# zalo/TetSim

Hardware: AMD Instinct MI355X
Metric: tet_solves_per_sec (higher is better)
Workload: dtype f32; 1 GPU; Kuhn-6 cube lattice 55x55x55 cells (998250 tets, 175616 particles), polar-decomposition Jacobi, 20 substeps/frame, dt=1/1200 s; solver=polar_jacobi, arithmetic=fast, formulation=reference (rest shape carried from substep to substep, 148 B/tet), tets=998250, particles=175616, parallelism=single GPU

## Files before the change

### include/tetsim.h

```cpp
#ifndef TETSIM_H
#define TETSIM_H

#include <stdint.h>

#ifdef __cplusplus
extern "C" {
#endif

#define TETSIM_ABI_VERSION 5

typedef struct tetsim_body *tetsim_handle;

enum {
    TETSIM_OK = 0,
    TETSIM_EINVAL = 1,
    TETSIM_ENODEVICE = 2,
    TETSIM_EHIP = 3,
    TETSIM_ENOMEM = 4,
    TETSIM_ECOMM = 5,
    TETSIM_ESTATE = 6
};

enum {
    TETSIM_SOLVER_POLAR_JACOBI = 0,
// ... 215 lines not shown
       TETSIM_POSE_L0 = 16 , TETSIM_POSE_G = 19 , TETSIM_POSE_Q0 = 25,
       TETSIM_POSE_COM = 26 , TETSIM_POSE_VCOM = 29 , TETSIM_POSE_Q = 32 , TETSIM_POSE_OMEGA = 36 ,
       TETSIM_POSE_L = 39 , TETSIM_POSE_RESIDUAL = 42, TETSIM_POSE_GAP = 43, TETSIM_POSE_RESERVED = 44  };
int tetsim_body_poses_device(tetsim_handle h, void *dst, uint64_t row_stride, void *caller_stream);
int tetsim_read_body_poses(tetsim_handle h, double *out);
int tetsim_prep_pose_table(const float *verts, uint32_t nv, const int32_t *tets, uint32_t nt,
                           const uint32_t *body_first_vert, const uint32_t *body_first_tet, uint32_t num_bodies,
                           double density, void *records_out, double *centres_out);


#define TETSIM_RAY_INVALID (-1)
int tetsim_raycast_visual_device(tetsim_handle h,
        const void *rays,     uint64_t ray_stride,
        const void *ray_body,
        uint32_t count,
        void *hits,           uint64_t hit_stride,
        void *caller_stream);
int tetsim_visual_bounding_spheres_device(tetsim_handle h, void *dst, uint64_t row_stride, void *caller_stream);


#define TETSIM_STRAIN_WIDTH 16
#define TETSIM_STRAIN_BODY_WIDTH 8
#define TETSIM_STRAIN_SWEEPS 4
enum { TETSIM_STRAIN_F = 0 , TETSIM_STRAIN_J = 9, TETSIM_STRAIN_DEV = 10,
       TETSIM_STRAIN_STRETCH = 11 , TETSIM_STRAIN_GREEN = 14, TETSIM_STRAIN_RESERVED = 15  };
int tetsim_tet_strain_device(tetsim_handle h, void *dst, uint64_t row_stride, void *caller_stream);
int tetsim_read_tet_strain(tetsim_handle h, float *out);
int tetsim_body_strain_device(tetsim_handle h, void *dst, uint64_t row_stride, void *caller_stream);
int tetsim_visual_strain_device(tetsim_handle h, int32_t channel, void *dst, uint64_t row_stride, void *caller_stream);
int tetsim_prep_strain_table(const float *verts, uint32_t nv, const int32_t *tets, uint32_t nt, double density, void *records_out);


int tetsim_profile(tetsim_handle h, uint32_t n, double dt, const TetSimParams *params, TetSimProfile *out);
int tetsim_time_kernels(tetsim_handle h, uint32_t reps, double dt, const TetSimParams *params, TetSimProfile *out);
int tetsim_time_step_n(tetsim_handle h, uint32_t n, double dt, const TetSimParams *params, double *ms_out);
int tetsim_measure_copy_bandwidth(int32_t device, uint64_t bytes, uint32_t reps, double *gbps_out);
int tetsim_measure_stream_bandwidth(int32_t device, uint64_t bytes, uint32_t reps, int32_t kind, double *gbps_out);


int tetsim_comm_unique_id(void *id128);
int tetsim_comm_init(tetsim_handle h, const void *id128, int32_t rank, int32_t nranks);
typedef struct TetSimCommInfo {
    int32_t rccl_ranks, rccl_rank;
    uint32_t neighbours;
    uint64_t send_bytes_per_substep, recv_bytes_per_substep, max_message_bytes;
    int32_t loopback;
    int32_t p2p;
} TetSimCommInfo;
int tetsim_comm_info(tetsim_handle h, TetSimCommInfo *out);
int tetsim_comm_selftest(tetsim_handle h);
int tetsim_comm_probe(tetsim_handle h, uint64_t bytes, uint32_t reps, int32_t use_graph, uint32_t per_graph,
                      double *host_us, double *total_us);
int tetsim_halo_probe(tetsim_handle h, uint32_t reps, double *min_us, double *median_us, double *max_us);
#define TETSIM_P2P_BLOB_BYTES 512
int tetsim_halo_p2p_export(tetsim_handle h, void *blob);
int tetsim_halo_p2p_connect(tetsim_handle h, const void *blobs, uint32_t count);
int tetsim_halo_p2p_probe(tetsim_handle h, uint32_t reps, double *min_us, double *median_us, double *max_us);
int tetsim_group_step_n(tetsim_handle *handles, uint32_t count, uint32_t n, double dt, const TetSimParams *params);
int tetsim_halo_exchange_local(tetsim_handle *handles, uint32_t count);
int tetsim_get_halo_plan(tetsim_handle h, int32_t *neigh ,
                         int32_t *send_counts, int32_t *recv_counts,
                         int32_t *send_ids, int32_t *recv_ids);
int tetsim_halo_export(tetsim_handle h, uint32_t n, float *out_xyzw);
int tetsim_halo_import(tetsim_handle h, uint32_t n, const float *in_xyzw);


int tetsim_prep_levels(const int32_t *tets, uint32_t nt, uint32_t nv, int32_t *level, uint32_t *num_levels);
int tetsim_prep_colours(const int32_t *tets, uint32_t nt, uint32_t nv, int32_t *colour, uint32_t *num_colours);
int tetsim_prep_clusters(const int32_t *tets, uint32_t nt, uint32_t nv, int32_t *order, int32_t *launch, int32_t *lane,
                         int32_t *step, uint32_t *num_launches, uint32_t *num_clusters);
int tetsim_prep_tiles(const float *verts, uint32_t nv, const int32_t *tets, uint32_t nt, const uint32_t *body_first_tet,
                      const uint32_t *body_first_vert, uint32_t bodies, int32_t *tile_tets, uint32_t *tile_off,
                      uint8_t *corner_slot, uint32_t *num_tiles);
int tetsim_prep_slot_table(const int32_t *tets, uint32_t nt, uint32_t nv, int32_t ref_quirk,
                           int32_t *slots , uint32_t *dropped);
int tetsim_prep_call_tiles(const float *verts, uint32_t nv, const int32_t *tets, uint32_t nt, uint32_t sizes[4],
                           uint32_t *blk_vert_off, int32_t *blk_verts, uint32_t *vp_ell);
int tetsim_prep_call_schedule(const int32_t *blk_verts, const uint32_t *blk_vert_off, uint32_t nb, const uint32_t *vp_ell,
                              uint32_t vp_cols, uint32_t nv_pad, uint32_t nv_owned, uint32_t lag, uint32_t *entry,
                              uint32_t capacity, uint32_t *period, uint32_t *tail, int32_t *fell_back);
int tetsim_prep_check_call_schedule(const int32_t *blk_verts, const uint32_t *blk_vert_off, uint32_t nb, const uint32_t *vp_ell,
                                    uint32_t vp_cols, uint32_t nv_pad, uint32_t nv_owned, const uint32_t *entry, uint32_t period,
                                    uint32_t tail);
int tetsim_prep_ref_grab_texels(int32_t grab_id, uint32_t num_elems, uint32_t num_particles, int32_t out[2]);
int tetsim_prep_boundary_surface(const float *verts ,
                                 const int32_t *tets, uint32_t nt, uint32_t nv,
                                 float *vis_verts , int32_t *tri_ids ,
                                 uint32_t *nrows, uint32_t *ntri);
int tetsim_prep_rest(const float *verts, uint32_t nv, const int32_t *tets, uint32_t nt, double density,
                     float *inv_mass, float *inv_rest_pose, float *inv_rest_volume);

int tetsim_prep_partition(const float *verts , uint32_t nv, const int32_t *tets, uint32_t nt,
                          int32_t part_count, int32_t *vert_owner_out);
typedef struct TetSimPartQuality {
    uint32_t owned_particles;
    uint32_t ghost_particles;
    uint32_t boundary_particles;
    uint32_t local_elems;
    uint32_t owned_elems;
    uint32_t num_neighbours;
} TetSimPartQuality;
int tetsim_prep_partition_quality(const int32_t *tets, uint32_t nt, uint32_t nv, int32_t part_count,
                                  const int32_t *vert_owner, TetSimPartQuality *out);

typedef struct tetsim_plan_s *tetsim_plan;
typedef struct TetSimPlanSizes {
    uint32_t owned_particles, boundary_particles, local_particles, local_elems, owned_elems, num_neighbours;
} TetSimPlanSizes;
int tetsim_plan_create(const int32_t *tets, uint32_t nt, uint32_t nv, int32_t part_count, int32_t part_index,
                       const int32_t *vert_owner, tetsim_plan *out);
int tetsim_plan_create_deep(const int32_t *tets, uint32_t nt, uint32_t nv, int32_t part_count, int32_t part_index,
                            const int32_t *vert_owner, int32_t depth, tetsim_plan *out);
int tetsim_plan_layers(tetsim_plan p, uint32_t *first_layer_ghosts, uint8_t *tet_layer);
int tetsim_plan_neighbour_layer2(tetsim_plan p, uint32_t i, uint32_t *send_count, uint32_t *recv_start, uint32_t *recv_count);
int tetsim_plan_neighbour_layer2_ids(tetsim_plan p, uint32_t i, int32_t *send_local, int32_t *send_global, int32_t *recv_global);
void tetsim_plan_destroy(tetsim_plan p);
int tetsim_plan_sizes(tetsim_plan p, TetSimPlanSizes *out);
int tetsim_plan_arrays(tetsim_plan p, int32_t *local_to_global_vert, int32_t *local_to_global_tet, int32_t *local_tets);
int tetsim_plan_neighbour(tetsim_plan p, uint32_t i, int32_t *rank, uint32_t *send_count, uint32_t *recv_start,
                          uint32_t *recv_count, int32_t *send_is_contiguous);
int tetsim_plan_neighbour_ids(tetsim_plan p, uint32_t i, int32_t *send_local, int32_t *send_global, int32_t *recv_global);

int tetsim_abi_version(void);
typedef struct TetSimLibraryInfo {
    int32_t abi;
    int32_t ablation;
    uint32_t debug_env;
    char source_sha[20];
    char kernel_sha[20];
} TetSimLibraryInfo;
int tetsim_library_info(TetSimLibraryInfo *out);

typedef struct TetSimMeshArrays {
    uint32_t num_particles;
    uint32_t num_elems;
    uint32_t num_edges;
    uint32_t num_vis_verts;
    uint32_t num_vis_tris;
    uint32_t part_count;
    const float *verts;
    const int32_t *tets;
    const int32_t *edge_ids;
    const float *vis_verts;
    const int32_t *vis_tri_ids;
    const int32_t *tet_colour;
    const int32_t *vert_owner;
} TetSimMeshArrays;
typedef struct tetsim_mesh_file *tetsim_mesh;

int tetsim_mesh_write(const char *path, const TetSimMeshArrays *a);
int tetsim_mesh_open(const char *path, tetsim_mesh *out);
int tetsim_mesh_arrays(tetsim_mesh m, TetSimMeshArrays *out);
int tetsim_mesh_close(tetsim_mesh m);
int tetsim_create_from_file(const char *path, const TetSimOptions *opts, tetsim_handle *out);

#ifdef __cplusplus
}
#endif
#endif
```

### tetsim_amd/_capi.py

```python
import ctypes as C
import os

_HERE = os.path.dirname(os.path.abspath(__file__))
LIB_PATH = os.environ.get("TETSIM_HIP_LIB") or os.path.join(_HERE, "libtetsim_hip.so")

OK, EINVAL, ENODEVICE, EHIP, ENOMEM, ECOMM, ESTATE = range(7)
RAY_INVALID = -1
SOLVER_POLAR_JACOBI, SOLVER_NEOHOOKEAN_GS = 0, 1
PRECISE, FAST = 0, 1
ORDER_ORIGINAL, ORDER_COLOURED, ORDER_CLUSTERED = 0, 1, 2
FLAG_REF_SLOT_TABLE, FLAG_REF_FIXED_BOUNDS, FLAG_GATHER_FORMULATION, FLAG_CONSTANT_REST_SHAPE, FLAG_REF_GRAB_TEXEL, FLAG_DEEP_GHOSTS = 1, 2, 4, 8, 16, 32
FLAG_REF_ROTATION_EXIT = 64
FLAG_LEAN_STATE = 128
K_TET, K_VERTEX, K_HALO, K_COUNT = 0, 1, 2, 3
COLLIDER_SPHERE, COLLIDER_CAPSULE, COLLIDER_BOX, COLLIDER_PLANE = 0, 1, 2, 3
MAX_COLLIDERS = 8
BODY_COLLIDER_FLOATS = 24
BODY_PARAMS_WIDTH = 10
BP_GRAVITY, BP_FRICTION, BP_DEV_COMPLIANCE, BP_VOL_COMPLIANCE, BP_BOUNDS_LO, BP_BOUNDS_HI = 0, 1, 2, 3, 4, 7
FIELD_POSITIONS, FIELD_VELOCITIES, FIELD_PREV_POSITIONS, FIELD_QUATS, FIELD_VISUAL_POSITIONS, FIELD_VISUAL_NORMALS, FIELD_VISUAL_VERTEX_NORMALS = range(7)
MAX_EXPORT_FIELDS = 8
OBS_WIDTH = 20
(OBS_MASS, OBS_COM, OBS_VCOM, OBS_VOLUME, OBS_REST_VOLUME, OBS_MIN_VOLUME_RATIO, OBS_INVERTED_TETS, OBS_AABB_MIN, OBS_AABB_MAX, OBS_MAX_SPEED2,
 OBS_NONFINITE, OBS_RESERVED) = 0, 1, 4, 7, 8, 9, 10, 11, 14, 17, 18, 19
# ... 40 lines not shown
                ("substeps", C.c_uint32), ("tets_per_tet_launch", C.c_uint32)]


class TetSimLibraryInfo(C.Structure):
    _fields_ = [("abi", C.c_int32), ("ablation", C.c_int32), ("debug_env", C.c_uint32), ("source_sha", C.c_char * 20),
                ("kernel_sha", C.c_char * 20)]


DEBUG_ENV_NAMES = ["TETSIM_DEBUG_LOOPBACK_HALO", "TETSIM_DEBUG_LOOPBACK_COPY", "TETSIM_DEBUG_ONE_STREAM", "TETSIM_DEBUG_GROUP_SYNC",
                   "TETSIM_DEBUG_HOSTPROF", "TETSIM_DEBUG_TRACE", "TETSIM_HALO_SYNC", "TETSIM_HALO_GRAPH", "TETSIM_DEBUG_LOOPBACK_DELAY_US", "TETSIM_NH_QUADS", "TETSIM_FUSED_PARTICLE_PASS",
                   "TETSIM_FRAME_KERNEL", "TETSIM_FRAME_LOCAL", "TETSIM_NH_FOLD", "TETSIM_HALO_ALIGNED_TILES", "TETSIM_HALO_FOLD_WAIT", "TETSIM_QUAD", "TETSIM_QUAD_POLL_DELAY", "TETSIM_NH_FRAME",
                   "TETSIM_NH_ONE_LAUNCH", "TETSIM_PJ_ONE_LAUNCH", "TETSIM_PJ_CALL_LAG"]


LAB_ENV_NAMES = ["TETSIM_DEBUG_TRACE", "TETSIM_NH_QUADS", "TETSIM_FRAME_LOCAL", "TETSIM_NH_FOLD", "TETSIM_HALO_ALIGNED_TILES", "TETSIM_QUAD_POLL_DELAY", "TETSIM_NH_FRAME"]


class TetSimCommInfo(C.Structure):
    _fields_ = [("rccl_ranks", C.c_int32), ("rccl_rank", C.c_int32), ("neighbours", C.c_uint32), ("send_bytes_per_substep", C.c_uint64),
                ("recv_bytes_per_substep", C.c_uint64), ("max_message_bytes", C.c_uint64), ("loopback", C.c_int32), ("p2p", C.c_int32)]


class TetSimPlanSizes(C.Structure):
    _fields_ = [("owned_particles", C.c_uint32), ("boundary_particles", C.c_uint32), ("local_particles", C.c_uint32),
                ("local_elems", C.c_uint32), ("owned_elems", C.c_uint32), ("num_neighbours", C.c_uint32)]


class TetSimPartQuality(C.Structure):
    _fields_ = [("owned_particles", C.c_uint32), ("ghost_particles", C.c_uint32), ("boundary_particles", C.c_uint32),
                ("local_elems", C.c_uint32), ("owned_elems", C.c_uint32), ("num_neighbours", C.c_uint32)]


class TetSimError(RuntimeError):
    def __init__(self, code, msg):
        super().__init__("tetsim error %d: %s" % (code, msg))
        self.code = code


class TetSimCollider(C.Structure):
    _fields_ = [("kind", C.c_int32), ("reserved", C.c_int32), ("a", C.c_double * 3), ("b", C.c_double * 3), ("axes", C.c_double * 9),
                ("radius", C.c_double), ("friction", C.c_double), ("velocity", C.c_double * 3)]


class TetSimRay(C.Structure):
    _fields_ = [("origin", C.c_double * 3), ("direction", C.c_double * 3), ("near", C.c_double), ("far", C.c_double)]


class TetSimRayHit(C.Structure):
    _fields_ = [("hit", C.c_int32), ("body", C.c_int32), ("triangle", C.c_int32), ("reserved", C.c_int32), ("distance", C.c_double),
                ("point", C.c_double * 3)]


class TetSimDeviceField(C.Structure):
    _fields_ = [("field", C.c_int32), ("reserved", C.c_int32), ("dst", C.c_void_p), ("row_stride", C.c_uint64)]


SYMBOLS = [
    "tetsim_abi_version", "tetsim_default_options", "tetsim_default_params", "tetsim_create", "tetsim_create_batch", "tetsim_get_batch_layout", "tetsim_destroy",
    "tetsim_last_error", "tetsim_get_info", "tetsim_step", "tetsim_step_n", "tetsim_sync",
    "tetsim_library_info", "tetsim_read_quats_pinned", "tetsim_state_size", "tetsim_save_state", "tetsim_load_state",
    "tetsim_read_positions", "tetsim_read_positions_pinned", "tetsim_read_prev_positions", "tetsim_read_velocities", "tetsim_read_quats",
    "tetsim_read_vol_error", "tetsim_write_state", "tetsim_get_owned_ids", "tetsim_get_local_tets",
    "tetsim_get_tet_order", "tetsim_get_level_offsets", "tetsim_read_inv_mass", "tetsim_set_visual_mesh", "tetsim_get_visual_ids", "tetsim_halo_refresh_final", "tetsim_group_refresh_final", "tetsim_halo_probe", "tetsim_halo_p2p_probe",
    "tetsim_read_visual_mesh", "tetsim_set_visual_triangles", "tetsim_read_visual_vertex_normals", "tetsim_visual_vertex_normals_from", "tetsim_group_read_visual_vertex_normals", "tetsim_set_grab", "tetsim_set_colliders",
    "tetsim_start_grab", "tetsim_nearest_particle", "tetsim_profile", "tetsim_time_kernels", "tetsim_time_step_n", "tetsim_measure_copy_bandwidth", "tetsim_measure_stream_bandwidth",
    "tetsim_comm_unique_id", "tetsim_comm_init", "tetsim_comm_info", "tetsim_comm_selftest", "tetsim_comm_probe", "tetsim_group_step_n", "tetsim_halo_exchange_local", "tetsim_get_halo_plan",
    "tetsim_halo_p2p_export", "tetsim_halo_p2p_connect",
    "tetsim_halo_export", "tetsim_halo_import", "tetsim_prep_levels", "tetsim_prep_colours", "tetsim_prep_clusters",
    "tetsim_prep_tiles", "tetsim_prep_slot_table", "tetsim_prep_call_tiles", "tetsim_prep_call_schedule", "tetsim_prep_check_call_schedule", "tetsim_prep_ref_grab_texels", "tetsim_prep_rest", "tetsim_prep_partition", "tetsim_prep_partition_quality", "tetsim_plan_create", "tetsim_plan_destroy", "tetsim_plan_sizes",
    "tetsim_plan_arrays", "tetsim_plan_neighbour", "tetsim_plan_neighbour_ids",
    "tetsim_plan_create_deep", "tetsim_plan_layers", "tetsim_plan_neighbour_layer2", "tetsim_plan_neighbour_layer2_ids",
    "tetsim_raycast_visual", "tetsim_start_grab_ray", "tetsim_read_visual_bounding_sphere", "tetsim_prep_boundary_surface",
    "tetsim_export_device", "tetsim_import_device",
    "tetsim_snapshot_create", "tetsim_snapshot_capture", "tetsim_snapshot_restore", "tetsim_snapshot_destroy",
    "tetsim_observe_bodies_device", "tetsim_read_body_observations",
    "tetsim_body_poses_device", "tetsim_read_body_poses", "tetsim_prep_pose_table",
    "tetsim_raycast_visual_device", "tetsim_visual_bounding_spheres_device",
    "tetsim_tet_strain_device", "tetsim_read_tet_strain", "tetsim_body_strain_device", "tetsim_visual_strain_device", "tetsim_prep_strain_table",
    "tetsim_set_body_grabs", "tetsim_set_body_grabs_device", "tetsim_nearest_particles_device",
    "tetsim_set_body_colliders", "tetsim_set_body_colliders_device",
    "tetsim_set_body_params", "tetsim_set_body_params_device",
    "tetsim_place_bodies_device", "tetsim_place_bodies",
    "tetsim_mesh_write", "tetsim_mesh_open", "tetsim_mesh_arrays", "tetsim_mesh_close", "tetsim_create_from_file",
]

OPTIONAL_SYMBOLS = ("tetsim_set_colliders", "tetsim_raycast_visual", "tetsim_start_grab_ray", "tetsim_read_visual_bounding_sphere", "tetsim_prep_boundary_surface",
                    "tetsim_export_device", "tetsim_import_device",
                    "tetsim_snapshot_create", "tetsim_snapshot_capture", "tetsim_snapshot_restore", "tetsim_snapshot_destroy",
                    "tetsim_observe_bodies_device", "tetsim_read_body_observations",
                    "tetsim_raycast_visual_device", "tetsim_visual_bounding_spheres_device",
                    "tetsim_tet_strain_device", "tetsim_read_tet_strain", "tetsim_body_strain_device", "tetsim_visual_strain_device", "tetsim_prep_strain_table",
                    "tetsim_set_body_grabs", "tetsim_set_body_grabs_device", "tetsim_nearest_particles_device",
                    "tetsim_set_body_colliders", "tetsim_set_body_colliders_device",
                    "tetsim_set_body_params", "tetsim_set_body_params_device",
                    "tetsim_place_bodies_device", "tetsim_place_bodies",
                    "tetsim_body_poses_device", "tetsim_read_body_poses", "tetsim_prep_pose_table")

_lib = None


def lib():
    global _lib
    if _lib is not None:
        return _lib
    if not os.path.exists(LIB_PATH):
        raise ImportError("libtetsim_hip.so is not built: run `python -m tetsim_amd.build` "
                          "(the HIP extension is mandatory; there is no CPU fallback)")
    L = C.CDLL(LIB_PATH)
    H, fp, ip, dp = C.c_void_p, C.POINTER(C.c_float), C.POINTER(C.c_int32), C.POINTER(C.c_double)
    u32, i32, dbl = C.c_uint32, C.c_int32, C.c_double
    PP = C.POINTER(TetSimParams)
    L.tetsim_abi_version.restype = C.c_int
    L.tetsim_default_options.argtypes = [C.POINTER(TetSimOptions)]
    L.tetsim_default_options.restype = None
    L.tetsim_default_params.argtypes = [PP]
    L.tetsim_default_params.restype = None
    L.tetsim_create.argtypes = [fp, u32, ip, u32, C.POINTER(TetSimOptions), C.POINTER(H)]
    L.tetsim_create_batch.argtypes = [C.POINTER(fp), C.POINTER(u32), C.POINTER(ip), C.POINTER(u32), u32, C.POINTER(TetSimOptions), C.POINTER(H)]
    L.tetsim_get_batch_layout.argtypes = [H, C.POINTER(u32), C.POINTER(u32)]
    L.tetsim_destroy.argtypes = [H]
    L.tetsim_destroy.restype = None
    L.tetsim_comm_probe.argtypes = [H, C.c_uint64, u32, i32, u32, dp, dp]
    L.tetsim_nearest_particle.argtypes = [H, fp, ip, dp]
    L.tetsim_mesh_write.argtypes = [C.c_char_p, C.POINTER(TetSimMeshArrays)]
    L.tetsim_mesh_open.argtypes = [C.c_char_p, C.POINTER(H)]
    L.tetsim_mesh_arrays.argtypes = [H, C.POINTER(TetSimMeshArrays)]
    L.tetsim_mesh_close.argtypes = [H]
    L.tetsim_create_from_file.argtypes = [C.c_char_p, C.POINTER(TetSimOptions), C.POINTER(H)]
    L.tetsim_last_error.argtypes = [H]
    L.tetsim_last_error.restype = C.c_char_p
    L.tetsim_get_info.argtypes = [H, C.POINTER(TetSimInfo)]
    L.tetsim_step.argtypes = [H, dbl, PP]
    L.tetsim_step_n.argtypes = [H, u32, dbl, PP]
    L.tetsim_sync.argtypes = [H]
    for n in ("positions", "prev_positions", "velocities", "quats", "inv_mass"):
        getattr(L, "tetsim_read_" + n).argtypes = [H, fp]
    L.tetsim_read_positions_pinned.argtypes = [H, C.POINTER(fp)]
    L.tetsim_read_quats_pinned.argtypes = [H, C.POINTER(fp)]
    L.tetsim_library_info.argtypes = [C.POINTER(TetSimLibraryInfo)]
    L.tetsim_state_size.argtypes = [H, C.POINTER(C.c_uint64)]
    L.tetsim_save_state.argtypes = [H, C.c_void_p, C.c_uint64]
    L.tetsim_load_state.argtypes = [H, C.c_void_p, C.c_uint64]
    L.tetsim_read_vol_error.argtypes = [H, dp]
    L.tetsim_write_state.argtypes = [H, fp, fp]
    for n in ("owned_ids", "local_tets", "tet_order", "level_offsets"):
        getattr(L, "tetsim_get_" + n).argtypes = [H, ip]
    L.tetsim_set_visual_mesh.argtypes = [H, fp, u32, fp]
    L.tetsim_read_visual_mesh.argtypes = [H, fp, fp]
    L.tetsim_get_visual_ids.argtypes = [H, C.POINTER(C.c_int32)]
    L.tetsim_halo_refresh_final.argtypes = [H]
    L.tetsim_halo_probe.argtypes = [H, u32, C.POINTER(C.c_double), C.POINTER(C.c_double), C.POINTER(C.c_double)]
    L.tetsim_halo_p2p_probe.argtypes = [H, u32, C.POINTER(C.c_double), C.POINTER(C.c_double), C.POINTER(C.c_double)]
    L.tetsim_group_refresh_final.argtypes = [C.POINTER(H), u32]
    L.tetsim_set_visual_triangles.argtypes = [H, ip, u32]
    L.tetsim_read_visual_vertex_normals.argtypes = [H, fp]
    L.tetsim_visual_vertex_normals_from.argtypes = [H, fp, fp]
    L.tetsim_group_read_visual_vertex_normals.argtypes = [C.POINTER(H), u32, fp, fp]
    L.tetsim_set_grab.argtypes = [H, i32, fp]
    if hasattr(L, "tetsim_set_colliders"):
        L.tetsim_set_colliders.argtypes = [H, C.POINTER(TetSimCollider), u32]
    L.tetsim_start_grab.argtypes = [H, fp, ip]
    if hasattr(L, "tetsim_raycast_visual"):
        L.tetsim_raycast_visual.argtypes = [H, C.c_void_p, u32, C.c_void_p]
        L.tetsim_start_grab_ray.argtypes = [H, C.POINTER(TetSimRay), C.POINTER(TetSimRayHit), ip]
        L.tetsim_read_visual_bounding_sphere.argtypes = [H, dp, dp]
        L.tetsim_prep_boundary_surface.argtypes = [fp, ip, u32, u32, fp, ip, C.POINTER(u32), C.POINTER(u32)]
    if hasattr(L, "tetsim_export_device"):
        L.tetsim_export_device.argtypes = [H, C.POINTER(TetSimDeviceField), u32, C.c_void_p]
        L.tetsim_import_device.argtypes = [H, C.c_void_p, C.c_uint64, C.c_void_p, C.c_uint64, C.c_void_p]
    if hasattr(L, "tetsim_snapshot_create"):
        L.tetsim_snapshot_create.argtypes = [H, C.POINTER(H)]
        L.tetsim_snapshot_capture.argtypes = [H, H, C.c_void_p, C.c_void_p]
        L.tetsim_snapshot_restore.argtypes = [H, H, C.c_void_p, C.c_void_p]
        L.tetsim_snapshot_destroy.argtypes = [H]
        L.tetsim_snapshot_destroy.restype = None
    if hasattr(L, "tetsim_observe_bodies_device"):
        L.tetsim_observe_bodies_device.argtypes = [H, C.c_void_p, C.c_uint64, C.c_void_p]
        L.tetsim_read_body_observations.argtypes = [H, dp]
    if hasattr(L, "tetsim_raycast_visual_device"):
        L.tetsim_raycast_visual_device.argtypes = [H, C.c_void_p, C.c_uint64, C.c_void_p, u32, C.c_void_p, C.c_uint64, C.c_void_p]
        L.tetsim_visual_bounding_spheres_device.argtypes = [H, C.c_void_p, C.c_uint64, C.c_void_p]
    if hasattr(L, "tetsim_tet_strain_device"):
        L.tetsim_tet_strain_device.argtypes = [H, C.c_void_p, C.c_uint64, C.c_void_p]
        L.tetsim_read_tet_strain.argtypes = [H, fp]
        L.tetsim_body_strain_device.argtypes = [H, C.c_void_p, C.c_uint64, C.c_void_p]
        L.tetsim_visual_strain_device.argtypes = [H, i32, C.c_void_p, C.c_uint64, C.c_void_p]
        L.tetsim_prep_strain_table.argtypes = [fp, u32, ip, u32, dbl, C.c_void_p]
    if hasattr(L, "tetsim_set_body_grabs"):
        L.tetsim_set_body_grabs.argtypes = [H, ip, fp]
        L.tetsim_set_body_grabs_device.argtypes = [H, C.c_void_p, C.c_void_p, C.c_uint64, C.c_void_p, C.c_void_p]
        L.tetsim_nearest_particles_device.argtypes = [H, C.c_void_p, C.c_uint64, C.c_void_p, C.c_void_p, C.c_void_p]
    if hasattr(L, "tetsim_set_body_colliders"):
        L.tetsim_set_body_colliders.argtypes = [H, fp, u32]
        L.tetsim_set_body_colliders_device.argtypes = [H, C.c_void_p, C.c_uint64, u32, C.c_void_p, C.c_void_p]
    if hasattr(L, "tetsim_set_body_params"):
        L.tetsim_set_body_params.argtypes = [H, C.POINTER(C.c_double)]
        L.tetsim_set_body_params_device.argtypes = [H, C.c_void_p, C.c_uint64, C.c_void_p, C.c_void_p]
    if hasattr(L, "tetsim_place_bodies_device"):
        L.tetsim_place_bodies_device.argtypes = [H, C.c_void_p, C.c_uint64, C.c_void_p, u32, C.c_void_p]
        L.tetsim_place_bodies.argtypes = [H, fp, C.POINTER(C.c_uint8), u32]
    if hasattr(L, "tetsim_body_poses_device"):
        L.tetsim_body_poses_device.argtypes = [H, C.c_void_p, C.c_uint64, C.c_void_p]
        L.tetsim_read_body_poses.argtypes = [H, dp]
        L.tetsim_prep_pose_table.argtypes = [fp, u32, ip, u32, C.POINTER(u32), C.POINTER(u32), u32, dbl, C.c_void_p, dp]
    L.tetsim_profile.argtypes = [H, u32, dbl, PP, C.POINTER(TetSimProfile)]
    L.tetsim_time_kernels.argtypes = [H, u32, dbl, PP, C.POINTER(TetSimProfile)]
    L.tetsim_time_step_n.argtypes = [H, u32, dbl, PP, dp]
    L.tetsim_measure_copy_bandwidth.argtypes = [i32, C.c_uint64, u32, dp]
    L.tetsim_measure_stream_bandwidth.argtypes = [i32, C.c_uint64, u32, i32, dp]
    L.tetsim_comm_unique_id.argtypes = [C.c_void_p]
    L.tetsim_comm_init.argtypes = [H, C.c_void_p, i32, i32]
    L.tetsim_comm_selftest.argtypes = [H]
    L.tetsim_comm_info.argtypes = [H, C.POINTER(TetSimCommInfo)]
    L.tetsim_group_step_n.argtypes = [C.POINTER(H), u32, u32, dbl, PP]
    L.tetsim_halo_exchange_local.argtypes = [C.POINTER(H), u32]
    L.tetsim_halo_p2p_export.argtypes = [H, C.c_void_p]
    L.tetsim_halo_p2p_connect.argtypes = [H, C.c_void_p, u32]
    L.tetsim_get_halo_plan.argtypes = [H, ip, ip, ip, ip, ip]
    L.tetsim_halo_export.argtypes = [H, u32, fp]
    L.tetsim_halo_import.argtypes = [H, u32, fp]
    L.tetsim_prep_levels.argtypes = [ip, u32, u32, ip, C.POINTER(u32)]
    L.tetsim_prep_colours.argtypes = [ip, u32, u32, ip, C.POINTER(u32)]
    L.tetsim_prep_clusters.argtypes = [ip, u32, u32, ip, ip, ip, ip, C.POINTER(u32), C.POINTER(u32)]
    L.tetsim_prep_tiles.argtypes = [fp, u32, ip, u32, C.POINTER(u32), C.POINTER(u32), u32, ip, C.POINTER(u32), C.POINTER(C.c_uint8), C.POINTER(u32)]
    L.tetsim_prep_slot_table.argtypes = [ip, u32, u32, i32, ip, C.POINTER(u32)]
    up = C.POINTER(u32)
    L.tetsim_prep_call_tiles.argtypes = [fp, u32, ip, u32, up, up, ip, up]
    L.tetsim_prep_call_schedule.argtypes = [ip, up, u32, up, u32, u32, u32, u32, up, u32, up, up, ip]
    L.tetsim_prep_check_call_schedule.argtypes = [ip, up, u32, up, u32, u32, u32, up, u32, u32]
    L.tetsim_prep_ref_grab_texels.argtypes = [i32, u32, u32, ip]
    L.tetsim_prep_rest.argtypes = [fp, u32, ip, u32, dbl, fp, fp, fp]
    L.tetsim_prep_partition.argtypes = [fp, u32, ip, u32, i32, ip]
    L.tetsim_prep_partition_quality.argtypes = [ip, u32, u32, i32, ip, C.POINTER(TetSimPartQuality)]
    L.tetsim_plan_create.argtypes = [ip, u32, u32, i32, i32, ip, C.POINTER(H)]
    L.tetsim_plan_destroy.argtypes = [H]
    L.tetsim_plan_destroy.restype = None
    L.tetsim_plan_sizes.argtypes = [H, C.POINTER(TetSimPlanSizes)]
    L.tetsim_plan_arrays.argtypes = [H, ip, ip, ip]
    L.tetsim_plan_neighbour.argtypes = [H, u32, ip, C.POINTER(u32), C.POINTER(u32), C.POINTER(u32), ip]
    L.tetsim_plan_neighbour_ids.argtypes = [H, u32, ip, ip, ip]
    L.tetsim_plan_create_deep.argtypes = [ip, u32, u32, i32, i32, ip, i32, C.POINTER(H)]
    L.tetsim_plan_layers.argtypes = [H, C.POINTER(u32), C.POINTER(C.c_uint8)]
    L.tetsim_plan_neighbour_layer2.argtypes = [H, u32, C.POINTER(u32), C.POINTER(u32), C.POINTER(u32)]
    L.tetsim_plan_neighbour_layer2_ids.argtypes = [H, u32, ip, ip, ip]
    for s in SYMBOLS:
        if s in OPTIONAL_SYMBOLS and not hasattr(L, s):
            continue
        f = getattr(L, s)
        if s not in ("tetsim_default_options", "tetsim_default_params", "tetsim_destroy", "tetsim_last_error",
                     "tetsim_plan_destroy", "tetsim_snapshot_destroy"):
            f.restype = C.c_int
    _lib = L
    return L


def library_info():
    li = TetSimLibraryInfo()
    check(lib().tetsim_library_info(C.byref(li)))
    return {"abi": li.abi, "ablation": bool(li.ablation), "source_sha": li.source_sha.decode(), "kernel_sha": li.kernel_sha.decode(),
            "debug_env": [n for i, n in enumerate(DEBUG_ENV_NAMES) if li.debug_env >> i & 1], "path": LIB_PATH}


def check(rc, handle=None):
    if rc != OK:
        msg = lib().tetsim_last_error(handle)
        raise TetSimError(rc, msg.decode("utf-8", "replace") if msg else "")
```

### tetsim_amd/csrc/body.h

```cpp
#pragma once
#include <dlfcn.h>
#include <hip/hip_runtime.h>
#include <rccl/rccl.h>

#include <algorithm>
#include <atomic>
#include <chrono>
#include <cmath>
#include <cstdio>
#include <cstdlib>
#include <cstring>
#include <map>
#include <string>
#include <vector>

#include "../../include/tetsim.h"
#include "dev_common.h"
#include "dev_store.h"
#include "query_device.h"
#include "host_prep.h"
#include "mesh_file.h"

namespace tetsim {

// ... 105 lines not shown
    double* partial = nullptr;
    float* rows = nullptr;
    bool ready = false;
};

struct PoseRec {
    double m;
    double q[3];
};
static_assert(sizeof(PoseRec) == 32 && alignof(PoseRec) == 8, "two dwordx4 loads per record");
struct PoseDev {
    const void* table = nullptr;
    double* partial = nullptr;
    double* rows = nullptr;
    bool ready = false;
};

}

using namespace tetsim;

struct tetsim_snapshot_s;

struct tetsim_body {
    std::string err;
    TetSimOptions opt{};
    TetSimInfo info{};
    hipStream_t stream = nullptr, comm_stream = nullptr;
    hipEvent_t ev_fork = nullptr, ev_bnd_tet = nullptr;
    uint32_t interior_tets = 0;
    bool queues_probed = false, queues_independent = false;
    uint64_t probe_generation = 0;
    std::map<uint32_t, std::pair<hipGraphExec_t, hipGraphExec_t>> flag_graphs;
    uint32_t* d_sync = nullptr;
    bool flag_sync = false;
    bool halo_graph_broken = false;
    bool halo_warm = false;
    bool loopback = false;
    bool vel_dead = false;
    bool needs_halo_refresh = false;
    bool fork_needed = true;
    hipEvent_t ev_a = nullptr, ev_b = nullptr, ev_halo = nullptr;
    hipEvent_t ev_boundary2[2] = {nullptr, nullptr}, ev_packed2[2] = {nullptr, nullptr}, ev_sent2[2] = {nullptr, nullptr};
    uint32_t halo_parity = 0;
    DevParams* d_params = nullptr;
    DevParams* d_params_halo = nullptr;
    std::vector<int32_t> tet_colour;
    int32_t grab_global = -1;
    int32_t grab_ref[2] = {-1, -1};
    float grab_pos[3] = {0, 0, 0};
    uint32_t n_colliders = 0;
    DevColliderF col[kMaxColliders] = {};
    DevColliderD d_col[kMaxColliders] = {};
    bool body_grabs_on = false;
    uint32_t* d_grab_body = nullptr;
    int4* d_grab_rows = nullptr;
    bool body_colliders_on = false;
    uint32_t* d_bcol_count = nullptr;
    DevColliderF* d_bcol_f = nullptr;
    DevColliderD* d_bcol_d = nullptr;
    bool body_params_on = false;
    BodyParamsF* d_bp_f = nullptr;
    BodyParamsD* d_bp_d = nullptr;
    uint32_t* d_tet_body = nullptr;
    uint32_t* d_body_first = nullptr;
    double* d_near_d2 = nullptr;
    uint32_t* d_near_id = nullptr;
    std::map<uint32_t, hipGraphExec_t> graphs;
    std::vector<void*> allocs;
    std::vector<float> h_verts;
    std::vector<int32_t> h_tets;
    std::vector<uint32_t> batch_first_vert, batch_first_tet;
    bool fast = false;

    PJDev pj;
    PJBlk blk;
    bool blocked = false;
    bool halo_use_flags = true;
    bool halo_use_graph = true;
    bool fused = false;
    bool pj_one_launch = false;
    uint32_t* d_substep_err = nullptr;
    PJCallSched call_sched;
    float4 *rest0_a = nullptr, *rest0_b = nullptr, *rest0_c = nullptr;
    bool quat_stale = false;
    bool frame = false;
    uint32_t frame_epoch = 1;
    uint32_t fold_wave_limit = 0, fold_tile_limit = 0;
    bool quad = false;
    uint32_t* d_frame_err = nullptr;
    int32_t* d_block_tile = nullptr;
    uint32_t frame_blocks = 0;
    DevParams params_on_device;
    bool params_known = false;
    bool frame_local = false;
    bool frame_turn_counted = false;
    bool epoch_block_fresh = false;
    bool frame_exclusive = false;
    float4* partial_b = nullptr;
    size_t partial_slots = 0;
    float4* pos_final_b = nullptr;
    bool fold_halo = false;
    bool fold_possible = false;
    bool fold_wait = false;
    bool v_pending = false;
    uint32_t fuse_step = 0;
    bool fin_in_b = false;
    std::vector<int32_t> tet_perm;
    std::vector<uint32_t> api2dev, dev2api;
    Partition part;
    bool partitioned = false;
    std::vector<int32_t> g2l_owned;
    std::vector<NeighDev> neigh;
    bool pred_any_dt = true;
    float dt_pred = 0.0f;
    ncclComm_t comm = nullptr;
    int comm_rank = -1, comm_size = 0;
    bool deep = false;
    uint32_t n_ghost1 = 0, nb_first = 0;
    std::vector<int32_t> g2l_ghost1;
    bool p2p = false;
    uint32_t timeout_ms = 0;
    float4* ghost_alt = nullptr;
    uint32_t* d_arrived = nullptr;
    uint32_t* d_peer_slots = nullptr;
    uint32_t p2p_cols = 0, p2p_stride = 0;
    uint32_t* d_peer_slots2 = nullptr;
    uint32_t p2p_cols2 = 0;
    float4* own_g1_even[2] = {nullptr, nullptr};
    float4* own_g1_final[2] = {nullptr, nullptr};
    float4* own_g2_even[2] = {nullptr, nullptr};
    float4* own_g2_odd[2] = {nullptr, nullptr};
    std::vector<PeerLink> links;
    uint32_t p2p_probe_base = 0;
    uint64_t p2p_round = 0;
    bool p2p_raise_pending = false;
    bool halo_pending = false;
    bool final_ghosts_fresh = false;
    std::vector<tetsim_body*> group;

    SkinDev skin;
    std::vector<uint32_t> vis_tet;
    std::vector<int32_t> vis_global;
    bool vis_attached = false;
    uint32_t vis_total = 0;
    float4* d_vis_full = nullptr;
    float* pinned_pos = nullptr;
    float* d_packed = nullptr;
    size_t packed_cap = 0;
    float* pinned_quat = nullptr;
    uint32_t* d_api2dev = nullptr;
    hipEvent_t ev_io[2][2] = {{nullptr, nullptr}, {nullptr, nullptr}};
    uint32_t io_parity = 0;
    std::vector<tetsim_snapshot_s*> snapshots;
    uint32_t *d_snap_first_vert = nullptr, *d_snap_first_elem = nullptr, *d_snap_tet_body = nullptr;
    float* d_place_rows = nullptr;
    uint8_t* d_place_mask = nullptr;
    ChunkTable chunk_table[2];
    ObsDev obs;
    StrainDev strain;
    PoseDev pose;
    double* d_best = nullptr; uint32_t* d_best_id = nullptr;
    uint32_t* d_sphere = nullptr;
    RayIn* d_rays = nullptr; RayPrep* d_ray_prep = nullptr; RayOut* d_ray_hits = nullptr; RayCand* d_ray_cand = nullptr;
    size_t ray_cap = 0, ray_prep_cap = 0, ray_hits_cap = 0, ray_cand_cap = 0;
    std::vector<int32_t> vis_row_body, tri_body;
// ... 196 lines not shown
```

### tetsim_amd/csrc/dev_common.h

```cpp
#pragma once
#include <hip/hip_ext.h>
#include <hip/hip_runtime.h>

#include "host_prep.h"

#include <cstddef>
#include <cstdint>

namespace tetsim {

constexpr uint32_t kMaxColliders = 8;
struct DevColliderF {
    float a[3], b[3], u[9], radius, friction, v[3];
    int32_t kind, pad;
};
struct DevColliderD {
    double a[3], b[3], u[9], radius, friction, v[3];
    int32_t kind, pad;
};

__host__ __device__ inline float ref_fixed_lo(int c) { return c == 1 ? -1.0f : -2.5f; }
__host__ __device__ inline float ref_fixed_hi(int c) { return c == 1 ? 10.0f : 2.5f; }
struct BodyParamsF { float gravity, friction, dev_compliance, vol_compliance, lo[3], hi[3], pad[2]; };
struct BodyParamsD { double gravity, friction, dev_compliance, vol_compliance, lo[3], hi[3]; };
// ... 23 lines not shown
    const BodyParamsD* bp_d;
    const uint32_t* tet_body;
    DevColliderF col[kMaxColliders];
    DevColliderD d_col[kMaxColliders];
};
constexpr size_t kDevParamsHead = offsetof(DevParams, col);
static_assert(kDevParamsHead % 8 == 0 && offsetof(DevParams, d_col) % 8 == 0, "DevParams layout");
constexpr size_t kKernelArgLimit = 4096;
static_assert(sizeof(DevParams) <= 2560, "DevParams must leave room for the other by-value arguments of a launch");
__device__ __forceinline__ void store_params(DevParams* dst, const DevParams& v) {
    const uint2* s = reinterpret_cast<const uint2*>(&v);
    uint2* d = reinterpret_cast<uint2*>(dst);
#pragma unroll
    for (size_t i = 0; i < kDevParamsHead / 8; i++) d[i] = s[i];
    for (uint32_t k = 0; k < v.n_colliders && k < kMaxColliders; k++) { dst->col[k] = v.col[k]; dst->d_col[k] = v.d_col[k]; }
}

__device__ __forceinline__ void body_grab_pick(const DevParams& P, uint32_t v, bool& held, float& x, float& y, float& z) {
    if (P.body_grabs) {
        const int4 row = P.grab_rows[P.grab_body[v]];
        held = row.x == static_cast<int32_t>(v);
        if (held) { x = __int_as_float(row.y); y = __int_as_float(row.z); z = __int_as_float(row.w); }
    }
}
__device__ __forceinline__ uint32_t body_colliders_body(const DevParams& P, uint32_t v) { return P.body_colliders ? P.grab_body[v] : 0u; }
__device__ __forceinline__ void body_colliders_pick(const DevParams& P, uint32_t body, const DevColliderF** list, uint32_t* count) {
    *list = P.col; *count = P.n_colliders;
    if (P.body_colliders) { *list = P.bcol_f + static_cast<size_t>(body) * kMaxColliders; *count = P.bcol_count[body]; }
}
__device__ __forceinline__ void body_colliders_pick(const DevParams& P, uint32_t body, const DevColliderD** list, uint32_t* count) {
    *list = P.d_col; *count = P.n_colliders;
    if (P.body_colliders) { *list = P.bcol_d + static_cast<size_t>(body) * kMaxColliders; *count = P.bcol_count[body]; }
}

__device__ __forceinline__ const BodyParamsF* body_params_row(const DevParams& P, uint32_t body, float) { return P.bp_f + body; }
__device__ __forceinline__ const BodyParamsD* body_params_row(const DevParams& P, uint32_t body, double) { return P.bp_d + body; }
__device__ __forceinline__ uint32_t body_params_uniform(uint32_t body) { return static_cast<uint32_t>(__builtin_amdgcn_readfirstlane(static_cast<int32_t>(body))); }
struct PolarBodyParams { float gravity, friction, lo[3], hi[3]; };
template <bool kUniform>
__device__ __forceinline__ PolarBodyParams body_params_polar(const DevParams& P, uint32_t v) {
    PolarBodyParams o = {P.gravity, P.friction, {P.lo[0], P.lo[1], P.lo[2]}, {P.hi[0], P.hi[1], P.hi[2]}};
    if (P.body_params) {
        uint32_t body = P.grab_body[v];
        if constexpr (kUniform) body = body_params_uniform(body);
        const BodyParamsF* const r = body_params_row(P, body, 0.0f);
        o.gravity = r->gravity; o.friction = r->friction;
        for (int k = 0; k < 3; k++) { o.lo[k] = r->lo[k]; o.hi[k] = r->hi[k]; }
    }
    return o;
}

struct PJDev {
    uint32_t nv_local = 0, nv_owned = 0, nv_boundary = 0, nt = 0;
    uint32_t nt_pad = 0;
    uint32_t nv_pad = 0;
    uint32_t max_valence = 0;
    float4* pos_pred = nullptr;
    float4* pos_final = nullptr;
    float4* vel = nullptr;
    int4* tet_idx = nullptr;
    float4* elem = nullptr;
    float4* quat = nullptr;
    int32_t* slot_tab = nullptr;
    uint32_t* slot_cnt = nullptr;
    const DevParams* params = nullptr;
    float rot_exit_w2 = 1.0e-18f;
};

struct PJBlk {
    uint32_t nb = 0, nb_interior = 0, nt = 0, nv_local = 0, nv_owned = 0, nv_boundary = 0;
    const uint32_t* blk_tet_off = nullptr;
    const uint32_t* blk_vert_off = nullptr;
    const int32_t* blk_verts = nullptr;
    const uchar4* tet_lidx = nullptr;
    float4* rest_a = nullptr;
    float4* rest_b = nullptr;
    float4* rest_c = nullptr;
    float* rest_c1 = nullptr;
    const float* vol = nullptr;
    float4* quat = nullptr;
    const uint32_t* lc_range = nullptr;
    const uint2* lc_ent = nullptr;
    float4* partial = nullptr;
    const float* wsum = nullptr;
    const uint32_t* vp_ell = nullptr;
    uint32_t vp_cols = 0, nv_pad = 0;
    float4* pos_pred = nullptr;
    float4* pos_final = nullptr;
    float4* vel = nullptr;
    const float4* partial_prev = nullptr;
    const float4* fin_in = nullptr;
    float4* fin_out = nullptr;
    const uint32_t* slot_src = nullptr;
    const uint32_t* blk_maxsrc = nullptr;
    uint32_t ns_pad = 0;
    const DevParams* params = nullptr;
    const float4* ghost_alt = nullptr;
    const float4* ghost2 = nullptr;
    uint32_t n_ghost1 = 0xffffffffu;
    bool lean = false;
    bool lean_state = false;
    float rot_exit_w2 = 1.0e-18f;
    uint32_t epoch = 0;
    unsigned long long* trace = nullptr;
    unsigned long long* iter_hist = nullptr;
};

struct NHDev {
    uint32_t nv = 0, nt = 0;
    float4* pos = nullptr;
    float4* prev = nullptr;
    float4* vel = nullptr;
    int4* tet_idx = nullptr;
    float4* irp_a = nullptr;
    float4* irp_b = nullptr;
    float4* irp_c = nullptr;
    double* vol_err = nullptr;
    int32_t* order = nullptr;
    uint32_t* corner_slots = nullptr;
    const DevParams* params = nullptr;
};
constexpr uint32_t max_grid_blocks(uint32_t threads) { return 0xffffffffu / threads; }
struct PJCallSched { const uint32_t* entry = nullptr; uint32_t period = 0, tail = 0; };
constexpr uint32_t pjb_call_chunk(uint32_t period, uint32_t tail, uint32_t threads, uint32_t cap) {
    const uint32_t room = max_grid_blocks(threads) > tail ? max_grid_blocks(threads) - tail : 0u;
    const uint32_t fit = period ? room / period : cap;
    return fit < 1u ? 1u : fit < cap ? fit : cap;
}
constexpr uint32_t nh_call_blocks_per_sub(uint32_t blocks) { return (blocks + 7u) & ~7u; }
constexpr uint32_t call_chunk(uint32_t per_sub, uint32_t threads, uint32_t cap) {
    const uint32_t fit = per_sub ? max_grid_blocks(threads) / per_sub : cap;
    return fit < 1u ? 1u : fit < cap ? fit : cap;
}
static_assert(pjb_call_chunk(pjb_call_blocks_per_sub(2282u, 103823u, 256u), 0u, 256u, 8192u) == 6223u, "46-cell lattice: 2,696 blocks per substep");
static_assert(pjb_call_chunk(pjb_call_blocks_per_sub(2282u, 103823u, 256u), 2696u, 256u, 8192u) == 6222u, "... and a tail of a whole period takes one substep's room");
static_assert(call_chunk(nh_call_blocks_per_sub(2601u), 256u, 65000u / 8u) == 6432u, "55-cell lattice, clustered: 2,608 blocks per substep");

constexpr uint32_t kNHClusterVerts = 8, kNHClusterTets = 8;
struct NHClusterLaunch {
    uint32_t nsteps = 0, clusters = 0;
    uint32_t first[kNHClusterTets] = {}, count[kNHClusterTets] = {};
    const int32_t* slot_vid = nullptr;
    const uint8_t* first_mask = nullptr;
};

struct NHSweepColour {
    NHClusterLaunch L;
    const float* slot_im = nullptr;
    const uint2* delta = nullptr;
    const uint8_t* last_mask = nullptr;
    const uint2* delta_first = nullptr;
    uint32_t first_block = 0;
    uint32_t pad = 0;
};
struct NHSweep {
    const NHSweepColour* colours = nullptr;
    uint32_t ncolours = 0, blocks = 0;
    float4* exchange = nullptr;
    uint32_t* error = nullptr;
    uint32_t timeout_ms = 0;
};
void nh_launch_sweep1_fast(hipStream_t s, const NHDev& d, const NHSweep& w, bool fold, uint32_t sub_index, uint32_t epoch);
void nh_launch_call_fast(hipStream_t s, const NHDev& d, const NHSweep& w, uint32_t n);

void pj_launch_tet_precise(hipStream_t s, const PJDev& d, hipEvent_t e0 = nullptr, hipEvent_t e1 = nullptr);
void pj_launch_tet_fast(hipStream_t s, const PJDev& d, hipEvent_t e0 = nullptr, hipEvent_t e1 = nullptr);
void pj_launch_vertex_precise(hipStream_t s, const PJDev& d, uint32_t first, uint32_t count, hipEvent_t e0 = nullptr, hipEvent_t e1 = nullptr);
void pj_launch_vertex_fast(hipStream_t s, const PJDev& d, uint32_t first, uint32_t count, hipEvent_t e0 = nullptr, hipEvent_t e1 = nullptr);
void pj_launch_repredict_precise(hipStream_t s, const PJDev& d);
void pj_launch_repredict_fast(hipStream_t s, const PJDev& d);

void nh_launch_post_predict_precise(hipStream_t s, const NHDev& d);
void nh_launch_post_predict_fast(hipStream_t s, const NHDev& d);
void nh_launch_cluster_precise(hipStream_t s, const NHDev& d, const NHClusterLaunch& L, bool fold = false);
void nh_launch_cluster_fast(hipStream_t s, const NHDev& d, const NHClusterLaunch& L, bool fold = false);
struct NHFrameLaunch {
    const uint32_t* seg = nullptr;
    const uint32_t* first_vert = nullptr;
    uint32_t levels = 0, bodies = 0, block = 512;
    uint32_t max_body_particles = 0;
};
void nh_launch_frame_precise(hipStream_t s, const NHDev& d, const NHFrameLaunch& f, uint32_t n, const DevParams& params, DevParams* params_dev);
void nh_launch_frame_fast(hipStream_t s, const NHDev& d, const NHFrameLaunch& f, uint32_t n, const DevParams& params, DevParams* params_dev);
constexpr uint32_t kNHQuadLevelFast = 128, kNHQuadLevelPrecise = 64;
void nh_launch_level4_fast(hipStream_t s, const NHDev& d, uint32_t first, uint32_t count);
void nh_launch_level4_precise(hipStream_t s, const NHDev& d, uint32_t first, uint32_t count);
uint32_t nh_frame_lds_limit_precise();
uint32_t nh_frame_lds_limit_fast();
void nh_launch_post_predict_list_precise(hipStream_t s, const NHDev& d, const uint32_t* list, uint32_t n);
void nh_launch_post_predict_list_fast(hipStream_t s, const NHDev& d, const uint32_t* list, uint32_t n);
void pjb_launch_tet(hipStream_t s, const PJBlk& d, uint32_t tile_first, uint32_t tile_count, hipEvent_t e0 = nullptr,
                    hipEvent_t e1 = nullptr, uint32_t* raise_word = nullptr, uint32_t* clear_word = nullptr);
void pjb_launch_call(hipStream_t s, const PJBlk& d, const PJCallSched& sched, uint32_t n, uint32_t* err, uint32_t timeout_ms, const DevParams& params, DevParams* params_dev);
void pjb_launch_tet_fused(hipStream_t s, const PJBlk& d, hipEvent_t e0 = nullptr, hipEvent_t e1 = nullptr);
void pjb_launch_vertex(hipStream_t s, const PJBlk& d, uint32_t first, uint32_t count, hipEvent_t e0 = nullptr, hipEvent_t e1 = nullptr,
                       uint32_t* raise_word = nullptr, uint32_t* clear_word = nullptr);
void pjb_launch_repredict(hipStream_t s, const PJBlk& d);
void pjb_launch_recover_quats(hipStream_t s, const PJBlk& d, const float4* rest0_a, const float4* rest0_b, const float4* rest0_c);
void pjb_launch_frame(hipStream_t s, const PJBlk& d, uint32_t n, const int32_t* block_tile, uint32_t blocks, bool local, float4* pbuf0, float4* pbuf1,
                      uint32_t* err, uint32_t timeout_ms, const DevParams& params, DevParams* params_dev, hipEvent_t e0 = nullptr, hipEvent_t e1 = nullptr);
void pjq_launch_frame(hipStream_t s, const PJBlk& d, uint32_t n, const int32_t* block_tile, uint32_t blocks, bool local, float4* pbuf0, float4* pbuf1,
                      uint32_t* err, uint32_t timeout_ms, const DevParams& params, DevParams* params_dev, hipEvent_t e0 = nullptr, hipEvent_t e1 = nullptr);
void pjq_launch_tet(hipStream_t s, const PJBlk& d, hipEvent_t e0 = nullptr, hipEvent_t e1 = nullptr);
void pjq_launch_vertex(hipStream_t s, const PJBlk& d, hipEvent_t e0 = nullptr, hipEvent_t e1 = nullptr);
uint32_t pjq_frame_capacity(uint32_t* compute_units);
uint32_t pjb_frame_capacity(int mode, uint32_t* compute_units);
void pjb_wait_capacity(int mode, uint32_t* vertex_waves, uint32_t* hwait_blocks);
inline int pjb_mode(const PJBlk& d) { return d.lean ? 1 : d.lean_state ? 2 : 0; }
uint32_t pjb_probe_xcd(hipStream_t s, uint32_t blocks);
struct PJSync {
    uint32_t* flag = nullptr;
    uint32_t* error = nullptr;
    uint32_t timeout_ms = 0;
};
constexpr uint32_t kMaxPeers = 8;
struct PJPeer {
    float4* ghost[kMaxPeers] = {};
    const uint32_t* slots = nullptr;
    uint32_t cols = 0, stride = 0, n = 0;
    float4* fin[kMaxPeers] = {};
    float4* ghost2[kMaxPeers] = {};
    const uint32_t* slots2 = nullptr;
    uint32_t cols2 = 0;
};
struct PJPeerSync {
    uint32_t* raise[kMaxPeers] = {};
    uint32_t* wait[kMaxPeers] = {};
    uint32_t n_raise = 0, n_wait = 0;
    uint32_t delay_us = 0;
};
void pjb_launch_wait(hipStream_t s, const PJSync& y);
void pjb_launch_wait_peers(hipStream_t s, const PJSync& y, const PJPeerSync& w);
struct PJClear { uint32_t* word[kMaxPeers + 1] = {}; uint32_t n = 0; };
void pjb_launch_vertex_peer(hipStream_t s, const PJBlk& d, uint32_t first, uint32_t count, const PJPeer& peer, uint32_t* raise_word, const PJClear& clr = PJClear());
void pjb_launch_tet_hwait(hipStream_t s, const PJBlk& d, uint32_t tile_first, uint32_t tile_count, const PJSync& yv, const PJPeerSync& w, const float4* ghosts);
void pjb_launch_tet_alt(hipStream_t s, const PJBlk& d, uint32_t tile_first, uint32_t tile_count);
void pjb_launch_signal(hipStream_t s, const PJSync& y, uint32_t* clear_word = nullptr);
void pjb_launch_vertex_await(hipStream_t s, const PJBlk& d, uint32_t first, uint32_t count, const PJSync& y, hipEvent_t e0 = nullptr, hipEvent_t e1 = nullptr);

void nh_launch_predict_precise(hipStream_t s, const NHDev& d);
void nh_launch_predict_fast(hipStream_t s, const NHDev& d);
void nh_launch_predict_value_precise(hipStream_t s, const NHDev& d, const DevParams& params, DevParams* params_dev);
void nh_launch_predict_value_fast(hipStream_t s, const NHDev& d, const DevParams& params, DevParams* params_dev);
void nh_launch_level_precise(hipStream_t s, const NHDev& d, uint32_t first, uint32_t count);
void nh_launch_level_fast(hipStream_t s, const NHDev& d, uint32_t first, uint32_t count);
void nh_launch_post_precise(hipStream_t s, const NHDev& d);
void nh_launch_post_fast(hipStream_t s, const NHDev& d);

struct SkinDev {
    uint32_t nvis = 0;
    const int4* corner = nullptr;
    const float4* weight = nullptr;
    const int32_t* qidx = nullptr;
    const float4* normal0 = nullptr;
    float4* out_pos = nullptr;
    float4* out_nrm = nullptr;
    uint32_t ntri = 0;
    const int4* tri = nullptr;
    const uint32_t* vt_off = nullptr;
    const uint32_t* vt_tri = nullptr;
    float4* out_vnrm = nullptr;
    const float4* tri_pos = nullptr;
};
void skin_launch(hipStream_t s, const SkinDev& d, const float4* pos, const float4* quat, bool js_order);
void skin_launch_vertex_normals(hipStream_t s, const SkinDev& d);

void util_launch_nearest(hipStream_t s, const float4* pos, const uint32_t* map, uint32_t n, double px, double py, double pz,
                         double* best_d2, uint32_t* best_id);
void util_launch_copy(hipStream_t s, const float4* src, float4* dst, uint64_t n);
void util_launch_stream(hipStream_t s, int kind, bool nt, uint32_t unroll, uint32_t grid, const float4* src, float4* dst, uint64_t n);
void util_launch_delay(hipStream_t s, uint32_t us);
struct P2PProbe { uint32_t* raise[kMaxPeers] = {}; uint32_t* wait[kMaxPeers] = {}; uint32_t n = 0; };
void util_launch_set_params(hipStream_t s, DevParams* dst, const DevParams& v);
void util_launch_p2p_probe(hipStream_t s, const P2PProbe& p, uint32_t base, uint32_t reps, unsigned long long* ticks, uint32_t* error, uint32_t timeout_ms);
void util_launch_gather4(hipStream_t s, const float4* src, const int32_t* idx, float4* dst, uint32_t n);

// ... 25 lines not shown
```

### tetsim_amd/csrc/dev_store.h

```cpp
#pragma once
#include <hip/hip_runtime.h>

#ifndef TETSIM_POLL_SLEEP
#define TETSIM_POLL_SLEEP 8
#endif
#ifndef TETSIM_NH_POLL_SLEEP
#define TETSIM_NH_POLL_SLEEP 2
#endif

namespace tetsim {

constexpr uint32_t kStoreWtMaxIndex = 1u << 27;

typedef unsigned int v4u_t __attribute__((ext_vector_type(4)));

__device__ __forceinline__ void store_wt(float4* base, uint32_t index, const float4& v) {
    const __amdgpu_buffer_rsrc_t rsrc = __builtin_amdgcn_make_buffer_rsrc(base, 0, 0x7fffffff, 0x00020000);
    const v4u_t x = {__float_as_uint(v.x), __float_as_uint(v.y), __float_as_uint(v.z), __float_as_uint(v.w)};
    __builtin_amdgcn_raw_buffer_store_b128(x, rsrc, static_cast<int>(index * 16u), 0, 0x11);
}

__device__ __forceinline__ void store_wt1(float* base, uint32_t index, float v) {
    const __amdgpu_buffer_rsrc_t rsrc = __builtin_amdgcn_make_buffer_rsrc(base, 0, 0x7fffffff, 0x00020000);
    __builtin_amdgcn_raw_buffer_store_b32(__float_as_uint(v), rsrc, static_cast<int>(index * 4u), 0, 0x11);
}

__device__ __forceinline__ void store_plain(float4* base, uint32_t index, const float4& v) {
    const __amdgpu_buffer_rsrc_t rsrc = __builtin_amdgcn_make_buffer_rsrc(base, 0, 0x7fffffff, 0x00020000);
    const v4u_t x = {__float_as_uint(v.x), __float_as_uint(v.y), __float_as_uint(v.z), __float_as_uint(v.w)};
    __builtin_amdgcn_raw_buffer_store_b128(x, rsrc, static_cast<int>(index * 16u), 0, 0);
}
__device__ __forceinline__ float4 load_l2(const float4* base, uint32_t index) {
    const __amdgpu_buffer_rsrc_t rsrc = __builtin_amdgcn_make_buffer_rsrc(const_cast<float4*>(base), 0, 0x7fffffff, 0x00020000);
    const v4u_t x = __builtin_amdgcn_raw_buffer_load_b128(rsrc, static_cast<int>(index * 16u), 0, 0x10);
    return make_float4(__uint_as_float(x.x), __uint_as_float(x.y), __uint_as_float(x.z), __uint_as_float(x.w));
}

__device__ __forceinline__ float4 load_coherent(const float4* base, uint32_t index) {
    const __amdgpu_buffer_rsrc_t rsrc = __builtin_amdgcn_make_buffer_rsrc(const_cast<float4*>(base), 0, 0x7fffffff, 0x00020000);
    const v4u_t x = __builtin_amdgcn_raw_buffer_load_b128(rsrc, static_cast<int>(index * 16u), 0, 0x11);
    return make_float4(__uint_as_float(x.x), __uint_as_float(x.y), __uint_as_float(x.z), __uint_as_float(x.w));
}

__device__ __forceinline__ float load_coherent1(const float* base, uint32_t index) {
    const __amdgpu_buffer_rsrc_t rsrc = __builtin_amdgcn_make_buffer_rsrc(const_cast<float*>(base), 0, 0x7fffffff, 0x00020000);
    return __uint_as_float(__builtin_amdgcn_raw_buffer_load_b32(rsrc, static_cast<int>(index * 4u), 0, 0x11));
}

}
```

### tetsim_amd/csrc/host_prep.cpp

```cpp
#include "host_prep.h"

#include <algorithm>
#include <cmath>
#include <numeric>

namespace tetsim {

namespace {
inline float fround(double x) { return static_cast<float>(x); }

inline void edge_matrix(const float* verts, const int32_t* t, float m[9]) {
    for (int k = 0; k < 3; k++)
        for (int c = 0; c < 3; c++)
            m[3 * k + c] = fround(static_cast<double>(verts[3 * t[k + 1] + c]) - static_cast<double>(verts[3 * t[0] + c]));
}
inline double det3(const float* A) {
    double a11 = A[0], a12 = A[3], a13 = A[6];
    double a21 = A[1], a22 = A[4], a23 = A[7];
    double a31 = A[2], a32 = A[5], a33 = A[8];
    return a11 * a22 * a33 + a12 * a23 * a31 + a13 * a21 * a32 - a13 * a22 * a31 - a12 * a21 * a33 - a11 * a23 * a32;
}
}

void prep_rest(const float* verts, uint32_t nv, const int32_t* tets, uint32_t nt, double density,
// ... 468 lines not shown
namespace {
struct SchedDeps {
    uint32_t per_xcd = 0, tet_blocks = 0, npb = 0, plain_period = 0;
    std::vector<std::vector<uint32_t>> tiles_of_pb, pbs_of_tile;
};
SchedDeps sched_deps(const int32_t* blk_verts, const uint32_t* blk_vert_off, uint32_t nb, const uint32_t* vp_ell, uint32_t vp_cols, uint32_t nv_pad,
                     uint32_t nv_owned, uint32_t tile) {
    SchedDeps D;
    D.per_xcd = (nb + 7u) / 8u; D.tet_blocks = D.per_xcd * 8u; D.npb = (nv_owned + tile - 1u) / tile;
    D.plain_period = pjb_call_blocks_per_sub(nb, nv_owned, tile);
    D.tiles_of_pb.resize(D.npb); D.pbs_of_tile.resize(nb);
    for (uint32_t v = 0; v < nv_owned; v++)
        for (uint32_t j = 0; j < vp_cols; j++) {
            const uint32_t idx = vp_ell[static_cast<size_t>(j) * nv_pad + v];
            if (idx == 0xffffffffu) continue;
            const uint32_t b = static_cast<uint32_t>(std::upper_bound(blk_vert_off, blk_vert_off + nb + 1, idx) - blk_vert_off) - 1u;
            if (b < nb) D.tiles_of_pb[v / tile].push_back(b);
        }
    for (uint32_t b = 0; b < nb; b++)
        for (uint32_t g = blk_vert_off[b]; g < blk_vert_off[b + 1]; g++)
            if (static_cast<uint32_t>(blk_verts[g]) < nv_owned) D.pbs_of_tile[b].push_back(static_cast<uint32_t>(blk_verts[g]) / tile);
    auto uniq = [](std::vector<uint32_t>& v) { std::sort(v.begin(), v.end()); v.erase(std::unique(v.begin(), v.end()), v.end()); };
    for (auto& v : D.tiles_of_pb) uniq(v);
    for (auto& v : D.pbs_of_tile) uniq(v);
    return D;
}
inline uint32_t sched_tile_of(uint32_t r, uint32_t per_xcd) { return (r & 7u) * per_xcd + (r >> 3); }
void sched_plain(const SchedDeps& D, uint32_t nb, CallSchedule* out) {
    out->period = D.plain_period;
    out->tail = 0; out->lag = 0;
    out->entry.assign(out->period, sched_entry(kSchedEmpty, 0));
    for (uint32_t r = 0; r < D.tet_blocks; r++)
        if (sched_tile_of(r, D.per_xcd) < nb) out->entry[r] = sched_entry(kSchedTile, r);
    for (uint32_t k = 0; k < D.npb; k++) out->entry[D.tet_blocks + k] = sched_entry(kSchedParticles, k);
}
struct SchedPass { std::vector<uint32_t> entry, ready, left; uint32_t head_end = 0; bool stuck = false; };
SchedPass sched_pass(const SchedDeps& D, uint32_t nb, uint32_t lag, const std::vector<uint32_t>& head_at) {
    constexpr uint32_t none = 0xffffffffu;
    SchedPass R;
    R.ready.assign(D.npb, none);
    std::vector<uint32_t> need(D.npb), head, queue;
    std::vector<uint8_t> head_placed(D.npb, 0);
    for (uint32_t k = 0; k < D.npb; k++) {
        need[k] = static_cast<uint32_t>(D.tiles_of_pb[k].size());
        if (head_at[k] != none) head.push_back(k);
        if (need[k] == 0) { R.ready[k] = 0; if (head_at[k] == none) queue.push_back(k); }
    }
    std::stable_sort(head.begin(), head.end(), [&](uint32_t a, uint32_t b) { return head_at[a] < head_at[b]; });
    std::vector<std::vector<uint32_t>> pbs_by_tile(nb);
    for (uint32_t k = 0; k < D.npb; k++) for (uint32_t b : D.tiles_of_pb[k]) pbs_by_tile[b].push_back(k);
    size_t hi = 0, qi = 0;
    uint32_t col_next[8] = {}, tiles_left = D.tet_blocks;
    const uint64_t limit = 4ull * (D.tet_blocks + D.npb) + 64ull * (static_cast<uint64_t>(lag) + 1ull) + 64ull;
    for (uint32_t p = 0;; p++) {
        if (tiles_left == 0 && hi == head.size() && (p & 7u) == 0u) break;
        if (p >= limit) { R.stuck = true; break; }
        const uint32_t x = p & 7u;
        if (hi < head.size() && head_at[head[hi]] <= p) {
            const uint32_t k = head[hi++];
            R.entry.push_back(sched_entry(kSchedParticles, k, true));
            head_placed[k] = 1; R.head_end = p + 1u;
            continue;
        }
        if (qi < queue.size() && R.ready[queue[qi]] <= p) { R.entry.push_back(sched_entry(kSchedParticles, queue[qi++])); continue; }
        if (col_next[x] < D.per_xcd) {
            const uint32_t r = 8u * col_next[x] + x, b = sched_tile_of(r, D.per_xcd);
            bool held = false;
            if (b < nb) for (uint32_t k : D.pbs_of_tile[b]) held = held || (head_at[k] != none && !head_placed[k]);
            if (!held) {
                col_next[x]++; tiles_left--;
                R.entry.push_back(b < nb ? sched_entry(kSchedTile, r) : sched_entry(kSchedEmpty, 0));
                if (b < nb) for (uint32_t k : pbs_by_tile[b])
                    if (--need[k] == 0) { R.ready[k] = p + 8u * lag; if (head_at[k] == none) queue.push_back(k); }
                continue;
            }
        }
        R.entry.push_back(sched_entry(kSchedEmpty, 0));
    }
    R.left.assign(queue.begin() + static_cast<std::ptrdiff_t>(qi), queue.end());
    return R;
}
}

std::string check_call_schedule(const int32_t* blk_verts, const uint32_t* blk_vert_off, uint32_t nb, const uint32_t* vp_ell, uint32_t vp_cols,
                                uint32_t nv_pad, uint32_t nv_owned, const uint32_t* entry, uint32_t period, uint32_t tail, uint32_t tile) {
    constexpr uint32_t none = 0xffffffffu;
    const SchedDeps D = sched_deps(blk_verts, blk_vert_off, nb, vp_ell, vp_cols, nv_pad, nv_owned, tile);
    if (period == 0 || period % 8u != 0u) return "the period is not a positive multiple of 8";
    if (period < D.plain_period) return "the period is shorter than a substep's blocks";
    std::vector<uint64_t> at_tile(nb, none), at_pb(D.npb, none);
    uint32_t col_seen[8] = {}, wrapped_end = 0;
    for (uint32_t p = 0; p < period; p++) {
        const uint32_t kind = entry[p] >> 30, index = entry[p] & kSchedIndexMask;
        const bool wrapped = (entry[p] & kSchedWrapped) != 0u;
        if (kind == kSchedEmpty) continue;
        if (kind == kSchedTile) {
            const uint32_t b = sched_tile_of(index, D.per_xcd);
            if (index >= D.tet_blocks || b >= nb) return "entry " + std::to_string(p) + " names a tile that does not exist";
            if ((index & 7u) != (p & 7u)) return "tile block " + std::to_string(index) + " is not on its XCD";
            if (wrapped) return "tile block " + std::to_string(index) + " is wrapped";
            if ((index >> 3) < col_seen[p & 7u]) return "tile block " + std::to_string(index) + " is out of its XCD's order";
            col_seen[p & 7u] = (index >> 3) + 1u;
            if (at_tile[b] != none) return "tile " + std::to_string(b) + " appears twice";
            at_tile[b] = p;
        } else if (kind == kSchedParticles) {
            if (index >= D.npb) return "entry " + std::to_string(p) + " names a particle block that does not exist";
            if (at_pb[index] != none) return "particle block " + std::to_string(index) + " appears twice";
            at_pb[index] = static_cast<uint64_t>(p) + (wrapped ? period : 0u);
            if (wrapped) wrapped_end = p + 1u;
        } else return "entry " + std::to_string(p) + " has no kind";
    }
    for (uint32_t b = 0; b < nb; b++) if (at_tile[b] == none) return "tile " + std::to_string(b) + " is missing";
    for (uint32_t k = 0; k < D.npb; k++) if (at_pb[k] == none) return "particle block " + std::to_string(k) + " is missing";
    if (tail < wrapped_end || tail > period) return "the tail does not cover the wrapped entries";
    for (uint32_t k = 0; k < D.npb; k++)
        for (uint32_t b : D.tiles_of_pb[k])
            if (!(at_tile[b] < at_pb[k])) return "particle block " + std::to_string(k) + " does not follow tile " + std::to_string(b) + " of its lists";
    for (uint32_t b = 0; b < nb; b++)
        for (uint32_t k : D.pbs_of_tile[b])
            if (!(at_pb[k] < at_tile[b] + period)) return "tile " + std::to_string(b) + " of the next substep does not follow particle block " + std::to_string(k);
    return "";
}

void build_call_schedule(const int32_t* blk_verts, const uint32_t* blk_vert_off, uint32_t nb, const uint32_t* vp_ell, uint32_t vp_cols,
                         uint32_t nv_pad, uint32_t nv_owned, uint32_t lag, CallSchedule* out, uint32_t tile) {
    constexpr uint32_t none = 0xffffffffu;
    const SchedDeps D = sched_deps(blk_verts, blk_vert_off, nb, vp_ell, vp_cols, nv_pad, nv_owned, tile);
    *out = CallSchedule();
    auto plain = [&](const std::string& why) {
        sched_plain(D, nb, out);
        out->fell_back = !why.empty(); out->why = why;
    };
    if (lag == 0 || nb == 0) return plain("");
    if (static_cast<uint64_t>(lag) * 8u >= D.plain_period) return plain("lag " + std::to_string(lag) + ": a whole substep or more");
    std::vector<uint32_t> head_at(D.npb, none);
    SchedPass R;
    bool settled = false;
    for (int pass = 0; pass < 64 && !settled; pass++) {
        R = sched_pass(D, nb, lag, head_at);
        if (R.stuck) return plain("lag " + std::to_string(lag) + ": the layout does not close");
        const uint32_t period = static_cast<uint32_t>(R.entry.size());
        settled = R.left.empty();
        for (uint32_t k : R.left) head_at[k] = 0;
        for (uint32_t k = 0; k < D.npb; k++)
            if (head_at[k] != none && !settled) head_at[k] = R.ready[k] != none && R.ready[k] > period ? R.ready[k] - period : 0u;
    }
    if (!settled) return plain("lag " + std::to_string(lag) + ": the wrapped blocks do not settle");
    out->entry = R.entry;
    out->period = static_cast<uint32_t>(R.entry.size());
    out->tail = R.head_end;
    out->lag = lag;
    const std::string bad = check_call_schedule(blk_verts, blk_vert_off, nb, vp_ell, vp_cols, nv_pad, nv_owned, out->entry.data(), out->period, out->tail, tile);
    if (!bad.empty()) return plain("lag " + std::to_string(lag) + ": " + bad);
}

std::string validate_mesh(const float* verts, uint32_t nv, const int32_t* tets, uint32_t nt, bool forbid_repeats) {
    if ((nv && !verts) || (nt && !tets)) return "null mesh pointer";
    if (nv == 0) return "mesh has no vertices";
    if (nv > 0x3fffffffu || nt > 0x1fffffffu) return "mesh too large for 32-bit slot encoding";
    for (uint32_t e = 0; e < nt; e++) {
        const int32_t* t = &tets[4 * e];
        for (int k = 0; k < 4; k++)
            if (t[k] < 0 || static_cast<uint32_t>(t[k]) >= nv)
                return "tet " + std::to_string(e) + " references vertex " + std::to_string(t[k]) + " outside [0," + std::to_string(nv) + ")";
        if (forbid_repeats && (t[0] == t[1] || t[0] == t[2] || t[0] == t[3] || t[1] == t[2] || t[1] == t[3] || t[2] == t[3]))
            return "tet " + std::to_string(e) + " repeats a vertex (unsupported by the parallel Gauss-Seidel schedule)";
    }
    return "";
}

std::string build_partition(const int32_t* tets, uint32_t nt, uint32_t nv, int part_count, int part_index,
                            const int32_t* vert_owner, Partition* out, int depth) {
    Partition& P = *out;
    P = Partition();
    P.nv_global = nv;
    P.nt_global = nt;
    P.part_count = part_count;
    P.part_index = part_index;
    P.depth = depth;
    if (part_count < 1 || part_index < 0 || part_index >= part_count) return "bad part_index/part_count";
    if (depth != 1 && depth != 2) return "ghost depth must be 1 or 2";

    std::vector<int32_t> owner(nv);
    if (vert_owner) {
        for (uint32_t v = 0; v < nv; v++) {
            if (vert_owner[v] < 0 || vert_owner[v] >= part_count) return "vert_owner out of range";
            owner[v] = vert_owner[v];
        }
    } else {
        const std::string perr = prep_partition(nullptr, nv, tets, nt, part_count, owner.data());
        if (!perr.empty()) return perr;
    }
    const int me = part_index;

    std::vector<std::vector<int32_t>> near1(nv), near2(depth == 2 ? nv : 0);
    auto add = [](std::vector<int32_t>& s, int32_t r) { if (std::find(s.begin(), s.end(), r) == s.end()) s.push_back(r); };
    for (uint32_t e = 0; e < nt; e++) {
        const int32_t* t = &tets[4 * e];
        const int32_t o[4] = {owner[t[0]], owner[t[1]], owner[t[2]], owner[t[3]]};
        if (o[0] == o[1] && o[1] == o[2] && o[2] == o[3]) continue;
        for (int a = 0; a < 4; a++)
            for (int b = 0; b < 4; b++)
                if (o[b] != o[a]) add(near1[t[a]], o[b]);
    }
    if (depth == 2)
        for (uint32_t e = 0; e < nt; e++) {
            const int32_t* t = &tets[4 * e];
            for (int a = 0; a < 4; a++)
                for (int32_t r : near1[t[a]])
                    for (int b = 0; b < 4; b++) {
                        const int32_t v = t[b];
                        if (owner[v] != r && std::find(near1[v].begin(), near1[v].end(), r) == near1[v].end()) add(near2[v], r);
                    }
        }
    auto reads = [&](const std::vector<std::vector<int32_t>>& near, uint32_t v, int32_t r) {
        return !near.empty() && std::find(near[v].begin(), near[v].end(), r) != near[v].end();
    };

    for (uint32_t e = 0; e < nt; e++) {
        const int32_t* t = &tets[4 * e];
        bool mine = false, first_layer = false;
        int lowest = part_count;
        for (int k = 0; k < 4; k++) {
            if (owner[t[k]] == me) mine = true;
            else if (reads(near1, static_cast<uint32_t>(t[k]), me)) first_layer = true;
            lowest = std::min(lowest, owner[t[k]]);
        }
        if (!mine && !(depth == 2 && first_layer)) continue;
        P.local_to_global_tet.push_back(static_cast<int32_t>(e));
        P.tet_layer.push_back(mine ? 0 : 1);
        if (mine && lowest == me) P.owned_tets++;
    }

    std::vector<int32_t> g2l(nv, -1);
    auto is_boundary = [&](uint32_t v) { return !near1[v].empty() || (depth == 2 && !near2[v].empty()); };
    for (uint32_t v = 0; v < nv; v++)
// ... 52 lines not shown
```

### tetsim_amd/csrc/host_prep.h

```cpp
#pragma once
#include <cstdint>
#include <string>
#include <vector>

namespace tetsim {

constexpr int kRefSlots = 36;

void prep_rest(const float* verts, uint32_t nv, const int32_t* tets, uint32_t nt, double density,
               float* inv_mass, float* inv_rest_pose, float* inv_rest_volume);

float pj_inv_rest_volume(const float* verts, const int32_t* tet);

uint32_t prep_levels(const int32_t* tets, uint32_t nt, uint32_t nv, int32_t* level);
uint32_t prep_colours(const int32_t* tets, uint32_t nt, uint32_t nv, int32_t* colour);
constexpr uint32_t kClusterTets = 8, kClusterVerts = 8;
struct ClusterPlan {
    std::vector<int32_t> pre;
    std::vector<uint32_t> exec_pos;
    std::vector<uint32_t> corner_slots;
    std::vector<uint32_t> launch_off;
    std::vector<uint32_t> step_off;
    std::vector<uint32_t> step_first, step_count;
    std::vector<uint32_t> vid_off;
// ... 8 lines not shown
    std::vector<int32_t> slot;
    uint32_t max_valence = 0;
    uint32_t dropped = 0;
};
Incidence build_incidence(const int32_t* tets, uint32_t nt, uint32_t nv, bool ref_quirk, bool ref_cap);

struct Partition {
    uint32_t nv_global = 0, nt_global = 0;
    int part_count = 1, part_index = 0;
    std::vector<int32_t> local_to_global_vert;
    uint32_t n_owned = 0, n_boundary = 0;
    std::vector<int32_t> local_to_global_tet;
    std::vector<int32_t> local_tets;
    uint32_t owned_tets = 0;
    struct Neighbour {
        int rank;
        std::vector<int32_t> send_local;
        std::vector<int32_t> send_global;
        uint32_t recv_start = 0, recv_count = 0;
        std::vector<int32_t> recv_global;
        bool send_contiguous = false;
        std::vector<int32_t> send2_local, send2_global;
        uint32_t recv2_start = 0, recv2_count = 0;
        std::vector<int32_t> recv2_global;
    };
    std::vector<Neighbour> neigh;
    int depth = 1;
    uint32_t n_ghost1 = 0;
    std::vector<uint8_t> tet_layer;
};
std::string prep_partition(const float* verts, uint32_t nv, const int32_t* tets, uint32_t nt, int parts, int32_t* out_owner);
struct PartQuality {
    uint32_t owned_particles = 0, ghost_particles = 0, boundary_particles = 0;
    uint32_t local_elems = 0, owned_elems = 0;
    uint32_t num_neighbours = 0;
};
std::string partition_quality(const int32_t* tets, uint32_t nt, uint32_t nv, int parts, const int32_t* owner, PartQuality* out);
std::string build_partition(const int32_t* tets, uint32_t nt, uint32_t nv, int part_count, int part_index,
                            const int32_t* vert_owner, Partition* out, int depth = 1);

std::vector<uint32_t> morton_vertex_order(const float* xyz, uint32_t n, uint32_t first, uint32_t count);

#ifndef TETSIM_TILE
#define TETSIM_TILE 256
#endif
constexpr uint32_t kBlockTile = TETSIM_TILE;
constexpr uint32_t kQuadTile = 64;
constexpr int32_t kQuadPollDelay = 0;
constexpr uint32_t kQuadMaxPartials = 12;
struct BlockPlan {
    uint32_t num_blocks = 0;
    uint32_t tile = kBlockTile;
    std::vector<int32_t> tet_perm;
    std::vector<uint32_t> blk_tet_off;
    std::vector<uint32_t> blk_vert_off;
    std::vector<int32_t> blk_verts;
    std::vector<uint8_t> tet_lidx;
    std::vector<uint32_t> lc_range;
    std::vector<uint16_t> lc_ent;
    std::vector<uint32_t> vp_off;
    std::vector<uint32_t> vp_idx;
    std::vector<uint32_t> vp_ell;
    uint32_t vp_cols = 0;
    std::vector<uint32_t> slot_src;
    std::vector<uint32_t> blk_maxsrc;
    uint32_t ns_pad = 0;
    bool every_owned_particle_has_a_partial = true;
    uint32_t nv_pad = 0;
    uint32_t max_tile_verts = 0, max_partials = 0;
    uint32_t num_interior_blocks = 0;
    uint32_t num_first_blocks = 0;
};
void build_blocks(const float* verts, const int32_t* tets, uint32_t nt, uint32_t nv, uint32_t nv_sum,
                  const Incidence& inc, BlockPlan* out, const uint32_t* body_first_tet = nullptr,
                  const uint32_t* body_first_vert = nullptr, uint32_t bodies = 1, uint32_t nv_boundary = 0,
                  const uint8_t* tet_class = nullptr, uint32_t nv_owned = 0xffffffffu, uint32_t tile = kBlockTile);

constexpr uint32_t kSchedTile = 0u, kSchedParticles = 1u, kSchedEmpty = 2u, kSchedWrapped = 1u << 29, kSchedIndexMask = (1u << 29) - 1u;
constexpr uint32_t sched_entry(uint32_t kind, uint32_t index, bool wrapped = false) { return kind << 30 | (wrapped ? kSchedWrapped : 0u) | index; }
constexpr uint32_t pjb_call_blocks_per_sub(uint32_t nb, uint32_t nv_owned, uint32_t threads) {
    return (((nb + 7u) & ~7u) + (nv_owned + threads - 1u) / threads + 7u) & ~7u;
}
constexpr uint32_t kPJCallLagDefault = 0;
struct CallSchedule {
    std::vector<uint32_t> entry;
    uint32_t period = 0, tail = 0;
    uint32_t lag = 0;
    bool fell_back = false;
    std::string why;
};
void build_call_schedule(const int32_t* blk_verts, const uint32_t* blk_vert_off, uint32_t nb, const uint32_t* vp_ell, uint32_t vp_cols,
                         uint32_t nv_pad, uint32_t nv_owned, uint32_t lag, CallSchedule* out, uint32_t tile = kBlockTile);
std::string check_call_schedule(const int32_t* blk_verts, const uint32_t* blk_vert_off, uint32_t nb, const uint32_t* vp_ell, uint32_t vp_cols,
                                uint32_t nv_pad, uint32_t nv_owned, const uint32_t* entry, uint32_t period, uint32_t tail, uint32_t tile = kBlockTile);

std::string validate_mesh(const float* verts, uint32_t nv, const int32_t* tets, uint32_t nt, bool forbid_repeats);

}
```

### tetsim_amd/csrc/pj_blocked.hip

```cpp
#define TETSIM_FAST 1
#include <cstdio>
#include <algorithm>
#include <cstdlib>
#include <type_traits>
#include <vector>

#include "collide.h"
#include "dev_common.h"
#include "dev_store.h"
#include "host_prep.h"
#include "pj_lab.h"

namespace tetsim {
namespace {

#include "pj_math.inc"
#include "pj_blocked_lab.inc"


__device__ __forceinline__ uint32_t xcd_tile(uint32_t b, uint32_t tiles_per_xcd) { return (b & 7u) * tiles_per_xcd + (b >> 3); }

struct VertexOut { f3 p, vel, pred; };
template <bool kUniformBody, bool kTable = true>
__device__ __forceinline__ VertexOut pjb_vertex_update(f3 acc, float wsum, f3 prev, const DevParams& P, uint32_t v) {
    const float rw = __builtin_amdgcn_rcpf(wsum);
    f3 p = F3(acc.x * rw, acc.y * rw, acc.z * rw);
    bool grabbed = static_cast<int32_t>(v) == P.grab_local || static_cast<int32_t>(v) == P.grab_local2;
    if (grabbed) p = F3(P.grab[0], P.grab[1], P.grab[2]);
    body_grab_pick(P, v, grabbed, p.x, p.y, p.z);
    PolarBodyParams B = {P.gravity, P.friction, {P.lo[0], P.lo[1], P.lo[2]}, {P.hi[0], P.hi[1], P.hi[2]}};
    if constexpr (kTable) B = body_params_polar<kUniformBody>(P, v);
    p.x = fminf(fmaxf(p.x, B.lo[0]), B.hi[0]);
    p.y = fminf(fmaxf(p.y, B.lo[1]), B.hi[1]);
    p.z = fminf(fmaxf(p.z, B.lo[2]), B.hi[2]);
    if (p.y < 0.0f) {
        p.y = 0.0f;
        const float Fx = prev.x - p.x, Fz = prev.z - p.z;
        const float fr = fminf(1.0f, P.dt * B.friction);
        p.x = fmaf(Fx, fr, p.x);
        p.z = fmaf(Fz, fr, p.z);
    }
    if (any_colliders(P)) collide_particle_f32<true>(p.x, p.y, p.z, prev.x, prev.y, prev.z, P, v, !grabbed);
    const float dt = P.dt;
    const float rdt = __builtin_amdgcn_rcpf(dt);
    VertexOut o;
    o.p = p;
    const float gx = dt * 0.0f, gy = dt * B.gravity, gz = dt * 0.0f;
    o.vel = F3(fmaf(rdt, p.x - prev.x, gx), fmaf(rdt, p.y - prev.y, gy), fmaf(rdt, p.z - prev.z, gz));
    o.pred = F3(fmaf(dt, o.vel.x, p.x), fmaf(dt, o.vel.y, p.y), fmaf(dt, o.vel.z, p.z));
    return o;
}

constexpr uint32_t kTile = kBlockTile;

__device__ __forceinline__ f3 lean_fourth_corner(const f3 r[4]) {
    return F3(-((r[0].x + r[1].x) + r[2].x), -((r[0].y + r[1].y) + r[2].y), -((r[0].z + r[1].z) + r[2].z));
}
struct PJHaloWait { const PJPeerSync* w; const uint32_t* vflag; uint32_t* error; uint32_t timeout_ms; const float4* ghosts; };
constexpr int kModeCarried = 0, kModeConstantRest = 1, kModeLeanState = 2;
inline int blk_mode(const PJBlk& d) { return pjb_mode(d); }
struct PJPoll { uint32_t block, want; uint32_t* error; uint32_t timeout_ms; };
template <int kMode, bool kFused, bool kAlt = false, bool kHaloWait = false, bool kPoll = false>
__device__ __forceinline__ void pjb_tet_body(const PJBlk& d, uint32_t tile_first, uint32_t tile_count, uint32_t tiles_per_xcd TETSIM_DBG_PARAM,
                                             [[maybe_unused]] const PJHaloWait* hw = nullptr, const uint32_t stamp = 0u, [[maybe_unused]] const PJPoll* poll = nullptr) {
    __shared__ float4 s_pos[kTile];
    __shared__ float s_gx[4 * kTile];
    __shared__ float s_gy[4 * kTile];
    __shared__ float s_gz[4 * kTile];
    __shared__ uint2 s_ent[kTile];

    constexpr bool kLean = kMode == kModeConstantRest;
    uint32_t block_index = blockIdx.x;
    if constexpr (kPoll) block_index = poll->block;
    const uint32_t rel = xcd_tile(block_index, tiles_per_xcd);
    if (rel >= tile_count) return;
    const uint32_t b = tile_first + rel;
    const uint32_t tid = threadIdx.x;
    TETSIM_LAB_TILE_BEGIN();
    TETSIM_POLL_TILE(0);
    const uint32_t t0 = d.blk_tet_off[b], ntb = d.blk_tet_off[b + 1] - t0;
    const uint32_t v0 = d.blk_vert_off[b], nu = d.blk_vert_off[b + 1] - v0;

    const bool has_slot = tid < nu, has_tet = tid < ntb;
    const uint32_t slot = v0 + (has_slot ? tid : 0u), e = t0 + (has_tet ? tid : 0u);
    const uint32_t vid = static_cast<uint32_t>(d.blk_verts[slot]);
    const uint32_t range = has_slot ? d.lc_range[slot] : 0u;
    uint32_t src[8];
    uint32_t src8 = 0xffffffffu;
    [[maybe_unused]] uint32_t maxsrc = 0;
    if constexpr (kFused) {
        maxsrc = d.blk_maxsrc[b];
        const uint32_t* col = d.slot_src + slot;
#pragma unroll
        for (uint32_t j = 0; j < 8u; j++) src[j] = (j < maxsrc) ? col[static_cast<size_t>(j) * d.ns_pad] : 0xffffffffu;
        if (maxsrc > 8u) src8 = col[8ull * d.ns_pad];
    }
    const uchar4 li = d.tet_lidx[e];
    auto rec4 = [](const float4* a, uint32_t i) { if constexpr (kPoll) return load_coherent(a, i); else return a[i]; };
    float4 ra = make_float4(0.0f, 0.0f, 0.0f, 0.0f), rb = ra, rc = ra, q_old = make_float4(0.0f, 0.0f, 0.0f, 1.0f);
    auto load_record = [&]() {
        ra = rec4(d.rest_a, e); rb = rec4(d.rest_b, e);
        if constexpr (kMode == kModeLeanState) { if constexpr (kPoll) rc.x = load_coherent1(d.rest_c1, e); else rc.x = d.rest_c1[e]; }
        else { rc = rec4(d.rest_c, e); q_old = rec4(d.quat, e); }
    };
    bool record_late = false;
    if constexpr (kPoll) record_late = poll->want != 0u;
    if (!record_late) load_record();
    const float V = d.vol[e];
    const uint2 ent_row = d.lc_ent[e];
    float4 pos_stage;
    if constexpr (kFused) {
        f3 g[8];
#pragma unroll
        for (uint32_t j = 0; j < 8u; j++) {
            const float4 t = d.partial_prev[src[j] == 0xffffffffu ? 0u : src[j]];
            g[j] = src[j] == 0xffffffffu ? F3(0.0f, 0.0f, 0.0f) : xyz(t);
        }
        const float4 t8 = d.partial_prev[src8 == 0xffffffffu ? 0u : src8];
        const float4 prev4 = d.fin_in[vid];
        const float wsum = d.wsum[vid];
        f3 acc = F3(0.0f, 0.0f, 0.0f);
#pragma unroll
        for (uint32_t j = 0; j < 8u; j++) { acc.x += g[j].x; acc.y += g[j].y; acc.z += g[j].z; }
        if (src8 != 0xffffffffu) { acc.x += t8.x; acc.y += t8.y; acc.z += t8.z; }
        if (maxsrc > 9u) {
            const uint32_t* col = d.slot_src + slot;
            for (uint32_t j = 9u; j < maxsrc; j++) {
                const uint32_t sj = col[static_cast<size_t>(j) * d.ns_pad];
                const float4 tj = d.partial_prev[sj == 0xffffffffu ? 0u : sj];
                if (sj != 0xffffffffu) { acc.x += tj.x; acc.y += tj.y; acc.z += tj.z; }
            }
        }
        const VertexOut o = pjb_vertex_update<true>(acc, wsum, xyz(prev4), *d.params, vid);
        pos_stage = make_float4(o.pred.x, o.pred.y, o.pred.z, 0.0f);
        if (has_slot && ((range >> 15) & 1u)) {
            store_wt(d.fin_out, vid, make_float4(o.p.x, o.p.y, o.p.z, 0.0f));
            if (d.vel) store_wt(d.vel, vid, make_float4(o.vel.x, o.vel.y, o.vel.z, 0.0f));
        }
    } else if constexpr (kHaloWait) {
        if (tid < 64u) {
            const PJPeerSync& w = *hw->w;
            const uint32_t* word = tid == 0u ? hw->vflag : (tid <= w.n_wait ? w.wait[tid - 1u] : nullptr);
            bool pending = word != nullptr;
            const long long t0 = wall_clock64(), limit = 100000ll * hw->timeout_ms;
            while (true) {
                if (pending) pending = __hip_atomic_load(word, __ATOMIC_RELAXED, __HIP_MEMORY_SCOPE_SYSTEM) == 0u;
                if (__builtin_amdgcn_ballot_w64(pending) == 0ull) break;
                __builtin_amdgcn_s_sleep(16);
                if (limit && wall_clock64() - t0 > limit) { if (tid == 0) __hip_atomic_store(hw->error, 1u, __ATOMIC_RELAXED, __HIP_MEMORY_SCOPE_SYSTEM); break; }
            }
            if (w.delay_us && w.n_wait) { const long long d0 = wall_clock64(); while (wall_clock64() - d0 < 100ll * w.delay_us) __builtin_amdgcn_s_sleep(8); }
        }
        __syncthreads();
        const bool ghost = vid >= d.nv_owned;
        const float4 own = load_coherent(d.pos_pred, ghost ? 0u : vid), gh = load_coherent(hw->ghosts, ghost ? vid - d.nv_owned : 0u);
        pos_stage = ghost ? gh : own;
    } else if constexpr (kAlt) {
        const uint32_t g = vid - d.nv_owned;
        const float4* src = vid >= d.nv_owned ? (g < d.n_ghost1 ? d.ghost_alt + g : d.ghost2 + (g - d.n_ghost1)) : d.pos_pred + vid;
        pos_stage = *src;
    } else if constexpr (kPoll) {
        TETSIM_POLL_BEGIN();
        TETSIM_POLL_TILE(1);
        pos_stage = load_coherent(d.pos_pred, vid);
        if (poll->want != 0u) {
            bool pend = has_slot && __float_as_uint(pos_stage.w) != poll->want;
            if (__builtin_amdgcn_ballot_w64(pend) != 0ull) {
                const long long t0 = wall_clock64(), limit = 100000ll * poll->timeout_ms;
                do {
                    __builtin_amdgcn_s_sleep(TETSIM_POLL_SLEEP);
                    TETSIM_POLL_LOOK();
                    asm volatile("" ::: "memory");
                    if (pend) { pos_stage = load_coherent(d.pos_pred, vid); pend = __float_as_uint(pos_stage.w) != poll->want; }
                    if (limit && pend && wall_clock64() - t0 > limit) { __hip_atomic_store(poll->error, 1u, __ATOMIC_RELAXED, __HIP_MEMORY_SCOPE_SYSTEM); pend = false; }
                } while (__builtin_amdgcn_ballot_w64(pend) != 0ull);
            }
            TETSIM_POLL_TILE(2);
            __syncthreads();
            TETSIM_POLL_TILE(3);
            load_record();
        }
        TETSIM_POLL_TILE_SAVE();
    } else {
        pos_stage = d.pos_pred[vid];
    }
    if (has_slot) s_pos[tid] = pos_stage;
    if (has_tet) s_ent[tid] = ent_row;
    TETSIM_STAMP(1);
    __builtin_amdgcn_s_waitcnt(0x0F70);
    __syncthreads();
    TETSIM_STAMP(2);

    if (has_tet) {
        f3 cur[4], rest[4], goal[4];
        cur[0] = xyz(s_pos[li.x]); cur[1] = xyz(s_pos[li.y]); cur[2] = xyz(s_pos[li.z]); cur[3] = xyz(s_pos[li.w]);
        rest[0] = F3(ra.x, ra.y, ra.z); rest[1] = F3(ra.w, rb.x, rb.y);
        rest[2] = F3(rb.z, rb.w, rc.x); rest[3] = F3(rc.y, rc.z, rc.w);
        if constexpr (kMode == kModeLeanState) rest[3] = lean_fourth_corner(rest);
        float4 q_new;
        f3 cc;
        TETSIM_LAB_SOLVE_TET(cur, rest, q_old, q_new, goal, cc);
        TETSIM_STAMP(3);
        const f3 vcc = cc * V;
#pragma unroll
        for (int k = 0; k < 4; k++) {
            s_gx[k * kTile + tid] = fmaf(goal[k].x, V, vcc.x);
            s_gy[k * kTile + tid] = fmaf(goal[k].y, V, vcc.y);
            s_gz[k * kTile + tid] = fmaf(goal[k].z, V, vcc.z);
        }
        if constexpr (kMode != kModeLeanState) store_wt(d.quat, e, q_new);
        if (!kLean && TETSIM_DBG_STORE_REST) {
            store_wt(d.rest_a, e, make_float4(goal[0].x, goal[0].y, goal[0].z, goal[1].x));
            store_wt(d.rest_b, e, make_float4(goal[1].y, goal[1].z, goal[2].x, goal[2].y));
            if constexpr (kMode == kModeLeanState) store_wt1(d.rest_c1, e, goal[2].z);
            else store_wt(d.rest_c, e, make_float4(goal[2].z, goal[3].x, goal[3].y, goal[3].z));
        }
    }
    TETSIM_STAMP(4);
    if constexpr (kPoll) __builtin_amdgcn_s_waitcnt(0x0F70);
    __syncthreads();
    TETSIM_STAMP(5);

    if (tid < nu) {
        const uint32_t first = range & 0x7ffu, last = range >> 16;
        const uint16_t* ent = reinterpret_cast<const uint16_t*>(s_ent);
        auto plane = [](const float* base, uint32_t byte_off) { return *reinterpret_cast<const float*>(reinterpret_cast<const char*>(base) + byte_off); };
        float4 acc = make_float4(0.0f, 0.0f, 0.0f, 0.0f);
        uint32_t i = first;
        for (; i + 4u <= last; i += 4u) {
            uint32_t o[4];
            float gx[4], gy[4], gz[4];
#pragma unroll
            for (uint32_t j = 0; j < 4u; j++) o[j] = static_cast<uint32_t>(ent[i + j]) << 2;
#pragma unroll
            for (uint32_t j = 0; j < 4u; j++) { gx[j] = plane(s_gx, o[j]); gy[j] = plane(s_gy, o[j]); gz[j] = plane(s_gz, o[j]); }
#pragma unroll
            for (uint32_t j = 0; j < 4u; j++) { acc.x += gx[j]; acc.y += gy[j]; acc.z += gz[j]; }
        }
        for (; i < last; i++) {
            const uint32_t o = static_cast<uint32_t>(ent[i]) << 2;
            acc.x += plane(s_gx, o); acc.y += plane(s_gy, o); acc.z += plane(s_gz, o);
        }
        acc.w = __uint_as_float(stamp);
        store_wt(d.partial, v0 + tid, acc);
    }
    TETSIM_STAMP(6);
    TETSIM_POLL_TILE(4);
}

__global__ __launch_bounds__(kTile, 2) void pjb_tet_kernel(PJBlk d, uint32_t tile_first, uint32_t tile_count,
                                                        uint32_t tiles_per_xcd TETSIM_DBG_PARAM) {
    pjb_tet_body<kModeCarried, false>(d, tile_first, tile_count, tiles_per_xcd TETSIM_DBG_ARG);
}
__global__ __launch_bounds__(kTile, 2) void pjb_tet_kernel_constant_rest(PJBlk d, uint32_t tile_first, uint32_t tile_count,
                                                                      uint32_t tiles_per_xcd TETSIM_DBG_PARAM) {
    pjb_tet_body<kModeConstantRest, false>(d, tile_first, tile_count, tiles_per_xcd TETSIM_DBG_ARG);
// ... 212 lines not shown
    }
}
#define TETSIM_FRAME_KERNEL(name, mode, local)                                                                                         \
    __global__ __launch_bounds__(kTile, 2) void name(PJBlk d, uint32_t n, const int32_t* block_tile, float4* pbuf0, float4* pbuf1, uint32_t* err, \
                                                     uint32_t timeout_ms, DevParams pv, DevParams* pdev) {                             \
        if (blockIdx.x == 0u && threadIdx.x == 0u) store_params(pdev, pv);              \
        pjb_frame_body<mode, local>(d, pv, n, block_tile, pbuf0, pbuf1, err, timeout_ms);                                              \
    }
TETSIM_FRAME_KERNEL(pjb_frame_kernel, kModeCarried, false)
TETSIM_FRAME_KERNEL(pjb_frame_kernel_constant_rest, kModeConstantRest, false)
TETSIM_FRAME_KERNEL(pjb_frame_kernel_lean, kModeLeanState, false)
TETSIM_FRAME_KERNEL(pjb_frame_kernel_local, kModeCarried, true)
TETSIM_FRAME_KERNEL(pjb_frame_kernel_constant_rest_local, kModeConstantRest, true)
TETSIM_FRAME_KERNEL(pjb_frame_kernel_lean_local, kModeLeanState, true)
#undef TETSIM_FRAME_KERNEL
__global__ void pjb_probe_xcd_kernel(uint32_t* out) {
    if (threadIdx.x == 0) out[blockIdx.x] = __builtin_amdgcn_s_getreg(20 | (0 << 6) | (3 << 11));
}

__device__ __forceinline__ void await_done(const PJSync& y) {
    if (threadIdx.x == 0) {
        const long long t0 = wall_clock64(), limit = 100000ll * y.timeout_ms;
        while (__hip_atomic_load(y.flag, __ATOMIC_ACQUIRE, __HIP_MEMORY_SCOPE_AGENT) == 0u) {
            __builtin_amdgcn_s_sleep(4);
            if (limit && wall_clock64() - t0 > limit) {
                __hip_atomic_store(y.error, 1u, __ATOMIC_RELAXED, __HIP_MEMORY_SCOPE_SYSTEM);
                return;
            }
        }
        __hip_atomic_store(y.flag, 0u, __ATOMIC_RELAXED, __HIP_MEMORY_SCOPE_AGENT);
    }
}

template <bool kPeer = false, bool kCoherent = false>
__device__ __forceinline__ void pjb_vertex_body(const PJBlk& d, uint32_t first, uint32_t count, const PJPeer* peer = nullptr) {
    const uint32_t i = blockIdx.x * 64u + threadIdx.x;
    if (i >= count) return;
    const uint32_t v = first + i;

    float4 acc = make_float4(0.0f, 0.0f, 0.0f, 0.0f);
    const uint32_t* col = d.vp_ell + v;
    for (uint32_t j0 = 0; j0 < d.vp_cols; j0 += 8u) {
        uint32_t idx[8];
        float4 g[8];
#pragma unroll
        for (uint32_t j = 0; j < 8u; j++) idx[j] = (j0 + j < d.vp_cols) ? col[static_cast<size_t>(j0 + j) * d.nv_pad] : 0xffffffffu;
#pragma unroll
        for (uint32_t j = 0; j < 8u; j++) {
            if constexpr (kCoherent) { const float4 t = load_coherent(d.partial, idx[j] != 0xffffffffu ? idx[j] : 0u); g[j] = idx[j] != 0xffffffffu ? t : make_float4(0.0f, 0.0f, 0.0f, 0.0f); }
            else g[j] = idx[j] != 0xffffffffu ? d.partial[idx[j]] : make_float4(0.0f, 0.0f, 0.0f, 0.0f);
        }
#pragma unroll
        for (uint32_t j = 0; j < 8u; j++) { acc.x += g[j].x; acc.y += g[j].y; acc.z += g[j].z; }
        if (__all(idx[7] == 0xffffffffu)) break;
    }
    const VertexOut o = pjb_vertex_update<false>(xyz(acc), d.wsum[v], xyz(d.fin_in[v]), *d.params, v);
    store_wt(d.fin_out, v, make_float4(o.p.x, o.p.y, o.p.z, 0.0f));
    if (d.vel) store_wt(d.vel, v, make_float4(o.vel.x, o.vel.y, o.vel.z, 0.0f));
    store_wt(d.pos_pred, v, make_float4(o.pred.x, o.pred.y, o.pred.z, 0.0f));
    if constexpr (kPeer) {
        const float4 pred4 = make_float4(o.pred.x, o.pred.y, o.pred.z, 0.0f), fin4 = make_float4(o.p.x, o.p.y, o.p.z, 0.0f);
        const uint32_t* col = peer->slots + v;
        for (uint32_t c = 0; c < peer->cols; c++) {
            const uint32_t e = col[static_cast<size_t>(c) * peer->stride];
            for (uint32_t k = 0; k < peer->n; k++) {
                if (peer->ghost[k] && e != 0xffffffffu && (e >> 24) == k) store_wt(peer->ghost[k], e & 0xffffffu, pred4);
                if (peer->fin[k] && e != 0xffffffffu && (e >> 24) == k) store_wt(peer->fin[k], e & 0xffffffu, fin4);
            }
        }
        if (peer->slots2) {
            const uint32_t* col2 = peer->slots2 + v;
            for (uint32_t c = 0; c < peer->cols2; c++) {
                const uint32_t e = col2[static_cast<size_t>(c) * peer->stride];
                for (uint32_t k = 0; k < peer->n; k++)
                    if (peer->ghost2[k] && e != 0xffffffffu && (e >> 24) == k) store_wt(peer->ghost2[k], e & 0xffffffu, pred4);
            }
        }
    }
}

__global__ __launch_bounds__(64) void pjb_vertex_kernel(PJBlk d, uint32_t first, uint32_t count) { pjb_vertex_body(d, first, count); }

template <int kMode>
__global__ __launch_bounds__(kTile, 2) void pjb_call_kernel(PJBlk d, uint32_t n_sub, uint32_t tile_count, uint32_t tiles_per_xcd, const uint32_t* __restrict__ sched, uint32_t period,
                                                           uint32_t* err, uint32_t timeout_ms, DevParams pv, DevParams* pdev TETSIM_DBG_PARAM) {
    const uint32_t turn = blockIdx.x / period, entry = sched[blockIdx.x - turn * period];
    if (blockIdx.x == 0u && threadIdx.x == 0u) store_params(pdev, pv);
    const uint32_t back = (entry & kSchedWrapped) ? 1u : 0u, kind = entry >> 30, r = entry & kSchedIndexMask;
    if (kind == kSchedEmpty || turn < back || turn - back >= n_sub) return;
    const uint32_t sub = turn - back;
    const uint32_t stamp = (d.epoch ? d.epoch : pv.epoch) + sub + 1u;
    TETSIM_LAB_CALL_MARK(sub, n_sub);
    if (kind == kSchedTile) {
        const PJPoll poll = {r, sub ? stamp - 1u : 0u, err, timeout_ms};
        pjb_tet_body<kMode, false, false, false, true>(d, 0u, tile_count, tiles_per_xcd TETSIM_DBG_ARG, nullptr, stamp, &poll);
        return;
    }
    const uint32_t v = r * kTile + threadIdx.x;
    if (v >= d.nv_owned) return;
    TETSIM_POLL_BEGIN();
    TETSIM_POLL_PB(0);
    float4 acc = make_float4(0.0f, 0.0f, 0.0f, 0.0f);
    const uint32_t* col = d.vp_ell + v;
    const long long limit = 100000ll * timeout_ms;
    const float wsum = d.wsum[v];
    float4 prev = load_coherent(d.fin_in, v);
    for (uint32_t j0 = 0; j0 < d.vp_cols; j0 += 8u) {
        uint32_t idx[8];
        float4 g[8];
#pragma unroll
        for (uint32_t j = 0; j < 8u; j++) idx[j] = (j0 + j < d.vp_cols) ? col[static_cast<size_t>(j0 + j) * d.nv_pad] : 0xffffffffu;
        uint32_t pend = 0;
        TETSIM_POLL_PB_FIRST(j0);
#pragma unroll
        for (uint32_t j = 0; j < 8u; j++) {
            const float4 t = load_coherent(d.partial, idx[j] != 0xffffffffu ? idx[j] : 0u);
            g[j] = idx[j] != 0xffffffffu ? t : make_float4(0.0f, 0.0f, 0.0f, 0.0f);
            pend |= (idx[j] != 0xffffffffu && __float_as_uint(t.w) != stamp ? 1u : 0u) << j;
        }
        if (__builtin_amdgcn_ballot_w64(pend != 0u) != 0ull) {
            const long long t0 = wall_clock64();
            do {
                __builtin_amdgcn_s_sleep(TETSIM_POLL_SLEEP);
                TETSIM_POLL_LOOK();
                asm volatile("" ::: "memory");
#pragma unroll
                for (uint32_t j = 0; j < 8u; j++)
                    if ((pend >> j) & 1u) {
                        const float4 t = load_coherent(d.partial, idx[j]);
                        if (__float_as_uint(t.w) == stamp) { g[j] = t; pend &= ~(1u << j); }
                    }
                if (limit && pend != 0u && wall_clock64() - t0 > limit) {
                    __hip_atomic_store(err, 1u, __ATOMIC_RELAXED, __HIP_MEMORY_SCOPE_SYSTEM);
                    pend = 0u;
                }
            } while (__builtin_amdgcn_ballot_w64(pend != 0u) != 0ull);
        }
#pragma unroll
        for (uint32_t j = 0; j < 8u; j++) { acc.x += g[j].x; acc.y += g[j].y; acc.z += g[j].z; }
        if (__all(idx[7] == 0xffffffffu)) break;
    }
    TETSIM_POLL_PB(2);
    if (sub) {
        const long long t0 = wall_clock64();
        while (__float_as_uint(prev.w) != stamp - 1u) {
            __builtin_amdgcn_s_sleep(4);
            TETSIM_POLL_LOOK();
            asm volatile("" ::: "memory");
            prev = load_coherent(d.fin_in, v);
            if (limit && wall_clock64() - t0 > limit) { __hip_atomic_store(err, 1u, __ATOMIC_RELAXED, __HIP_MEMORY_SCOPE_SYSTEM); break; }
        }
    }
    TETSIM_POLL_PB(3);
    const VertexOut o = pv.body_params ? pjb_vertex_update<false, true>(xyz(acc), wsum, xyz(prev), pv, v) : pjb_vertex_update<false, false>(xyz(acc), wsum, xyz(prev), pv, v);
    store_wt(d.fin_out, v, make_float4(o.p.x, o.p.y, o.p.z, __uint_as_float(stamp)));
    if (d.vel && sub + 1u == n_sub) store_wt(d.vel, v, make_float4(o.vel.x, o.vel.y, o.vel.z, 0.0f));
    store_wt(d.pos_pred, v, make_float4(o.pred.x, o.pred.y, o.pred.z, __uint_as_float(stamp)));
    TETSIM_POLL_PB(4);
    TETSIM_POLL_PB_SAVE();
}
__global__ __launch_bounds__(64) void pjb_vertex_kernel_raise(PJBlk d, uint32_t first, uint32_t count, uint32_t* sig, uint32_t* clear) {
    clear_then_raise(clear, sig);
    pjb_vertex_body(d, first, count);
}
__global__ __launch_bounds__(64) void pjb_vertex_kernel_await(PJBlk d, uint32_t first, uint32_t count, uint32_t* flag, uint32_t* error, uint32_t timeout_ms) {
    if (threadIdx.x == 0) {
        const long long t0 = wall_clock64(), limit = 100000ll * timeout_ms;
        while (__hip_atomic_load(flag, __ATOMIC_RELAXED, __HIP_MEMORY_SCOPE_AGENT) == 0u) {
            __builtin_amdgcn_s_sleep(16);
            if (limit && wall_clock64() - t0 > limit) { __hip_atomic_store(error, 1u, __ATOMIC_RELAXED, __HIP_MEMORY_SCOPE_SYSTEM); break; }
        }
    }
    __builtin_amdgcn_wave_barrier();
    pjb_vertex_body<false, true>(d, first, count);
}
__global__ __launch_bounds__(64) void pjb_vertex_kernel_peer(PJBlk d, uint32_t first, uint32_t count, PJPeer peer, uint32_t* sig, PJClear clr) {
    if (blockIdx.x == 0 && threadIdx.x == 0) {
        for (uint32_t i = 0; i < clr.n; i++) __hip_atomic_store(clr.word[i], 0u, __ATOMIC_RELAXED, __HIP_MEMORY_SCOPE_SYSTEM);
        if (sig) __hip_atomic_store(sig, 1u, __ATOMIC_RELEASE, __HIP_MEMORY_SCOPE_AGENT);
    }
    pjb_vertex_body<true>(d, first, count, &peer);
}
__global__ void pjb_wait_peers_kernel(uint32_t* flag, uint32_t* error, uint32_t timeout_ms, PJPeerSync w) {
    PJSync y;
    y.flag = flag; y.error = error; y.timeout_ms = timeout_ms;
    const uint32_t t = threadIdx.x;
    if (t < w.n_raise) __hip_atomic_store(w.raise[t], 1u, __ATOMIC_RELEASE, __HIP_MEMORY_SCOPE_SYSTEM);
    if (y.flag) await_done(y);
    if (t < w.n_wait) {
        const long long t0 = wall_clock64(), limit = 100000ll * y.timeout_ms;
        while (__hip_atomic_load(w.wait[t], __ATOMIC_ACQUIRE, __HIP_MEMORY_SCOPE_SYSTEM) == 0u) {
            __builtin_amdgcn_s_sleep(4);
            if (limit && wall_clock64() - t0 > limit) { __hip_atomic_store(y.error, 1u, __ATOMIC_RELAXED, __HIP_MEMORY_SCOPE_SYSTEM); break; }
        }
        __hip_atomic_store(w.wait[t], 0u, __ATOMIC_RELAXED, __HIP_MEMORY_SCOPE_SYSTEM);
        if (w.delay_us) { const long long d0 = wall_clock64(); while (wall_clock64() - d0 < 100ll * w.delay_us) __builtin_amdgcn_s_sleep(8); }
    }
}
__global__ void pjb_wait_kernel(uint32_t* flag, uint32_t* error, uint32_t timeout_ms) {
    PJSync y;
    y.flag = flag; y.error = error; y.timeout_ms = timeout_ms;
    await_done(y);
}
__global__ void pjb_signal_kernel(uint32_t* flag, uint32_t* clear) {
    if (threadIdx.x == 0) {
        if (clear) __hip_atomic_store(clear, 0u, __ATOMIC_RELAXED, __HIP_MEMORY_SCOPE_AGENT);
        __hip_atomic_store(flag, 1u, __ATOMIC_RELEASE, __HIP_MEMORY_SCOPE_AGENT);
    }
}

__global__ __launch_bounds__(256) void pjb_recover_quat_kernel(const float4* __restrict__ r0a, const float4* __restrict__ r0b, const float4* __restrict__ r0c,
                                                              const float4* __restrict__ ca, const float4* __restrict__ cb, const float* __restrict__ cc1,
                                                              float4* __restrict__ quat, uint32_t nt) {
    const uint32_t e = blockIdx.x * 256u + threadIdx.x;
    if (e >= nt) return;
    const float4 a0 = r0a[e], b0 = r0b[e], c0 = r0c[e], a = ca[e], b = cb[e];
    const float c1 = cc1[e];
    const float4 qp = quat[e];
    const double s[3][3] = {{a0.x, a0.y, a0.z}, {a0.w, b0.x, b0.y}, {b0.z, b0.w, c0.x}};
    const double c[3][3] = {{a.x, a.y, a.z}, {a.w, b.x, b.y}, {b.z, b.w, c1}};
    auto cr = [](const double* u, const double* v, double* o) { o[0] = u[1] * v[2] - u[2] * v[1]; o[1] = u[2] * v[0] - u[0] * v[2]; o[2] = u[0] * v[1] - u[1] * v[0]; };
    double inv[3][3];
    cr(s[1], s[2], inv[0]); cr(s[2], s[0], inv[1]); cr(s[0], s[1], inv[2]);
    const double det = s[0][0] * inv[0][0] + s[0][1] * inv[0][1] + s[0][2] * inv[0][2];
    if (!(fabs(det) > 1.0e-300)) return;
    const double rd = 1.0 / det;
    double R[3][3];
    for (int i = 0; i < 3; i++)
        for (int j = 0; j < 3; j++) R[i][j] = (c[0][i] * inv[0][j] + c[1][i] * inv[1][j] + c[2][i] * inv[2][j]) * rd;
    const double tr = R[0][0] + R[1][1] + R[2][2];
    double x, y, z, w;
    if (tr > 0.0) { w = tr + 1.0; x = R[2][1] - R[1][2]; y = R[0][2] - R[2][0]; z = R[1][0] - R[0][1]; }
    else if (R[0][0] >= R[1][1] && R[0][0] >= R[2][2]) { x = 1.0 + R[0][0] - R[1][1] - R[2][2]; y = R[0][1] + R[1][0]; z = R[0][2] + R[2][0]; w = R[2][1] - R[1][2]; }
    else if (R[1][1] >= R[2][2]) { y = 1.0 + R[1][1] - R[0][0] - R[2][2]; x = R[0][1] + R[1][0]; z = R[1][2] + R[2][1]; w = R[0][2] - R[2][0]; }
    else { z = 1.0 + R[2][2] - R[0][0] - R[1][1]; x = R[0][2] + R[2][0]; y = R[1][2] + R[2][1]; w = R[1][0] - R[0][1]; }
    const double n2 = x * x + y * y + z * z + w * w;
    if (!(n2 > 0.0) || !(n2 < 1.0e300)) return;
    double k = 1.0 / sqrt(n2);
    if (x * qp.x + y * qp.y + z * qp.z + w * qp.w < 0.0) k = -k;
    quat[e] = make_float4(static_cast<float>(x * k), static_cast<float>(y * k), static_cast<float>(z * k), static_cast<float>(w * k));
}

__global__ __launch_bounds__(256) void pjb_repredict_kernel(PJBlk d) {
    const uint32_t v = blockIdx.x * 256u + threadIdx.x;
    if (v >= d.nv_owned) return;
    const f3 pred = xyz(d.pos_final[v]) + xyz(d.vel[v]) * d.params->dt;
    d.pos_pred[v] = make_float4(pred.x, pred.y, pred.z, 0.0f);
}

}

void pjb_launch_tet(hipStream_t s, const PJBlk& d, uint32_t tile_first, uint32_t tile_count, hipEvent_t e0, hipEvent_t e1, uint32_t* raise_word,
                    uint32_t* clear_word) {
    if (tile_count == 0) return;
    if (raise_word || clear_word) return launch_tet_x(s, d, tile_first, tile_count, TetRaise{raise_word, clear_word}, e0, e1);
    const uint32_t per_xcd = (tile_count + 7u) / 8u;
    const int mode = blk_mode(d);
    auto* kernel = mode == kModeConstantRest ? pjb_tet_kernel_constant_rest : mode == kModeLeanState ? pjb_tet_kernel_lean : pjb_tet_kernel;
    if (e0) hipExtLaunchKernelGGL(kernel, dim3(per_xcd * 8u), dim3(kTile), 0, s, e0, e1, 0, d, tile_first, tile_count, per_xcd TETSIM_DBG_LAUNCH);
    else hipLaunchKernelGGL(kernel, dim3(per_xcd * 8u), dim3(kTile), 0, s, d, tile_first, tile_count, per_xcd TETSIM_DBG_LAUNCH);
}
void pjb_launch_call(hipStream_t s, const PJBlk& d, const PJCallSched& sched, uint32_t n, uint32_t* err, uint32_t timeout_ms, const DevParams& params, DevParams* params_dev) {
    if (d.nb == 0 || n == 0 || sched.period == 0) return;
    const uint32_t per_xcd = (d.nb + 7u) / 8u;
    const int mode = blk_mode(d);
    auto* kernel = mode == kModeConstantRest ? pjb_call_kernel<kModeConstantRest> : mode == kModeLeanState ? pjb_call_kernel<kModeLeanState> : pjb_call_kernel<kModeCarried>;
    hipLaunchKernelGGL(kernel, dim3(sched.period * n + sched.tail), dim3(kTile), 0, s, d, n, d.nb, per_xcd, sched.entry, sched.period, err, timeout_ms, params, params_dev TETSIM_DBG_LAUNCH);
}
void pjb_launch_tet_fused(hipStream_t s, const PJBlk& d, hipEvent_t e0, hipEvent_t e1) { launch_tet_x(s, d, 0u, d.nb, TetFused{0u}, e0, e1); }
void pjb_launch_frame(hipStream_t s, const PJBlk& d, uint32_t n, const int32_t* block_tile, uint32_t blocks, bool local, float4* pbuf0, float4* pbuf1,
                      uint32_t* err, uint32_t timeout_ms, const DevParams& params, DevParams* params_dev, hipEvent_t e0, hipEvent_t e1) {
    if (d.nb == 0 || n == 0 || blocks == 0) return;
    const int mode = blk_mode(d);
    auto* kernel = local ? (mode == kModeConstantRest ? pjb_frame_kernel_constant_rest_local : mode == kModeLeanState ? pjb_frame_kernel_lean_local : pjb_frame_kernel_local)
                         : (mode == kModeConstantRest ? pjb_frame_kernel_constant_rest : mode == kModeLeanState ? pjb_frame_kernel_lean : pjb_frame_kernel);
    if (e0) hipExtLaunchKernelGGL(kernel, dim3(blocks), dim3(kTile), 0, s, e0, e1, 0, d, n, block_tile, pbuf0, pbuf1, err, timeout_ms, params, params_dev);
    else hipLaunchKernelGGL(kernel, dim3(blocks), dim3(kTile), 0, s, d, n, block_tile, pbuf0, pbuf1, err, timeout_ms, params, params_dev);
}
uint32_t pjb_frame_capacity(int mode, uint32_t* compute_units) {
    int per_cu = 0, dev = 0;
    hipDeviceProp_t prop;
    if (hipGetDevice(&dev) != hipSuccess || hipGetDeviceProperties(&prop, dev) != hipSuccess) return 0;
    int per_cu_any = 0;
    auto* k_local = mode == kModeConstantRest ? pjb_frame_kernel_constant_rest_local : mode == kModeLeanState ? pjb_frame_kernel_lean_local : pjb_frame_kernel_local;
    auto* k_any = mode == kModeConstantRest ? pjb_frame_kernel_constant_rest : mode == kModeLeanState ? pjb_frame_kernel_lean : pjb_frame_kernel;
    const hipError_t e = hipOccupancyMaxActiveBlocksPerMultiprocessor(&per_cu, k_local, static_cast<int>(kTile), 0);
    const hipError_t e2 = hipOccupancyMaxActiveBlocksPerMultiprocessor(&per_cu_any, k_any, static_cast<int>(kTile), 0);
    if (e != hipSuccess || e2 != hipSuccess || per_cu <= 0 || per_cu_any <= 0) return 0;
    per_cu = std::min(per_cu, per_cu_any);
    if (compute_units) *compute_units = static_cast<uint32_t>(prop.multiProcessorCount);
    return static_cast<uint32_t>(per_cu);
}
void pjb_wait_capacity(int mode, uint32_t* vertex_waves, uint32_t* hwait_blocks) {
    *vertex_waves = 0; *hwait_blocks = 0;
    int per_cu_v = 0, per_cu_t = 0, dev = 0;
    hipDeviceProp_t prop;
    if (hipGetDevice(&dev) != hipSuccess || hipGetDeviceProperties(&prop, dev) != hipSuccess) return;
    if (hipOccupancyMaxActiveBlocksPerMultiprocessor(&per_cu_v, pjb_vertex_kernel_await, 64, 0) != hipSuccess) per_cu_v = 0;
    auto* k_hwait = mode == kModeConstantRest ? pjb_tet_kernel_x<kModeConstantRest, TetHwait> : mode == kModeLeanState ? pjb_tet_kernel_x<kModeLeanState, TetHwait> : pjb_tet_kernel_x<kModeCarried, TetHwait>;
    const hipError_t e = hipOccupancyMaxActiveBlocksPerMultiprocessor(&per_cu_t, k_hwait, static_cast<int>(kTile), 0);
    if (e != hipSuccess) per_cu_t = 0;
    const uint32_t cus = static_cast<uint32_t>(std::max(prop.multiProcessorCount, 0));
    *vertex_waves = static_cast<uint32_t>(std::max(per_cu_v, 0)) * cus / 2u;
    *hwait_blocks = static_cast<uint32_t>(std::max(per_cu_t, 0)) * cus / 4u;
}
uint32_t pjb_probe_xcd(hipStream_t s, uint32_t blocks) {
    uint32_t* d_out = nullptr;
    if (blocks < 16u || hipMalloc(reinterpret_cast<void**>(&d_out), blocks * sizeof(uint32_t)) != hipSuccess) return 0;
    std::vector<uint32_t> out(blocks, 0xffffffffu);
    hipLaunchKernelGGL(pjb_probe_xcd_kernel, dim3(blocks), dim3(64), 0, s, d_out);
    const bool ok = hipStreamSynchronize(s) == hipSuccess && hipMemcpy(out.data(), d_out, blocks * sizeof(uint32_t), hipMemcpyDeviceToHost) == hipSuccess;
    (void)hipFree(d_out);
    if (!ok) return 0;
    for (uint32_t i = 0; i < 8u; i++)
        for (uint32_t j = 0; j < i; j++) if (out[i] == out[j]) return 0;
    for (uint32_t i = 8u; i < blocks; i++) if (out[i] != out[i & 7u]) return 0;
    return 8;
}
void pjb_launch_wait_peers(hipStream_t s, const PJSync& y, const PJPeerSync& w) { hipLaunchKernelGGL(pjb_wait_peers_kernel, dim3(1), dim3(64), 0, s, y.flag, y.error, y.timeout_ms, w); }
void pjb_launch_vertex_peer(hipStream_t s, const PJBlk& d, uint32_t first, uint32_t count, const PJPeer& peer, uint32_t* raise_word, const PJClear& clr) {
    if (count == 0) return;
    hipLaunchKernelGGL(pjb_vertex_kernel_peer, dim3((count + 63u) / 64u), dim3(64), 0, s, d, first, count, peer, raise_word, clr);
}
void pjb_launch_tet_hwait(hipStream_t s, const PJBlk& d, uint32_t tile_first, uint32_t tile_count, const PJSync& yv, const PJPeerSync& w, const float4* ghosts) {
    launch_tet_x(s, d, tile_first, tile_count, TetHwait{w, yv.flag, yv.error, yv.timeout_ms, ghosts});
}
void pjb_launch_tet_alt(hipStream_t s, const PJBlk& d, uint32_t tile_first, uint32_t tile_count) { launch_tet_x(s, d, tile_first, tile_count, TetAlt{0u}); }
void pjb_launch_wait(hipStream_t s, const PJSync& y) { hipLaunchKernelGGL(pjb_wait_kernel, dim3(1), dim3(64), 0, s, y.flag, y.error, y.timeout_ms); }
void pjb_launch_signal(hipStream_t s, const PJSync& y, uint32_t* clear_word) { hipLaunchKernelGGL(pjb_signal_kernel, dim3(1), dim3(64), 0, s, y.flag, clear_word); }
void pjb_launch_vertex_await(hipStream_t s, const PJBlk& d, uint32_t first, uint32_t count, const PJSync& y, hipEvent_t e0, hipEvent_t e1) {
    if (count == 0) return;
    if (e0) hipExtLaunchKernelGGL(pjb_vertex_kernel_await, dim3((count + 63u) / 64u), dim3(64), 0, s, e0, e1, 0, d, first, count, y.flag, y.error, y.timeout_ms);
    else hipLaunchKernelGGL(pjb_vertex_kernel_await, dim3((count + 63u) / 64u), dim3(64), 0, s, d, first, count, y.flag, y.error, y.timeout_ms);
}
void pjb_launch_vertex(hipStream_t s, const PJBlk& d, uint32_t first, uint32_t count, hipEvent_t e0, hipEvent_t e1, uint32_t* raise_word, uint32_t* clear_word) {
    if (count == 0) return;
    if (raise_word || clear_word) {
        if (e0) hipExtLaunchKernelGGL(pjb_vertex_kernel_raise, dim3((count + 63u) / 64u), dim3(64), 0, s, e0, e1, 0, d, first, count, raise_word, clear_word);
        else hipLaunchKernelGGL(pjb_vertex_kernel_raise, dim3((count + 63u) / 64u), dim3(64), 0, s, d, first, count, raise_word, clear_word);
        return;
    }
    if (e0) hipExtLaunchKernelGGL(pjb_vertex_kernel, dim3((count + 63u) / 64u), dim3(64), 0, s, e0, e1, 0, d, first, count);
    else hipLaunchKernelGGL(pjb_vertex_kernel, dim3((count + 63u) / 64u), dim3(64), 0, s, d, first, count);
}
void pjb_launch_recover_quats(hipStream_t s, const PJBlk& d, const float4* rest0_a, const float4* rest0_b, const float4* rest0_c) {
    if (d.nt == 0 || !d.lean_state) return;
    hipLaunchKernelGGL(pjb_recover_quat_kernel, dim3((d.nt + 255u) / 256u), dim3(256), 0, s, rest0_a, rest0_b, rest0_c, d.rest_a, d.rest_b, d.rest_c1, d.quat, d.nt);
}
void pjb_launch_repredict(hipStream_t s, const PJBlk& d) {
    if (d.nv_owned == 0) return;
    hipLaunchKernelGGL(pjb_repredict_kernel, dim3((d.nv_owned + 255u) / 256u), dim3(256), 0, s, d);
// ... 4 lines not shown
```

### tetsim_amd/csrc/tetsim_api.hip

```cpp
#include <mutex>

#include "body.h"

using namespace tetsim;

namespace tetsim {

namespace {
thread_local std::string g_create_error;
}
HostProf g_hostprof;

int fail(tetsim_body* h, int code, const std::string& msg) {
    if (h) h->err = msg; else g_create_error = msg;
    return code;
}
const char* create_error() { return g_create_error.c_str(); }
int group_result(tetsim_body* const* hs, uint32_t count, int rc) {
    if (rc == TETSIM_OK || !hs) return rc;
    for (uint32_t i = 0; i < count; i++)
        if (hs[i] && !hs[i]->err.empty()) { g_create_error = "partition " + std::to_string(i) + ": " + hs[i]->err; return rc; }
    if (g_create_error.empty()) g_create_error = "bad argument";
    return rc;
}
void group_begin(tetsim_body* const* hs, uint32_t count) {
    g_create_error.clear();
    if (hs) for (uint32_t i = 0; i < count; i++) if (hs[i]) hs[i]->err.clear();
}

void ref_grab_texels(int32_t grab_id, uint32_t num_elems, uint32_t num_particles, int32_t out[2]) {
    out[0] = out[1] = -1;
    if (grab_id < 0) return;
    const int R = static_cast<int>(std::ceil(std::sqrt(static_cast<double>(num_elems))));
    const float Rf = static_cast<float>(R), Rm1 = Rf - 1.0f;
    int n = 0;
    for (int py = 0; py < R && n < 2; py++) {
        const float uy = (static_cast<float>(py) + 0.5f) / Rf;
        const int row = static_cast<int>((uy * Rm1) * Rf);
        const int a = grab_id - row;
        if (a < 0 || a >= R) continue;
        for (int px = std::max(0, a - 1); px <= std::min(R - 1, a + 1) && n < 2; px++) {
            const float ux = (static_cast<float>(px) + 0.5f) / Rf;
            const int idx = static_cast<int>(ux * Rm1) + row;
            const int64_t particle = static_cast<int64_t>(py) * R + px;
            if (static_cast<float>(idx) == static_cast<float>(grab_id) && particle < static_cast<int64_t>(num_particles)) out[n++] = static_cast<int32_t>(particle);
        }
    }
}

void fill_params(const tetsim_body* h, double dt, const TetSimParams& p, DevParams* o) {
    std::memset(o, 0, sizeof(*o));
    o->dt = static_cast<float>(dt);
    o->gravity = static_cast<float>(p.gravity);
    o->friction = static_cast<float>(p.friction);
    const bool fixed = h->opt.solver == TETSIM_SOLVER_POLAR_JACOBI && (h->opt.flags & TETSIM_FLAG_REF_FIXED_BOUNDS);
    for (int c = 0; c < 3; c++) {
        o->lo[c] = fixed ? ref_fixed_lo(c) : static_cast<float>(p.worldBounds[c]);
        o->hi[c] = fixed ? ref_fixed_hi(c) : static_cast<float>(p.worldBounds[3 + c]);
        o->d_lo[c] = p.worldBounds[c];
        o->d_hi[c] = p.worldBounds[3 + c];
        o->grab[c] = h->grab_pos[c];
    }
    auto to_device = [&](int32_t global) -> int32_t {
        if (global < 0) return -1;
        int32_t a = -1;
        if (!h->partitioned) a = global;
        else if (static_cast<size_t>(global) < h->g2l_owned.size()) a = h->g2l_owned[global];
        if (a < 0 && static_cast<size_t>(global) < h->g2l_ghost1.size()) a = h->g2l_ghost1[global];
        if (a < 0) return -1;
        return h->api2dev.empty() ? a : static_cast<int32_t>(h->api2dev[a]);
    };
    o->grab_local = o->grab_local2 = -1;
    if (h->grab_global >= 0) {
        if (h->opt.solver == TETSIM_SOLVER_POLAR_JACOBI && (h->opt.flags & TETSIM_FLAG_REF_GRAB_TEXEL)) {
            o->grab_local = to_device(h->grab_ref[0]);
            o->grab_local2 = to_device(h->grab_ref[1]);
        } else o->grab_local = to_device(h->grab_global);
    }
    o->body_grabs = h->body_grabs_on ? 1u : 0u;
    o->grab_body = h->d_grab_body;
    o->grab_rows = h->d_grab_rows;
    o->body_colliders = h->body_colliders_on ? 1u : 0u;
    o->bcol_count = h->d_bcol_count;
    o->bcol_f = h->d_bcol_f;
    o->bcol_d = h->d_bcol_d;
    o->body_params = h->body_params_on ? 1u : 0u;
    o->bp_f = h->d_bp_f;
    o->bp_d = h->d_bp_d;
    o->tet_body = h->d_tet_body;
    o->epoch = h->frame_epoch;
    static const int32_t poll_delay = [] { const char* e = lab_env("TETSIM_QUAD_POLL_DELAY"); return e ? atoi(e) : kQuadPollDelay; }();
    o->poll_delay = poll_delay;
    o->d_dt = dt;
    o->d_gravity = p.gravity;
    o->d_friction = p.friction;
    o->d_dev_compliance = p.devCompliance;
    o->d_vol_compliance = p.volCompliance;
    o->n_colliders = h->n_colliders;
    for (uint32_t k = 0; k < h->n_colliders; k++) { o->col[k] = h->col[k]; o->d_col[k] = h->d_col[k]; }
}

int next_epoch_block(tetsim_body* h) {
    if (h->frame_epoch >= 0xfffe0000u) {
        if (h->partial_b && h->partial_slots) {
            HIPCHK(h, hipMemsetAsync(h->blk.partial, 0, h->partial_slots * sizeof(float4), h->stream));
            HIPCHK(h, hipMemsetAsync(h->partial_b, 0, h->partial_slots * sizeof(float4), h->stream));
        }
        if (h->nh_one_launch) HIPCHK(h, hipMemsetAsync(h->nh_sweep1.exchange, 0, static_cast<size_t>(h->nh.nv) * sizeof(float4), h->stream));
        h->frame_epoch = 1u;
    }
    h->frame_epoch += 65536u;
    return 0;
}

constexpr uint32_t kDirectLaunchTets = 150000u;

int push_params(tetsim_body* h, double dt, const TetSimParams* params, bool reuse_ok) {
    if (!params) return fail(h, TETSIM_EINVAL, "params is null");
    if (!(dt > 0.0) || !std::isfinite(dt)) return fail(h, TETSIM_EINVAL, "dt must be a positive finite number");
    HIPCHK(h, hipSetDevice(h->opt.device));
    h->final_ghosts_fresh = false;
    h->quat_stale = true;
    if (reuse_ok && h->params_known && !h->comm_stream && !h->partitioned) {
        DevParams now;
        fill_params(h, dt, *params, &now);
        now.epoch = h->params_on_device.epoch;
        if (std::memcmp(&now, &h->params_on_device, sizeof now) == 0) { h->fork_needed = true; return 0; }
    }
    if (int rc = next_epoch_block(h)) return rc;
    h->epoch_block_fresh = reuse_ok;
    fill_params(h, dt, *params, &h->params_on_device);
    h->params_known = true;
    util_launch_set_params(h->stream, h->d_params, h->params_on_device);
    if (h->comm_stream && h->d_params_halo) util_launch_set_params(h->comm_stream, h->d_params_halo, h->params_on_device);
    const hipError_t le = hipGetLastError();
    if (le != hipSuccess) return fail(h, TETSIM_EHIP, std::string("kernel launch: ") + hipGetErrorString(le));
    h->fork_needed = true;
    return 0;
}

int stage_params(tetsim_body* h, double dt, const TetSimParams* params) {
    if (!params) return fail(h, TETSIM_EINVAL, "params is null");
    if (!(dt > 0.0) || !std::isfinite(dt)) return fail(h, TETSIM_EINVAL, "dt must be a positive finite number");
    HIPCHK(h, hipSetDevice(h->opt.device));
    h->final_ghosts_fresh = false;
    h->quat_stale = true;
    if (int rc = next_epoch_block(h)) return rc;
    h->epoch_block_fresh = false;
    fill_params(h, dt, *params, &h->params_on_device);
    h->params_known = true;
    h->fork_needed = true;
    return 0;
}

int params_for_launch(tetsim_body* h, double dt, const TetSimParams* params) {
    const bool repredict = h->opt.solver == TETSIM_SOLVER_POLAR_JACOBI && !h->pred_any_dt && static_cast<float>(dt) != h->dt_pred;
    if (int rc = repredict ? push_params(h, dt, params) : stage_params(h, dt, params)) return rc;
    return ensure_prediction(h, dt);
}

void pj_tet(tetsim_body* h, hipEvent_t e0, hipEvent_t e1) {
    if (h->quad) pjq_launch_tet(h->stream, h->blk, e0, e1);
    else if (h->blocked) pjb_launch_tet(h->stream, h->blk, 0, h->blk.nb, e0, e1);
    else h->fast ? pj_launch_tet_fast(h->stream, h->pj, e0, e1) : pj_launch_tet_precise(h->stream, h->pj, e0, e1);
}
void pj_vertex(tetsim_body* h, uint32_t first, uint32_t count, hipEvent_t e0, hipEvent_t e1) {
    if (h->quad) pjq_launch_vertex(h->stream, h->blk, e0, e1);
    else if (h->blocked) pjb_launch_vertex(h->stream, h->blk, first, count, e0, e1);
    else h->fast ? pj_launch_vertex_fast(h->stream, h->pj, first, count, e0, e1) : pj_launch_vertex_precise(h->stream, h->pj, first, count, e0, e1);
}
void pj_fused_substep(tetsim_body* h, bool first, bool last, hipEvent_t* e) {
    PJBlk k = h->blk;
    if (first) { h->fuse_step = 0; h->fin_in_b = false; }
    const uint32_t s = h->fuse_step++;
    float4* const pbuf[2] = {h->blk.partial, h->partial_b};
    float4* const fbuf[2] = {h->pj.pos_final, h->pos_final_b};
    k.partial = pbuf[s & 1u];
    if (s == 0) pjb_launch_tet(h->stream, k, 0, k.nb, e ? e[0] : nullptr, e ? e[1] : nullptr);
    else {
        k.partial_prev = pbuf[(s - 1u) & 1u];
        k.fin_in = fbuf[h->fin_in_b ? 1 : 0];
        k.fin_out = fbuf[h->fin_in_b ? 0 : 1];
        { PJBlk kf = k; kf.vel = nullptr; pjb_launch_tet_fused(h->stream, kf, e ? e[0] : nullptr, e ? e[1] : nullptr); }
        h->fin_in_b = !h->fin_in_b;
    }
    if (last) {
        k.fin_in = fbuf[h->fin_in_b ? 1 : 0];
        k.fin_out = h->pj.pos_final;
        pjb_launch_vertex(h->stream, k, 0, h->pj.nv_owned, e ? e[2] : nullptr, e ? e[3] : nullptr);
        h->fin_in_b = false;
// ... 606 lines not shown
```

### tetsim_amd/csrc/tetsim_create.hip

```cpp
#include "body.h"

namespace tetsim {

int create_polar(tetsim_body* h, const float* verts, uint32_t nv, const int32_t* tets, uint32_t nt) {
    const TetSimOptions& o = h->opt;
    const bool ref_table = (o.flags & TETSIM_FLAG_REF_SLOT_TABLE) != 0;
    std::vector<int32_t> ltets;
    std::vector<int32_t> l2g_v, l2g_t;
    uint32_t nvl = nv, nvo = nv, nvb = 0, ntl = nt;
    h->partitioned = o.part_count > 1;
    h->deep = h->partitioned && (o.flags & TETSIM_FLAG_DEEP_GHOSTS);
    {
        const char* sy = getenv("TETSIM_HALO_SYNC");
        const char* gr = getenv("TETSIM_HALO_GRAPH");
        h->halo_use_flags = !(sy && sy[0] == 'e');
        h->halo_use_graph = !(gr && gr[0] == '0');
    }
    if ((o.flags & TETSIM_FLAG_DEEP_GHOSTS) && !(h->partitioned && h->fast && !(o.flags & TETSIM_FLAG_GATHER_FORMULATION)))
        return fail(h, TETSIM_EINVAL, "TETSIM_FLAG_DEEP_GHOSTS needs a partitioned POLAR_JACOBI body in the blocked FAST formulation");
    uint32_t nvg1 = 0;
    if (h->partitioned) {
        std::string e = build_partition(tets, nt, nv, o.part_count, o.part_index, o.vert_owner, &h->part, h->deep ? 2 : 1);
        if (!e.empty()) return fail(h, TETSIM_EINVAL, e);
        if (h->deep) {
// ... 164 lines not shown
        if ((rc = dev_alloc(h, &bvo, B.blk_vert_off.size()))) return rc;
        if ((rc = dev_alloc(h, &bv, nslots))) return rc;
        if (ntl >= kStoreWtMaxIndex || nslots >= kStoreWtMaxIndex || nvl >= kStoreWtMaxIndex)
            return fail(h, TETSIM_EINVAL, "body too large for one handle (2^27 tets / particles / partial sums: 32-bit store offsets, dev_store.h); partition it");
        if ((rc = dev_alloc(h, &lidx, ntl))) return rc;
        if ((rc = dev_alloc(h, &k.rest_a, ntl))) return rc;
        if ((rc = dev_alloc(h, &k.rest_b, ntl))) return rc;
        if (lean_state) {
            if ((rc = dev_alloc(h, &k.rest_c1, ntl))) return rc;
            if ((rc = dev_alloc(h, &h->rest0_a, ntl))) return rc;
            if ((rc = dev_alloc(h, &h->rest0_b, ntl))) return rc;
            if ((rc = dev_alloc(h, &h->rest0_c, ntl))) return rc;
        } else if ((rc = dev_alloc(h, &k.rest_c, ntl))) return rc;
        if ((rc = dev_alloc(h, &vol, ntl))) return rc;
        if ((rc = dev_alloc(h, &k.quat, ntl))) return rc;
        if ((rc = dev_alloc(h, &lcr, nslots))) return rc;
        if ((rc = dev_alloc(h, &lce, ntl))) return rc;
        if ((rc = dev_alloc(h, &k.partial, nslots))) return rc;
        if ((rc = dev_alloc(h, &vpe, B.vp_ell.size()))) return rc;
        std::vector<float4> ra(ntl), rb(ntl), rcv(ntl), quat(ntl, make_float4(0, 0, 0, 1));
        std::vector<float> volh(ntl);
        std::vector<uchar4> lidxh(ntl);
        std::vector<uint2> lceh(ntl);
        for (uint32_t i = 0; i < ntl; i++) {
            const uint32_t lt = static_cast<uint32_t>(B.tet_perm[i]);
            const int32_t* c = &ltets[4 * lt];
            const float4 p0 = pos[c[0]], p1 = pos[c[1]], p2 = pos[c[2]], p3 = pos[c[3]];
            float4 r0 = p0, r1 = p1, r2 = p2, r3 = p3;
            {
                const float cx = (((p0.x + p1.x) + p2.x) + p3.x) * 0.25f, cy = (((p0.y + p1.y) + p2.y) + p3.y) * 0.25f,
                            cz = (((p0.z + p1.z) + p2.z) + p3.z) * 0.25f;
                r0 = make_float4(p0.x - cx, p0.y - cy, p0.z - cz, 0.0f); r1 = make_float4(p1.x - cx, p1.y - cy, p1.z - cz, 0.0f);
                r2 = make_float4(p2.x - cx, p2.y - cy, p2.z - cz, 0.0f); r3 = make_float4(p3.x - cx, p3.y - cy, p3.z - cz, 0.0f);
            }
            ra[i] = make_float4(r0.x, r0.y, r0.z, r1.x);
            rb[i] = make_float4(r1.y, r1.z, r2.x, r2.y);
            rcv[i] = make_float4(r2.z, r3.x, r3.y, r3.z);
            volh[i] = rest_weight(lt);
            lidxh[i] = make_uchar4(B.tet_lidx[4ull * i], B.tet_lidx[4ull * i + 1], B.tet_lidx[4ull * i + 2], B.tet_lidx[4ull * i + 3]);
            const uint16_t* en = &B.lc_ent[4ull * i];
            lceh[i] = make_uint2(en[0] | (static_cast<uint32_t>(en[1]) << 16), en[2] | (static_cast<uint32_t>(en[3]) << 16));
        }
        std::vector<float> wsum(std::max<size_t>(B.nv_pad, 1), 0.0f);
        {
            std::vector<float> slot_w(nslots, 0.0f);
            for (uint32_t b = 0; b < B.num_blocks; b++) {
                const uint32_t t0 = B.blk_tet_off[b], v0 = B.blk_vert_off[b], nu = B.blk_vert_off[b + 1] - v0;
                for (uint32_t u = 0; u < nu; u++) {
                    const uint32_t first = B.lc_range[v0 + u] & 0x7ffu, last = B.lc_range[v0 + u] >> 16;
                    float w = 0.0f;
                    for (uint32_t i = first; i < last; i++) w += volh[t0 + (B.lc_ent[4ull * t0 + i] % B.tile)];
                    slot_w[v0 + u] = w;
                }
            }
            for (uint32_t v = 0; v < nvo + nvg1; v++) {
                float w = 0.0f;
                for (uint32_t j = 0; j < B.max_partials; j++) {
                    const uint32_t idx = B.vp_ell[static_cast<size_t>(j) * B.nv_pad + v];
                    if (idx != 0xffffffffu) w += slot_w[idx];
                }
                wsum[v] = w;
            }
        }
        float* dws;
        if ((rc = dev_alloc(h, &dws, wsum.size()))) return rc;
        if ((rc = upload(h, dws, wsum))) return rc;
        k.wsum = dws;
        static const bool allow_fused = [] { const char* e = getenv("TETSIM_FUSED_PARTICLE_PASS"); return !(e && e[0] == '0'); }();
        static const bool force_fused = [] { const char* e = getenv("TETSIM_FUSED_PARTICLE_PASS"); return e && e[0] == '1'; }();
        h->fused = allow_fused && !h->quad && !h->partitioned && nvo == nvl && B.every_owned_particle_has_a_partial && ntl > 0 &&
                   (B.num_blocks < 2048u || force_fused);
        k.fin_in = d.pos_final; k.fin_out = d.pos_final;
        h->info.fused_particle_pass = h->fused ? 1u : 0u;
        {
            const char* e = getenv("TETSIM_PJ_ONE_LAUNCH");
            h->pj_one_launch = !(e && e[0] == '0') && !h->fused && !h->quad && !h->partitioned && nvo == nvl && ntl > 0 && B.num_blocks > 0;
            if (h->pj_one_launch) {
                h->info.fused_particle_pass = 5u;
                if ((rc = dev_alloc(h, &h->d_substep_err, 1))) return rc;
                HIPCHK(h, hipMemset(h->d_substep_err, 0, sizeof(uint32_t)));
                const char* lag_env = getenv("TETSIM_PJ_CALL_LAG");
                const uint32_t lag = lag_env ? static_cast<uint32_t>(std::min<unsigned long>(strtoul(lag_env, nullptr, 10), 1ul << 24)) : kPJCallLagDefault;
                CallSchedule S;
                build_call_schedule(B.blk_verts.data(), B.blk_vert_off.data(), B.num_blocks, B.vp_ell.data(), B.vp_cols, B.nv_pad, nvo, lag, &S);
                if (S.fell_back) fprintf(stderr, "[tetsim] TETSIM_PJ_CALL_LAG=%u ignored (%s): the call runs in the plain order\n", lag, S.why.c_str());
                uint32_t* dsched;
                if ((rc = dev_alloc(h, &dsched, S.entry.size()))) return rc;
                if ((rc = upload(h, dsched, S.entry))) return rc;
                h->call_sched.entry = dsched; h->call_sched.period = S.period; h->call_sched.tail = S.tail;
            }
        }
        if (h->fused || h->quad) {
            uint32_t *dsrc, *dmax;
            if ((rc = dev_alloc(h, &dsrc, B.slot_src.size()))) return rc;
            if ((rc = dev_alloc(h, &dmax, B.blk_maxsrc.size()))) return rc;
            if ((rc = dev_alloc(h, &h->partial_b, nslots))) return rc;
            if ((rc = upload(h, dsrc, B.slot_src))) return rc;
            if ((rc = upload(h, dmax, B.blk_maxsrc))) return rc;
            HIPCHK(h, hipMemset(h->partial_b, 0, std::max<size_t>(nslots, 1) * sizeof(float4)));
            h->partial_slots = nslots;
            if (h->fused) {
                if ((rc = dev_alloc(h, &h->pos_final_b, nvl))) return rc;
                if ((rc = upload(h, h->pos_final_b, pos))) return rc;
            }
            k.slot_src = dsrc; k.blk_maxsrc = dmax; k.ns_pad = B.ns_pad;
            static const bool allow_frame = [] { const char* e = getenv("TETSIM_FRAME_KERNEL"); return !(e && e[0] == '0'); }();
            uint32_t cus = 0;
            const uint32_t per_cu = !allow_frame ? 0u : h->quad ? pjq_frame_capacity(&cus) : pjb_frame_capacity(pjb_mode(k), &cus);
            const uint32_t nbk = B.num_blocks;
            std::vector<int32_t> block_tile;
            const uint32_t slots = per_cu * cus, exclusive_max = slots - slots / 10u;
            if (per_cu != 0u && nbk != 0u && nbk <= (h->partitioned ? slots / 2u : exclusive_max)) {
                h->frame_exclusive = nbk > slots / 2u;
                static const bool allow_local = [] { const char* e = lab_env("TETSIM_FRAME_LOCAL"); return !(e && e[0] == '0'); }();
                static int xcd_rule[64] = {};
                int& rule = xcd_rule[o.device & 63];
                if (allow_local && rule == 0) rule = pjb_probe_xcd(h->stream, 256) == 8u ? 1 : 2;
                std::vector<std::vector<uint32_t>> groups(bodies);
                for (uint32_t b = 0; b < nbk; b++) {
                    const uint32_t body = batch ? body_of_tet(h, static_cast<uint32_t>(B.tet_perm[B.blk_tet_off[b]])) : 0u;
                    groups[std::min(body, bodies - 1u)].push_back(b);
                }
                const uint32_t budget = per_cu * (cus / 8u) / 2u;
                std::vector<uint32_t> by_size(bodies);
                for (uint32_t g = 0; g < bodies; g++) by_size[g] = g;
                std::stable_sort(by_size.begin(), by_size.end(), [&](uint32_t a, uint32_t c) { return groups[a].size() > groups[c].size(); });
                std::vector<std::vector<uint32_t>> on_xcd(8);
                bool local = allow_local && rule == 1 && cus % 8u == 0u;
                for (uint32_t g : by_size) {
                    if (!local) break;
                    uint32_t best = 0;
                    for (uint32_t x = 1; x < 8u; x++) if (on_xcd[x].size() < on_xcd[best].size()) best = x;
                    if (on_xcd[best].size() + groups[g].size() > budget) { local = false; break; }
                    on_xcd[best].insert(on_xcd[best].end(), groups[g].begin(), groups[g].end());
                }
                if (!local) {
                    for (auto& v : on_xcd) v.clear();
                    for (uint32_t b = 0; b < nbk; b++) on_xcd[b & 7u].push_back(b);
                }
                uint32_t most = 0;
                for (auto& v : on_xcd) most = std::max<uint32_t>(most, static_cast<uint32_t>(v.size()));
                block_tile.assign(8ull * most, -1);
                for (uint32_t x = 0; x < 8u; x++)
                    for (uint32_t j = 0; j < on_xcd[x].size(); j++) block_tile[8ull * j + x] = static_cast<int32_t>(on_xcd[x][j]);
                h->frame = true;
                frame_turn_enter(h);
                h->frame_local = local;
                h->frame_blocks = static_cast<uint32_t>(block_tile.size());
            }
            if (h->frame) {
                if ((rc = dev_alloc(h, &h->d_block_tile, block_tile.size()))) return rc;
                if ((rc = upload(h, h->d_block_tile, block_tile))) return rc;
                if ((rc = dev_alloc(h, &h->d_frame_err, 1))) return rc;
                HIPCHK(h, hipMemset(h->d_frame_err, 0, sizeof(uint32_t)));
                h->info.fused_particle_pass = h->quad ? 3u : 2u;
            }
        }
        if ((rc = upload(h, bto, B.blk_tet_off))) return rc;
        if ((rc = upload(h, bvo, B.blk_vert_off))) return rc;
        if ((rc = upload(h, bv, B.blk_verts))) return rc;
        if ((rc = upload(h, lidx, lidxh))) return rc;
        if ((rc = upload(h, k.rest_a, ra))) return rc;
        if ((rc = upload(h, k.rest_b, rb))) return rc;
        if (lean_state) {
            std::vector<float> rc1(ntl);
            for (uint32_t i = 0; i < ntl; i++) rc1[i] = rcv[i].x;
            if ((rc = upload(h, k.rest_c1, rc1))) return rc;
            if ((rc = upload(h, h->rest0_a, ra))) return rc;
            if ((rc = upload(h, h->rest0_b, rb))) return rc;
            if ((rc = upload(h, h->rest0_c, rcv))) return rc;
        } else if ((rc = upload(h, k.rest_c, rcv))) return rc;
        if ((rc = upload(h, vol, volh))) return rc;
// ... 326 lines not shown
```

### tetsim_amd/csrc/tetsim_host.cpp

```cpp
#include "body.h"

using namespace tetsim;

namespace tetsim {
void build_strain_table(const float* verts, uint32_t nv, const int32_t* tets, uint32_t nt, double density, StrainRec* out) {
    std::vector<float> inv_mass(nv), irp(9ull * nt), irv(nt);
    prep_rest(verts, nv, tets, nt, density, inv_mass.data(), irp.data(), irv.data());
    for (uint32_t e = 0; e < nt; e++) {
        StrainRec& r = out[e];
        const int32_t* t = &tets[4ull * e];
        const double v0 = rest_volume(verts, t);
        bool finite = true;
        for (uint32_t k = 0; k < 9u; k++) {
            r.b[k] = irp[9ull * e + k];
            finite = finite && std::isfinite(r.b[k]);
        }
        for (uint32_t k = 0; k < 4u; k++) r.id[k] = t[k];
        r.degenerate = (v0 == 0.0 || !finite) ? 1u : 0u;
        r.v0_abs = std::fabs(v0);
    }
}
void build_pose_table(const float* verts, uint32_t nv, const int32_t* tets, uint32_t nt, const uint32_t* first_vert, uint32_t bodies, double density,
                      PoseRec* out, double* centres) {
    for (uint32_t i = 0; i < nv; i++) out[i].m = 0.0;
// ... 35 lines not shown
    if (!e.empty()) return fail(nullptr, TETSIM_EINVAL, e);
    *out = new tetsim_mesh_file{m};
    return TETSIM_OK;
}
int tetsim_mesh_arrays(tetsim_mesh m, TetSimMeshArrays* out) {
    if (!m || !out) return fail(nullptr, TETSIM_EINVAL, "null argument");
    *out = mesh_arrays(m->m);
    return TETSIM_OK;
}
int tetsim_mesh_close(tetsim_mesh m) {
    if (!m) return TETSIM_OK;
    mesh_close(m->m);
    delete m;
    return TETSIM_OK;
}

int tetsim_prep_levels(const int32_t* tets, uint32_t nt, uint32_t nv, int32_t* level, uint32_t* num_levels) {
    if ((nt && (!tets || !level)) || !num_levels) return TETSIM_EINVAL;
    std::string e = validate_mesh(reinterpret_cast<const float*>(tets), nv ? nv : 1, tets, nt, false);
    if (!e.empty()) return fail(nullptr, TETSIM_EINVAL, e);
    *num_levels = prep_levels(tets, nt, nv, level);
    return 0;
}
int tetsim_prep_colours(const int32_t* tets, uint32_t nt, uint32_t nv, int32_t* colour, uint32_t* num_colours) {
    if ((nt && (!tets || !colour)) || !num_colours) return TETSIM_EINVAL;
    std::string e = validate_mesh(reinterpret_cast<const float*>(tets), nv ? nv : 1, tets, nt, false);
    if (!e.empty()) return fail(nullptr, TETSIM_EINVAL, e);
    *num_colours = prep_colours(tets, nt, nv, colour);
    return 0;
}
int tetsim_prep_clusters(const int32_t* tets, uint32_t nt, uint32_t nv, int32_t* order, int32_t* launch, int32_t* lane, int32_t* step,
                         uint32_t* num_launches, uint32_t* num_clusters) {
    if ((nt && (!tets || !order || !launch || !lane || !step)) || !num_launches) return TETSIM_EINVAL;
    std::string e = validate_mesh(reinterpret_cast<const float*>(tets), nv ? nv : 1, tets, nt, false);
    if (!e.empty()) return fail(nullptr, TETSIM_EINVAL, e);
    const ClusterPlan P = prep_clusters(tets, nt, nv);
    for (uint32_t i = 0; i < nt; i++) order[i] = P.pre[i];
    const uint32_t nl = static_cast<uint32_t>(P.launch_off.size() - 1);
    for (uint32_t l = 0; l < nl; l++)
        for (uint32_t j = P.step_off[l]; j < P.step_off[l + 1]; j++)
            for (uint32_t i = 0; i < P.step_count[j]; i++) {
                const uint32_t pos = P.exec_pos[P.step_first[j] + i];
                launch[pos] = static_cast<int32_t>(l);
                lane[pos] = static_cast<int32_t>(i);
                step[pos] = static_cast<int32_t>(j - P.step_off[l]);
            }
    *num_launches = nl;
    if (num_clusters) *num_clusters = P.num_clusters;
    return 0;
}
int tetsim_prep_tiles(const float* verts, uint32_t nv, const int32_t* tets, uint32_t nt, const uint32_t* body_first_tet,
                      const uint32_t* body_first_vert, uint32_t bodies, int32_t* tile_tets, uint32_t* tile_off, uint8_t* corner_slot,
                      uint32_t* num_tiles) {
    if (!num_tiles) return TETSIM_EINVAL;
    std::string e = validate_mesh(verts, nv, tets, nt, false);
    if (!e.empty()) return fail(nullptr, TETSIM_EINVAL, e);
    if (body_first_tet && body_first_vert && bodies) {
        if (body_first_tet[0] != 0 || body_first_vert[0] != 0 || body_first_tet[bodies] != nt || body_first_vert[bodies] != nv)
            return fail(nullptr, TETSIM_EINVAL, "body ranges must cover the whole mesh");
        for (uint32_t b = 0; b < bodies; b++) {
            if (body_first_tet[b] > body_first_tet[b + 1] || body_first_vert[b] >= body_first_vert[b + 1]) return fail(nullptr, TETSIM_EINVAL, "body ranges must ascend");
            for (uint64_t i = 4ull * body_first_tet[b]; i < 4ull * body_first_tet[b + 1]; i++)
                if (static_cast<uint32_t>(tets[i]) < body_first_vert[b] || static_cast<uint32_t>(tets[i]) >= body_first_vert[b + 1])
                    return fail(nullptr, TETSIM_EINVAL, "a tet references a particle of another body");
        }
    }
    const Incidence inc = build_incidence(tets, nt, nv, false, false);
    BlockPlan B;
    build_blocks(verts, tets, nt, nv, nv, inc, &B, body_first_tet, body_first_vert, bodies);
    *num_tiles = B.num_blocks;
    if (tile_tets) std::copy(B.tet_perm.begin(), B.tet_perm.end(), tile_tets);
    if (tile_off) std::copy(B.blk_tet_off.begin(), B.blk_tet_off.end(), tile_off);
    if (corner_slot) std::copy(B.tet_lidx.begin(), B.tet_lidx.end(), corner_slot);
    return 0;
}
int tetsim_prep_slot_table(const int32_t* tets, uint32_t nt, uint32_t nv, int32_t ref_quirk, int32_t* slots, uint32_t* dropped) {
    if ((nt && !tets) || !slots) return TETSIM_EINVAL;
    std::string e = validate_mesh(reinterpret_cast<const float*>(tets), nv ? nv : 1, tets, nt, false);
    if (!e.empty()) return fail(nullptr, TETSIM_EINVAL, e);
    const uint32_t d = prep_slot_table(tets, nt, nv, ref_quirk != 0, slots);
    if (dropped) *dropped = d;
    return 0;
}
int tetsim_prep_call_tiles(const float* verts, uint32_t nv, const int32_t* tets, uint32_t nt, uint32_t sizes[4], uint32_t* blk_vert_off,
                           int32_t* blk_verts, uint32_t* vp_ell) {
    if (!sizes) return TETSIM_EINVAL;
    std::string e = validate_mesh(verts, nv, tets, nt, false);
    if (!e.empty()) return fail(nullptr, TETSIM_EINVAL, e);
    const std::vector<uint32_t> order = morton_vertex_order(verts, nv, 0, nv);
    std::vector<int32_t> to_dev(nv), ltets(4ull * nt);
    std::vector<float> lverts(3ull * nv);
    for (uint32_t i = 0; i < nv; i++) {
        to_dev[order[i]] = static_cast<int32_t>(i);
        for (int c = 0; c < 3; c++) lverts[3ull * i + c] = verts[3ull * order[i] + c];
    }
    for (uint64_t i = 0; i < 4ull * nt; i++) ltets[i] = to_dev[tets[i]];
    const Incidence inc = build_incidence(ltets.data(), nt, nv, false, false);
    BlockPlan B;
    build_blocks(lverts.data(), ltets.data(), nt, nv, nv, inc, &B);
    sizes[0] = B.num_blocks; sizes[1] = static_cast<uint32_t>(B.blk_verts.size()); sizes[2] = B.vp_cols; sizes[3] = B.nv_pad;
    if (blk_vert_off) std::copy(B.blk_vert_off.begin(), B.blk_vert_off.end(), blk_vert_off);
    if (blk_verts) std::copy(B.blk_verts.begin(), B.blk_verts.end(), blk_verts);
    if (vp_ell) std::copy(B.vp_ell.begin(), B.vp_ell.begin() + static_cast<std::ptrdiff_t>(static_cast<size_t>(B.vp_cols) * B.nv_pad), vp_ell);
    return 0;
}
int tetsim_prep_call_schedule(const int32_t* blk_verts, const uint32_t* blk_vert_off, uint32_t nb, const uint32_t* vp_ell, uint32_t vp_cols,
                              uint32_t nv_pad, uint32_t nv_owned, uint32_t lag, uint32_t* entry, uint32_t capacity, uint32_t* period,
                              uint32_t* tail, int32_t* fell_back) {
    if (!blk_vert_off || (nb && !blk_verts) || (vp_cols && !vp_ell) || !period || !tail) return TETSIM_EINVAL;
    if (nv_owned > nv_pad && vp_cols) return fail(nullptr, TETSIM_EINVAL, "tetsim_prep_call_schedule: nv_owned exceeds the column stride of vp_ell");
    CallSchedule S;
    build_call_schedule(blk_verts, blk_vert_off, nb, vp_ell, vp_cols, nv_pad, nv_owned, lag, &S);
    *period = S.period; *tail = S.tail;
    if (fell_back) *fell_back = S.fell_back ? 1 : 0;
    if (S.fell_back) fail(nullptr, TETSIM_OK, "tetsim_prep_call_schedule: " + S.why + " -- the plain order instead");
    if (entry) {
        if (capacity < S.period) return fail(nullptr, TETSIM_EINVAL, "tetsim_prep_call_schedule: the table needs " + std::to_string(S.period) + " entries");
        std::copy(S.entry.begin(), S.entry.end(), entry);
    }
    return 0;
}
int tetsim_prep_check_call_schedule(const int32_t* blk_verts, const uint32_t* blk_vert_off, uint32_t nb, const uint32_t* vp_ell, uint32_t vp_cols,
                                    uint32_t nv_pad, uint32_t nv_owned, const uint32_t* entry, uint32_t period, uint32_t tail) {
    if (!blk_vert_off || (nb && !blk_verts) || (vp_cols && !vp_ell) || !entry) return TETSIM_EINVAL;
    const std::string bad = check_call_schedule(blk_verts, blk_vert_off, nb, vp_ell, vp_cols, nv_pad, nv_owned, entry, period, tail);
    return bad.empty() ? 0 : fail(nullptr, TETSIM_EINVAL, "call schedule: " + bad);
}
int tetsim_prep_ref_grab_texels(int32_t grab_id, uint32_t num_elems, uint32_t num_particles, int32_t out[2]) {
    if (!out) return TETSIM_EINVAL;
    ref_grab_texels(grab_id, num_elems, num_particles, out);
    return 0;
}
int tetsim_prep_boundary_surface(const float* verts, const int32_t* tets, uint32_t nt, uint32_t nv, float* vis_verts, int32_t* tri_ids,
                                 uint32_t* nrows, uint32_t* ntri) {
    if ((nt && !tets) || !nrows || !ntri || (!vis_verts != !tri_ids)) return fail(nullptr, TETSIM_EINVAL, "tetsim_prep_boundary_surface: null argument");
    if (nt && nv == 0) return fail(nullptr, TETSIM_EINVAL, "tetsim_prep_boundary_surface: tets without particles (nv == 0)");
    std::string e = validate_mesh(reinterpret_cast<const float*>(tets), nv ? nv : 1, tets, nt, false);
    if (!e.empty()) return fail(nullptr, TETSIM_EINVAL, e);
    if (nt > (1u << 24)) return fail(nullptr, TETSIM_EINVAL, "tetsim_prep_boundary_surface: a tet id above 2^24 does not fit the f32 row format");
    static const int kFace[4][3] = {{1, 2, 3}, {0, 3, 2}, {0, 1, 3}, {0, 2, 1}};
    struct Face { int32_t key[3]; uint32_t tet, face; };
    std::vector<Face> faces(4ull * nt);
    for (uint32_t t = 0; t < nt; t++)
        for (uint32_t k = 0; k < 4; k++) {
            Face& f = faces[4ull * t + k];
            for (int j = 0; j < 3; j++) f.key[j] = tets[4 * t + kFace[k][j]];
            std::sort(f.key, f.key + 3);
            f.tet = t; f.face = k;
        }
    std::sort(faces.begin(), faces.end(), [](const Face& a, const Face& b) {
        return std::lexicographical_compare(a.key, a.key + 3, b.key, b.key + 3) || (std::equal(a.key, a.key + 3, b.key) && (a.tet < b.tet || (a.tet == b.tet && a.face < b.face)));
    });
    std::vector<uint64_t> boundary;
    for (size_t i = 0; i < faces.size();) {
        size_t j = i + 1;
        while (j < faces.size() && std::equal(faces[i].key, faces[i].key + 3, faces[j].key)) j++;
        if (j - i == 1) boundary.push_back(4ull * faces[i].tet + faces[i].face);
        i = j;
    }
    std::sort(boundary.begin(), boundary.end());
    std::vector<int32_t> row(nv, -1);
    for (uint64_t b : boundary)
        for (int j = 0; j < 3; j++) row[tets[4 * (b >> 2) + kFace[b & 3][j]]] = 0;
    uint32_t rows = 0;
    for (uint32_t v = 0; v < nv; v++)
        if (row[v] == 0) row[v] = static_cast<int32_t>(rows++);
    *nrows = rows;
    *ntri = static_cast<uint32_t>(boundary.size());
    if (!vis_verts) return 0;
    std::vector<uint8_t> done(rows, 0);
    for (uint32_t t = 0; t < nt; t++)
        for (int k = 0; k < 4; k++) {
            const int32_t r = row[tets[4 * t + k]];
            if (r < 0 || done[r]) continue;
            done[r] = 1;
            vis_verts[4 * r] = static_cast<float>(t);
            for (int j = 0; j < 3; j++) vis_verts[4 * r + 1 + j] = j == k ? 1.0f : 0.0f;
        }
    for (size_t i = 0; i < boundary.size(); i++) {
        const uint32_t t = static_cast<uint32_t>(boundary[i] >> 2), k = static_cast<uint32_t>(boundary[i] & 3);
        bool flip = false;
        if (verts) {
            const int32_t* c = tets + 4 * t;
            double m[3][3];
            for (int a = 0; a < 3; a++)
                for (int x = 0; x < 3; x++) m[a][x] = static_cast<double>(verts[3 * c[a + 1] + x]) - static_cast<double>(verts[3 * c[0] + x]);
            const double det = m[0][0] * (m[1][1] * m[2][2] - m[1][2] * m[2][1]) - m[0][1] * (m[1][0] * m[2][2] - m[1][2] * m[2][0]) +
                               m[0][2] * (m[1][0] * m[2][1] - m[1][1] * m[2][0]);
            flip = det < 0.0;
        }
        const int32_t a = row[tets[4 * t + kFace[k][0]]], b = row[tets[4 * t + kFace[k][1]]], c2 = row[tets[4 * t + kFace[k][2]]];
        tri_ids[3 * i] = a;
        tri_ids[3 * i + 1] = flip ? c2 : b;
        tri_ids[3 * i + 2] = flip ? b : c2;
    }
    return 0;
}
int tetsim_prep_rest(const float* verts, uint32_t nv, const int32_t* tets, uint32_t nt, double density, float* inv_mass, float* inv_rest_pose, float* inv_rest_volume) {
    if (!inv_mass || (nt && (!inv_rest_pose || !inv_rest_volume))) return TETSIM_EINVAL;
    std::string e = validate_mesh(verts, nv, tets, nt, false);
    if (!e.empty()) return fail(nullptr, TETSIM_EINVAL, e);
    prep_rest(verts, nv, tets, nt, density, inv_mass, inv_rest_pose, inv_rest_volume);
    return 0;
}

int tetsim_prep_strain_table(const float* verts, uint32_t nv, const int32_t* tets, uint32_t nt, double density, void* records_out) {
    if (nt && !records_out) return TETSIM_EINVAL;
    std::string e = validate_mesh(verts, nv, tets, nt, false);
// ... 147 lines not shown
```

Baseline: 35160 M tet-solves/s.

## Widen one-launch call dispatch entries to carry tile offsets; add optional push staging

Each one-launch schedule entry now becomes a 4-word record that carries the tile's tet offset, vertex offset and packed counts. The persistent kernel can then read its tile bounds from a single 16-byte load instead of separate dependent reads of blk_tet_off and blk_vert_off. An optional compile-time push mode (off by default) polls a per-slot staging buffer rather than gathering positions by vertex id. The schedule table grows fourfold, and a stricter host-side check validates the slot lists and the wide entries.

```diff
diff --git a/include/tetsim.h b/include/tetsim.h
--- a/include/tetsim.h
+++ b/include/tetsim.h
@@ -321,6 +321,15 @@
 int tetsim_prep_check_call_schedule(const int32_t *blk_verts, const uint32_t *blk_vert_off, uint32_t nb, const uint32_t *vp_ell,
                                     uint32_t vp_cols, uint32_t nv_pad, uint32_t nv_owned, const uint32_t *entry, uint32_t period,
                                     uint32_t tail);
+int tetsim_prep_call_tile_tets(const float *verts, uint32_t nv, const int32_t *tets, uint32_t nt, uint32_t *blk_tet_off,
+                               uint32_t capacity);
+int tetsim_prep_call_schedule_wide(const int32_t *blk_verts, const uint32_t *blk_vert_off, const uint32_t *blk_tet_off, uint32_t nb,
+                                   const uint32_t *vp_ell, uint32_t vp_cols, uint32_t nv_pad, uint32_t nv_owned, uint32_t lag,
+                                   uint32_t *wide , uint32_t capacity, uint32_t *period, uint32_t *tail,
+                                   int32_t *fell_back);
+int tetsim_prep_check_call_schedule_wide(const int32_t *blk_verts, const uint32_t *blk_vert_off, const uint32_t *blk_tet_off,
+                                         uint32_t nb, const uint32_t *vp_ell, uint32_t vp_cols, uint32_t nv_pad, uint32_t nv_owned,
+                                         const uint32_t *wide, uint32_t period, uint32_t tail);
 int tetsim_prep_ref_grab_texels(int32_t grab_id, uint32_t num_elems, uint32_t num_particles, int32_t out[2]);
 int tetsim_prep_boundary_surface(const float *verts ,
                                  const int32_t *tets, uint32_t nt, uint32_t nv,
diff --git a/tetsim_amd/_capi.py b/tetsim_amd/_capi.py
--- a/tetsim_amd/_capi.py
+++ b/tetsim_amd/_capi.py
@@ -146,6 +146,7 @@
     "tetsim_set_body_params", "tetsim_set_body_params_device",
     "tetsim_place_bodies_device", "tetsim_place_bodies",
     "tetsim_mesh_write", "tetsim_mesh_open", "tetsim_mesh_arrays", "tetsim_mesh_close", "tetsim_create_from_file",
+    "tetsim_prep_call_tile_tets", "tetsim_prep_call_schedule_wide", "tetsim_prep_check_call_schedule_wide",
 ]
 
 OPTIONAL_SYMBOLS = ("tetsim_set_colliders", "tetsim_raycast_visual", "tetsim_start_grab_ray", "tetsim_read_visual_bounding_sphere", "tetsim_prep_boundary_surface",
@@ -158,7 +159,8 @@
                     "tetsim_set_body_colliders", "tetsim_set_body_colliders_device",
                     "tetsim_set_body_params", "tetsim_set_body_params_device",
                     "tetsim_place_bodies_device", "tetsim_place_bodies",
-                    "tetsim_body_poses_device", "tetsim_read_body_poses", "tetsim_prep_pose_table")
+                    "tetsim_body_poses_device", "tetsim_read_body_poses", "tetsim_prep_pose_table",
+                    "tetsim_prep_call_tile_tets", "tetsim_prep_call_schedule_wide", "tetsim_prep_check_call_schedule_wide")
 
 _lib = None
 
@@ -292,6 +294,10 @@
     L.tetsim_prep_call_tiles.argtypes = [fp, u32, ip, u32, up, up, ip, up]
     L.tetsim_prep_call_schedule.argtypes = [ip, up, u32, up, u32, u32, u32, u32, up, u32, up, up, ip]
     L.tetsim_prep_check_call_schedule.argtypes = [ip, up, u32, up, u32, u32, u32, up, u32, u32]
+    if hasattr(L, "tetsim_prep_call_schedule_wide"):
+        L.tetsim_prep_call_tile_tets.argtypes = [fp, u32, ip, u32, up, u32]
+        L.tetsim_prep_call_schedule_wide.argtypes = [ip, up, up, u32, up, u32, u32, u32, u32, up, u32, up, up, ip]
+        L.tetsim_prep_check_call_schedule_wide.argtypes = [ip, up, up, u32, up, u32, u32, u32, up, u32, u32]
     L.tetsim_prep_ref_grab_texels.argtypes = [i32, u32, u32, ip]
     L.tetsim_prep_rest.argtypes = [fp, u32, ip, u32, dbl, fp, fp, fp]
     L.tetsim_prep_partition.argtypes = [fp, u32, ip, u32, i32, ip]
diff --git a/tetsim_amd/csrc/body.h b/tetsim_amd/csrc/body.h
--- a/tetsim_amd/csrc/body.h
+++ b/tetsim_amd/csrc/body.h
@@ -211,6 +211,7 @@
     bool pj_one_launch = false;
     uint32_t* d_substep_err = nullptr;
     PJCallSched call_sched;
+    size_t stage_slots = 0;
     float4 *rest0_a = nullptr, *rest0_b = nullptr, *rest0_c = nullptr;
     bool quat_stale = false;
     bool frame = false;
diff --git a/tetsim_amd/csrc/dev_common.h b/tetsim_amd/csrc/dev_common.h
--- a/tetsim_amd/csrc/dev_common.h
+++ b/tetsim_amd/csrc/dev_common.h
@@ -129,6 +129,7 @@
     const uint32_t* lc_range = nullptr;
     const uint2* lc_ent = nullptr;
     float4* partial = nullptr;
+    float4* stage = nullptr;
     const float* wsum = nullptr;
     const uint32_t* vp_ell = nullptr;
     uint32_t vp_cols = 0, nv_pad = 0;
@@ -168,7 +169,7 @@
     const DevParams* params = nullptr;
 };
 constexpr uint32_t max_grid_blocks(uint32_t threads) { return 0xffffffffu / threads; }
-struct PJCallSched { const uint32_t* entry = nullptr; uint32_t period = 0, tail = 0; };
+struct PJCallSched { const uint4* entry = nullptr; uint32_t period = 0, tail = 0; };
 constexpr uint32_t pjb_call_chunk(uint32_t period, uint32_t tail, uint32_t threads, uint32_t cap) {
     const uint32_t room = max_grid_blocks(threads) > tail ? max_grid_blocks(threads) - tail : 0u;
     const uint32_t fit = period ? room / period : cap;
@@ -239,6 +240,7 @@
 void pjb_launch_tet(hipStream_t s, const PJBlk& d, uint32_t tile_first, uint32_t tile_count, hipEvent_t e0 = nullptr,
                     hipEvent_t e1 = nullptr, uint32_t* raise_word = nullptr, uint32_t* clear_word = nullptr);
 void pjb_launch_call(hipStream_t s, const PJBlk& d, const PJCallSched& sched, uint32_t n, uint32_t* err, uint32_t timeout_ms, const DevParams& params, DevParams* params_dev);
+bool pjb_call_pushes();
 void pjb_launch_tet_fused(hipStream_t s, const PJBlk& d, hipEvent_t e0 = nullptr, hipEvent_t e1 = nullptr);
 void pjb_launch_vertex(hipStream_t s, const PJBlk& d, uint32_t first, uint32_t count, hipEvent_t e0 = nullptr, hipEvent_t e1 = nullptr,
                        uint32_t* raise_word = nullptr, uint32_t* clear_word = nullptr);
diff --git a/tetsim_amd/csrc/dev_store.h b/tetsim_amd/csrc/dev_store.h
--- a/tetsim_amd/csrc/dev_store.h
+++ b/tetsim_amd/csrc/dev_store.h
@@ -42,6 +42,11 @@
     return make_float4(__uint_as_float(x.x), __uint_as_float(x.y), __uint_as_float(x.z), __uint_as_float(x.w));
 }
 
+__device__ __forceinline__ uint32_t load_word(const uint32_t* base, uint32_t index) {
+    const __amdgpu_buffer_rsrc_t rsrc = __builtin_amdgcn_make_buffer_rsrc(const_cast<uint32_t*>(base), 0, 0x7fffffff, 0x00020000);
+    return __builtin_amdgcn_raw_buffer_load_b32(rsrc, static_cast<int>(index * 4u), 0, 0);
+}
+
 __device__ __forceinline__ float load_coherent1(const float* base, uint32_t index) {
     const __amdgpu_buffer_rsrc_t rsrc = __builtin_amdgcn_make_buffer_rsrc(const_cast<float*>(base), 0, 0x7fffffff, 0x00020000);
     return __uint_as_float(__builtin_amdgcn_raw_buffer_load_b32(rsrc, static_cast<int>(index * 4u), 0, 0x11));
diff --git a/tetsim_amd/csrc/host_prep.cpp b/tetsim_amd/csrc/host_prep.cpp
--- a/tetsim_amd/csrc/host_prep.cpp
+++ b/tetsim_amd/csrc/host_prep.cpp
@@ -574,9 +574,41 @@
 }
 }
 
+void widen_call_schedule(const uint32_t* entry, uint32_t period, const uint32_t* blk_tet_off, const uint32_t* blk_vert_off, uint32_t nb, std::vector<uint32_t>* wide) {
+    const uint32_t per_xcd = (nb + 7u) / 8u;
+    wide->assign(static_cast<size_t>(period) * kSchedWideWords, 0u);
+    for (uint32_t p = 0; p < period; p++) {
+        uint32_t* w = wide->data() + static_cast<size_t>(p) * kSchedWideWords;
+        w[0] = entry[p];
+        if (entry[p] >> 30 != kSchedTile) continue;
+        const uint32_t b = sched_tile_of(entry[p] & kSchedIndexMask, per_xcd);
+        if (b >= nb) continue;
+        w[1] = blk_tet_off[b]; w[2] = blk_vert_off[b];
+        w[3] = (blk_tet_off[b + 1] - blk_tet_off[b]) | (blk_vert_off[b + 1] - blk_vert_off[b]) << 16;
+    }
+}
+
 std::string check_call_schedule(const int32_t* blk_verts, const uint32_t* blk_vert_off, uint32_t nb, const uint32_t* vp_ell, uint32_t vp_cols,
-                                uint32_t nv_pad, uint32_t nv_owned, const uint32_t* entry, uint32_t period, uint32_t tail, uint32_t tile) {
+                                uint32_t nv_pad, uint32_t nv_owned, const uint32_t* entry, uint32_t period, uint32_t tail, uint32_t tile,
+                                const uint32_t* wide, const uint32_t* blk_tet_off) {
     constexpr uint32_t none = 0xffffffffu;
+    if ((wide == nullptr) != (blk_tet_off == nullptr)) return "a wide table needs blk_tet_off, and blk_tet_off a wide table";
+    {
+        const uint32_t nslots = blk_vert_off[nb];
+        std::vector<uint8_t> listed(nslots, 0);
+        for (uint32_t v = 0; v < nv_owned; v++)
+            for (uint32_t j = 0; j < vp_cols; j++) {
+                const uint32_t idx = vp_ell[static_cast<size_t>(j) * nv_pad + v];
+                if (idx == none) continue;
+                if (idx >= nslots) return "particle " + std::to_string(v) + " lists slot " + std::to_string(idx) + ", which no tile has";
+                if (static_cast<uint32_t>(blk_verts[idx]) != v) return "particle " + std::to_string(v) + " lists slot " + std::to_string(idx) + ", which holds another particle";
+                if (listed[idx]) return "slot " + std::to_string(idx) + " is listed twice";
+                listed[idx] = 1;
+            }
+        for (uint32_t g = 0; g < nslots; g++)
+            if (static_cast<uint32_t>(blk_verts[g]) < nv_owned && !listed[g])
+                return "slot " + std::to_string(g) + " stages particle " + std::to_string(blk_verts[g]) + " but is not on its list";
+    }
     const SchedDeps D = sched_deps(blk_verts, blk_vert_off, nb, vp_ell, vp_cols, nv_pad, nv_owned, tile);
     if (period == 0 || period % 8u != 0u) return "the period is not a positive multiple of 8";
     if (period < D.plain_period) return "the period is shorter than a substep's blocks";
@@ -611,17 +643,29 @@
     for (uint32_t b = 0; b < nb; b++)
         for (uint32_t k : D.pbs_of_tile[b])
             if (!(at_pb[k] < at_tile[b] + period)) return "tile " + std::to_string(b) + " of the next substep does not follow particle block " + std::to_string(k);
+    if (wide) {
+        std::vector<uint32_t> want;
+        widen_call_schedule(entry, period, blk_tet_off, blk_vert_off, nb, &want);
+        for (uint32_t p = 0; p < period; p++)
+            for (uint32_t w = 0; w < kSchedWideWords; w++)
+                if (wide[static_cast<size_t>(p) * kSchedWideWords + w] != want[static_cast<size_t>(p) * kSchedWideWords + w])
+                    return "wide entry " + std::to_string(p) + ", word " + std::to_string(w) + " differs from " + (w ? "the offset arrays" : "the entry");
+        for (uint32_t b = 0; b < nb; b++)
+            if (blk_tet_off[b + 1] - blk_tet_off[b] > 0xffffu || blk_vert_off[b + 1] - blk_vert_off[b] > 0xffffu) return "tile " + std::to_string(b) + " does not fit a wide entry's counts";
+    }
     return "";
 }
 
 void build_call_schedule(const int32_t* blk_verts, const uint32_t* blk_vert_off, uint32_t nb, const uint32_t* vp_ell, uint32_t vp_cols,
-                         uint32_t nv_pad, uint32_t nv_owned, uint32_t lag, CallSchedule* out, uint32_t tile) {
+                         uint32_t nv_pad, uint32_t nv_owned, uint32_t lag, CallSchedule* out, uint32_t tile, const uint32_t* blk_tet_off) {
     constexpr uint32_t none = 0xffffffffu;
     const SchedDeps D = sched_deps(blk_verts, blk_vert_off, nb, vp_ell, vp_cols, nv_pad, nv_owned, tile);
     *out = CallSchedule();
+    auto widen = [&]() { if (blk_tet_off) widen_call_schedule(out->entry.data(), out->period, blk_tet_off, blk_vert_off, nb, &out->wide); };
     auto plain = [&](const std::string& why) {
         sched_plain(D, nb, out);
         out->fell_back = !why.empty(); out->why = why;
+        widen();
     };
     if (lag == 0 || nb == 0) return plain("");
     if (static_cast<uint64_t>(lag) * 8u >= D.plain_period) return plain("lag " + std::to_string(lag) + ": a whole substep or more");
@@ -644,6 +688,7 @@
     out->lag = lag;
     const std::string bad = check_call_schedule(blk_verts, blk_vert_off, nb, vp_ell, vp_cols, nv_pad, nv_owned, out->entry.data(), out->period, out->tail, tile);
     if (!bad.empty()) return plain("lag " + std::to_string(lag) + ": " + bad);
+    widen();
 }
 
 std::string validate_mesh(const float* verts, uint32_t nv, const int32_t* tets, uint32_t nt, bool forbid_repeats) {
diff --git a/tetsim_amd/csrc/host_prep.h b/tetsim_amd/csrc/host_prep.h
--- a/tetsim_amd/csrc/host_prep.h
+++ b/tetsim_amd/csrc/host_prep.h
@@ -114,17 +114,21 @@
     return (((nb + 7u) & ~7u) + (nv_owned + threads - 1u) / threads + 7u) & ~7u;
 }
 constexpr uint32_t kPJCallLagDefault = 0;
+constexpr uint32_t kSchedWideWords = 4u;
 struct CallSchedule {
     std::vector<uint32_t> entry;
+    std::vector<uint32_t> wide;
     uint32_t period = 0, tail = 0;
     uint32_t lag = 0;
     bool fell_back = false;
     std::string why;
 };
 void build_call_schedule(const int32_t* blk_verts, const uint32_t* blk_vert_off, uint32_t nb, const uint32_t* vp_ell, uint32_t vp_cols,
-                         uint32_t nv_pad, uint32_t nv_owned, uint32_t lag, CallSchedule* out, uint32_t tile = kBlockTile);
+                         uint32_t nv_pad, uint32_t nv_owned, uint32_t lag, CallSchedule* out, uint32_t tile = kBlockTile, const uint32_t* blk_tet_off = nullptr);
 std::string check_call_schedule(const int32_t* blk_verts, const uint32_t* blk_vert_off, uint32_t nb, const uint32_t* vp_ell, uint32_t vp_cols,
-                                uint32_t nv_pad, uint32_t nv_owned, const uint32_t* entry, uint32_t period, uint32_t tail, uint32_t tile = kBlockTile);
+                                uint32_t nv_pad, uint32_t nv_owned, const uint32_t* entry, uint32_t period, uint32_t tail, uint32_t tile = kBlockTile,
+                                const uint32_t* wide = nullptr, const uint32_t* blk_tet_off = nullptr);
+void widen_call_schedule(const uint32_t* entry, uint32_t period, const uint32_t* blk_tet_off, const uint32_t* blk_vert_off, uint32_t nb, std::vector<uint32_t>* wide);
 
 std::string validate_mesh(const float* verts, uint32_t nv, const int32_t* tets, uint32_t nt, bool forbid_repeats);
 
diff --git a/tetsim_amd/csrc/pj_blocked.hip b/tetsim_amd/csrc/pj_blocked.hip
--- a/tetsim_amd/csrc/pj_blocked.hip
+++ b/tetsim_amd/csrc/pj_blocked.hip
@@ -59,7 +59,14 @@
 struct PJHaloWait { const PJPeerSync* w; const uint32_t* vflag; uint32_t* error; uint32_t timeout_ms; const float4* ghosts; };
 constexpr int kModeCarried = 0, kModeConstantRest = 1, kModeLeanState = 2;
 inline int blk_mode(const PJBlk& d) { return pjb_mode(d); }
-struct PJPoll { uint32_t block, want; uint32_t* error; uint32_t timeout_ms; };
+struct PJPoll { uint32_t block, want; uint32_t* error; uint32_t timeout_ms; uint32_t t0, v0, ntb, nu; };
+#ifndef TETSIM_CALL_PUSH
+#define TETSIM_CALL_PUSH 0
+#endif
+#ifndef TETSIM_CALL_WIDE
+#define TETSIM_CALL_WIDE 1
+#endif
+constexpr bool kCallPush = TETSIM_CALL_PUSH != 0, kCallWide = TETSIM_CALL_WIDE != 0;
 template <int kMode, bool kFused, bool kAlt = false, bool kHaloWait = false, bool kPoll = false>
 __device__ __forceinline__ void pjb_tet_body(const PJBlk& d, uint32_t tile_first, uint32_t tile_count, uint32_t tiles_per_xcd TETSIM_DBG_PARAM,
                                              [[maybe_unused]] const PJHaloWait* hw = nullptr, const uint32_t stamp = 0u, [[maybe_unused]] const PJPoll* poll = nullptr) {
@@ -78,12 +85,15 @@
     const uint32_t tid = threadIdx.x;
     TETSIM_LAB_TILE_BEGIN();
     TETSIM_POLL_TILE(0);
-    const uint32_t t0 = d.blk_tet_off[b], ntb = d.blk_tet_off[b + 1] - t0;
-    const uint32_t v0 = d.blk_vert_off[b], nu = d.blk_vert_off[b + 1] - v0;
+    uint32_t t0, ntb, v0, nu;
+    if constexpr (kPoll) { t0 = poll->t0; ntb = poll->ntb; v0 = poll->v0; nu = poll->nu; }
+    else { t0 = d.blk_tet_off[b]; ntb = d.blk_tet_off[b + 1] - t0; v0 = d.blk_vert_off[b]; nu = d.blk_vert_off[b + 1] - v0; }
 
     const bool has_slot = tid < nu, has_tet = tid < ntb;
     const uint32_t slot = v0 + (has_slot ? tid : 0u), e = t0 + (has_tet ? tid : 0u);
-    const uint32_t vid = static_cast<uint32_t>(d.blk_verts[slot]);
+    bool pushed = false;
+    if constexpr (kPoll && kCallPush) pushed = poll->want != 0u;
+    const uint32_t vid = pushed ? 0u : static_cast<uint32_t>(d.blk_verts[slot]);
     const uint32_t range = has_slot ? d.lc_range[slot] : 0u;
     uint32_t src[8];
     uint32_t src8 = 0xffffffffu;
@@ -162,7 +172,9 @@
     } else if constexpr (kPoll) {
         TETSIM_POLL_BEGIN();
         TETSIM_POLL_TILE(1);
-        pos_stage = load_coherent(d.pos_pred, vid);
+        const float4* const look = pushed ? d.stage : d.pos_pred;
+        const uint32_t at = pushed ? slot : vid;
+        pos_stage = load_coherent(look, at);
         if (poll->want != 0u) {
             bool pend = has_slot && __float_as_uint(pos_stage.w) != poll->want;
             if (__builtin_amdgcn_ballot_w64(pend) != 0ull) {
@@ -171,7 +183,7 @@
                     __builtin_amdgcn_s_sleep(TETSIM_POLL_SLEEP);
                     TETSIM_POLL_LOOK();
                     asm volatile("" ::: "memory");
-                    if (pend) { pos_stage = load_coherent(d.pos_pred, vid); pend = __float_as_uint(pos_stage.w) != poll->want; }
+                    if (pend) { pos_stage = load_coherent(look, at); pend = __float_as_uint(pos_stage.w) != poll->want; }
                     if (limit && pend && wall_clock64() - t0 > limit) { __hip_atomic_store(poll->error, 1u, __ATOMIC_RELAXED, __HIP_MEMORY_SCOPE_SYSTEM); pend = false; }
                 } while (__builtin_amdgcn_ballot_w64(pend) != 0ull);
             }
@@ -550,9 +562,11 @@
 __global__ __launch_bounds__(64) void pjb_vertex_kernel(PJBlk d, uint32_t first, uint32_t count) { pjb_vertex_body(d, first, count); }
 
 template <int kMode>
-__global__ __launch_bounds__(kTile, 2) void pjb_call_kernel(PJBlk d, uint32_t n_sub, uint32_t tile_count, uint32_t tiles_per_xcd, const uint32_t* __restrict__ sched, uint32_t period,
+__global__ __launch_bounds__(kTile, 2) void pjb_call_kernel(PJBlk d, uint32_t n_sub, uint32_t tile_count, uint32_t tiles_per_xcd, const uint4* __restrict__ sched, uint32_t period,
                                                            uint32_t* err, uint32_t timeout_ms, DevParams pv, DevParams* pdev TETSIM_DBG_PARAM) {
-    const uint32_t turn = blockIdx.x / period, entry = sched[blockIdx.x - turn * period];
+    const uint32_t turn = blockIdx.x / period;
+    const uint4 wide = sched[blockIdx.x - turn * period];
+    const uint32_t entry = wide.x;
     if (blockIdx.x == 0u && threadIdx.x == 0u) store_params(pdev, pv);
     const uint32_t back = (entry & kSchedWrapped) ? 1u : 0u, kind = entry >> 30, r = entry & kSchedIndexMask;
     if (kind == kSchedEmpty || turn < back || turn - back >= n_sub) return;
@@ -560,7 +574,11 @@
     const uint32_t stamp = (d.epoch ? d.epoch : pv.epoch) + sub + 1u;
     TETSIM_LAB_CALL_MARK(sub, n_sub);
     if (kind == kSchedTile) {
-        const PJPoll poll = {r, sub ? stamp - 1u : 0u, err, timeout_ms};
+        PJPoll poll = {r, sub ? stamp - 1u : 0u, err, timeout_ms, wide.y, wide.z, wide.w & 0xffffu, wide.w >> 16};
+        if constexpr (!kCallWide) {
+            const uint32_t b = xcd_tile(r, tiles_per_xcd) < tile_count ? xcd_tile(r, tiles_per_xcd) : 0u;
+            poll.t0 = d.blk_tet_off[b]; poll.ntb = d.blk_tet_off[b + 1] - poll.t0; poll.v0 = d.blk_vert_off[b]; poll.nu = d.blk_vert_off[b + 1] - poll.v0;
+        }
         pjb_tet_body<kMode, false, false, false, true>(d, 0u, tile_count, tiles_per_xcd TETSIM_DBG_ARG, nullptr, stamp, &poll);
         return;
     }
@@ -621,9 +639,21 @@
     }
     TETSIM_POLL_PB(3);
     const VertexOut o = pv.body_params ? pjb_vertex_update<false, true>(xyz(acc), wsum, xyz(prev), pv, v) : pjb_vertex_update<false, false>(xyz(acc), wsum, xyz(prev), pv, v);
+    const float4 pred4 = make_float4(o.pred.x, o.pred.y, o.pred.z, __uint_as_float(stamp));
+    if (kCallPush && sub + 1u < n_sub) {
+        for (uint32_t j0 = 0; j0 < d.vp_cols; j0 += 8u) {
+            uint32_t idx[8];
+#pragma unroll
+            for (uint32_t j = 0; j < 8u; j++) idx[j] = (j0 + j < d.vp_cols) ? load_word(d.vp_ell + static_cast<size_t>(j0 + j) * d.nv_pad, v) : 0xffffffffu;
+#pragma unroll
+            for (uint32_t j = 0; j < 8u; j++)
+                if (idx[j] != 0xffffffffu) store_wt(d.stage, idx[j], pred4);
+            if (__all(idx[7] == 0xffffffffu)) break;
+        }
+    }
     store_wt(d.fin_out, v, make_float4(o.p.x, o.p.y, o.p.z, __uint_as_float(stamp)));
     if (d.vel && sub + 1u == n_sub) store_wt(d.vel, v, make_float4(o.vel.x, o.vel.y, o.vel.z, 0.0f));
-    store_wt(d.pos_pred, v, make_float4(o.pred.x, o.pred.y, o.pred.z, __uint_as_float(stamp)));
+    store_wt(d.pos_pred, v, pred4);
     TETSIM_POLL_PB(4);
     TETSIM_POLL_PB_SAVE();
 }
@@ -735,6 +765,7 @@
     auto* kernel = mode == kModeConstantRest ? pjb_call_kernel<kModeConstantRest> : mode == kModeLeanState ? pjb_call_kernel<kModeLeanState> : pjb_call_kernel<kModeCarried>;
     hipLaunchKernelGGL(kernel, dim3(sched.period * n + sched.tail), dim3(kTile), 0, s, d, n, d.nb, per_xcd, sched.entry, sched.period, err, timeout_ms, params, params_dev TETSIM_DBG_LAUNCH);
 }
+bool pjb_call_pushes() { return kCallPush; }
 void pjb_launch_tet_fused(hipStream_t s, const PJBlk& d, hipEvent_t e0, hipEvent_t e1) { launch_tet_x(s, d, 0u, d.nb, TetFused{0u}, e0, e1); }
 void pjb_launch_frame(hipStream_t s, const PJBlk& d, uint32_t n, const int32_t* block_tile, uint32_t blocks, bool local, float4* pbuf0, float4* pbuf1,
                       uint32_t* err, uint32_t timeout_ms, const DevParams& params, DevParams* params_dev, hipEvent_t e0, hipEvent_t e1) {
diff --git a/tetsim_amd/csrc/tetsim_api.hip b/tetsim_amd/csrc/tetsim_api.hip
--- a/tetsim_amd/csrc/tetsim_api.hip
+++ b/tetsim_amd/csrc/tetsim_api.hip
@@ -106,6 +106,7 @@
             HIPCHK(h, hipMemsetAsync(h->blk.partial, 0, h->partial_slots * sizeof(float4), h->stream));
             HIPCHK(h, hipMemsetAsync(h->partial_b, 0, h->partial_slots * sizeof(float4), h->stream));
         }
+        if (h->blk.stage && h->stage_slots) HIPCHK(h, hipMemsetAsync(h->blk.stage, 0, h->stage_slots * sizeof(float4), h->stream));
         if (h->nh_one_launch) HIPCHK(h, hipMemsetAsync(h->nh_sweep1.exchange, 0, static_cast<size_t>(h->nh.nv) * sizeof(float4), h->stream));
         h->frame_epoch = 1u;
     }
diff --git a/tetsim_amd/csrc/tetsim_create.hip b/tetsim_amd/csrc/tetsim_create.hip
--- a/tetsim_amd/csrc/tetsim_create.hip
+++ b/tetsim_amd/csrc/tetsim_create.hip
@@ -270,12 +270,22 @@
                 const char* lag_env = getenv("TETSIM_PJ_CALL_LAG");
                 const uint32_t lag = lag_env ? static_cast<uint32_t>(std::min<unsigned long>(strtoul(lag_env, nullptr, 10), 1ul << 24)) : kPJCallLagDefault;
                 CallSchedule S;
-                build_call_schedule(B.blk_verts.data(), B.blk_vert_off.data(), B.num_blocks, B.vp_ell.data(), B.vp_cols, B.nv_pad, nvo, lag, &S);
+                build_call_schedule(B.blk_verts.data(), B.blk_vert_off.data(), B.num_blocks, B.vp_ell.data(), B.vp_cols, B.nv_pad, nvo, lag, &S, kBlockTile, B.blk_tet_off.data());
                 if (S.fell_back) fprintf(stderr, "[tetsim] TETSIM_PJ_CALL_LAG=%u ignored (%s): the call runs in the plain order\n", lag, S.why.c_str());
-                uint32_t* dsched;
-                if ((rc = dev_alloc(h, &dsched, S.entry.size()))) return rc;
-                if ((rc = upload(h, dsched, S.entry))) return rc;
+                const std::string bad = check_call_schedule(B.blk_verts.data(), B.blk_vert_off.data(), B.num_blocks, B.vp_ell.data(), B.vp_cols, B.nv_pad, nvo, S.entry.data(),
+                                                            S.period, S.tail, kBlockTile, S.wide.data(), B.blk_tet_off.data());
+                if (!bad.empty()) return fail(h, TETSIM_EINVAL, "internal error: the one-launch call's dispatch table fails its check (" + bad + ")");
+                std::vector<uint4> wide(S.period);
+                for (uint32_t p = 0; p < S.period; p++) wide[p] = make_uint4(S.wide[4ull * p], S.wide[4ull * p + 1], S.wide[4ull * p + 2], S.wide[4ull * p + 3]);
+                uint4* dsched;
+                if ((rc = dev_alloc(h, &dsched, wide.size()))) return rc;
+                if ((rc = upload(h, dsched, wide))) return rc;
                 h->call_sched.entry = dsched; h->call_sched.period = S.period; h->call_sched.tail = S.tail;
+                if (pjb_call_pushes()) {
+                    if ((rc = dev_alloc(h, &k.stage, nslots))) return rc;
+                    HIPCHK(h, hipMemset(k.stage, 0, std::max<size_t>(nslots, 1) * sizeof(float4)));
+                    h->stage_slots = nslots;
+                }
             }
         }
         if (h->fused || h->quad) {
diff --git a/tetsim_amd/csrc/tetsim_host.cpp b/tetsim_amd/csrc/tetsim_host.cpp
--- a/tetsim_amd/csrc/tetsim_host.cpp
+++ b/tetsim_amd/csrc/tetsim_host.cpp
@@ -141,11 +141,7 @@
     if (dropped) *dropped = d;
     return 0;
 }
-int tetsim_prep_call_tiles(const float* verts, uint32_t nv, const int32_t* tets, uint32_t nt, uint32_t sizes[4], uint32_t* blk_vert_off,
-                           int32_t* blk_verts, uint32_t* vp_ell) {
-    if (!sizes) return TETSIM_EINVAL;
-    std::string e = validate_mesh(verts, nv, tets, nt, false);
-    if (!e.empty()) return fail(nullptr, TETSIM_EINVAL, e);
+static void call_tiling(const float* verts, uint32_t nv, const int32_t* tets, uint32_t nt, BlockPlan* B) {
     const std::vector<uint32_t> order = morton_vertex_order(verts, nv, 0, nv);
     std::vector<int32_t> to_dev(nv), ltets(4ull * nt);
     std::vector<float> lverts(3ull * nv);
@@ -155,8 +151,15 @@
     }
     for (uint64_t i = 0; i < 4ull * nt; i++) ltets[i] = to_dev[tets[i]];
     const Incidence inc = build_incidence(ltets.data(), nt, nv, false, false);
+    build_blocks(lverts.data(), ltets.data(), nt, nv, nv, inc, B);
+}
+int tetsim_prep_call_tiles(const float* verts, uint32_t nv, const int32_t* tets, uint32_t nt, uint32_t sizes[4], uint32_t* blk_vert_off,
+                           int32_t* blk_verts, uint32_t* vp_ell) {
+    if (!sizes) return TETSIM_EINVAL;
+    std::string e = validate_mesh(verts, nv, tets, nt, false);
+    if (!e.empty()) return fail(nullptr, TETSIM_EINVAL, e);
     BlockPlan B;
-    build_blocks(lverts.data(), ltets.data(), nt, nv, nv, inc, &B);
+    call_tiling(verts, nv, tets, nt, &B);
     sizes[0] = B.num_blocks; sizes[1] = static_cast<uint32_t>(B.blk_verts.size()); sizes[2] = B.vp_cols; sizes[3] = B.nv_pad;
     if (blk_vert_off) std::copy(B.blk_vert_off.begin(), B.blk_vert_off.end(), blk_vert_off);
     if (blk_verts) std::copy(B.blk_verts.begin(), B.blk_verts.end(), blk_verts);
@@ -183,6 +186,40 @@
                                     uint32_t nv_pad, uint32_t nv_owned, const uint32_t* entry, uint32_t period, uint32_t tail) {
     if (!blk_vert_off || (nb && !blk_verts) || (vp_cols && !vp_ell) || !entry) return TETSIM_EINVAL;
     const std::string bad = check_call_schedule(blk_verts, blk_vert_off, nb, vp_ell, vp_cols, nv_pad, nv_owned, entry, period, tail);
+    return bad.empty() ? 0 : fail(nullptr, TETSIM_EINVAL, "call schedule: " + bad);
+}
+int tetsim_prep_call_tile_tets(const float* verts, uint32_t nv, const int32_t* tets, uint32_t nt, uint32_t* blk_tet_off, uint32_t capacity) {
+    if (!blk_tet_off) return TETSIM_EINVAL;
+    std::string e = validate_mesh(verts, nv, tets, nt, false);
+    if (!e.empty()) return fail(nullptr, TETSIM_EINVAL, e);
+    BlockPlan B;
+    call_tiling(verts, nv, tets, nt, &B);
+    if (capacity < B.num_blocks + 1u) return fail(nullptr, TETSIM_EINVAL, "tetsim_prep_call_tile_tets: blk_tet_off needs " + std::to_string(B.num_blocks + 1u) + " entries");
+    std::copy(B.blk_tet_off.begin(), B.blk_tet_off.end(), blk_tet_off);
+    return 0;
+}
+int tetsim_prep_call_schedule_wide(const int32_t* blk_verts, const uint32_t* blk_vert_off, const uint32_t* blk_tet_off, uint32_t nb, const uint32_t* vp_ell,
+                                   uint32_t vp_cols, uint32_t nv_pad, uint32_t nv_owned, uint32_t lag, uint32_t* wide, uint32_t capacity, uint32_t* period,
+                                   uint32_t* tail, int32_t* fell_back) {
+    if (!blk_vert_off || !blk_tet_off || (nb && !blk_verts) || (vp_cols && !vp_ell) || !period || !tail) return TETSIM_EINVAL;
+    if (nv_owned > nv_pad && vp_cols) return fail(nullptr, TETSIM_EINVAL, "tetsim_prep_call_schedule_wide: nv_owned exceeds the column stride of vp_ell");
+    CallSchedule S;
+    build_call_schedule(blk_verts, blk_vert_off, nb, vp_ell, vp_cols, nv_pad, nv_owned, lag, &S, kBlockTile, blk_tet_off);
+    *period = S.period; *tail = S.tail;
+    if (fell_back) *fell_back = S.fell_back ? 1 : 0;
+    if (S.fell_back) fail(nullptr, TETSIM_OK, "tetsim_prep_call_schedule_wide: " + S.why + " -- the plain order instead");
+    if (wide) {
+        if (capacity < S.period) return fail(nullptr, TETSIM_EINVAL, "tetsim_prep_call_schedule_wide: the table needs " + std::to_string(S.period) + " entries");
+        std::copy(S.wide.begin(), S.wide.end(), wide);
+    }
+    return 0;
+}
+int tetsim_prep_check_call_schedule_wide(const int32_t* blk_verts, const uint32_t* blk_vert_off, const uint32_t* blk_tet_off, uint32_t nb, const uint32_t* vp_ell,
+                                         uint32_t vp_cols, uint32_t nv_pad, uint32_t nv_owned, const uint32_t* wide, uint32_t period, uint32_t tail) {
+    if (!blk_vert_off || !blk_tet_off || (nb && !blk_verts) || (vp_cols && !vp_ell) || !wide) return TETSIM_EINVAL;
+    std::vector<uint32_t> entry(period);
+    for (uint32_t p = 0; p < period; p++) entry[p] = wide[static_cast<size_t>(p) * kSchedWideWords];
+    const std::string bad = check_call_schedule(blk_verts, blk_vert_off, nb, vp_ell, vp_cols, nv_pad, nv_owned, entry.data(), period, tail, kBlockTile, wide, blk_tet_off);
     return bad.empty() ? 0 : fail(nullptr, TETSIM_EINVAL, "call schedule: " + bad);
 }
 int tetsim_prep_ref_grab_texels(int32_t grab_id, uint32_t num_elems, uint32_t num_particles, int32_t out[2]) {
```

Result: no change. 35290 M tet-solves/s, median of 6 (+0.4%).
